# OpenMined/PIR

Hardware: AMD Instinct MI355X
Metric: PIR queries/sec (ms/query in ms_per_step), N=4096 DB=2^20 x 288B d=2 (higher is better)
Workload: dtype u64; 1 GPU; N=4096, 2 RNS data primes (36,36 bit | special 37 bit), t=24 bit, DB=2^20 x 288B, d=2, dims=[162, 162], num_pt=26215, 64 queries/step (whole job), 16 in flight per GPU (BASELINE.json configs[2]); workers=16, dist_mode=single, exchange=none, parallelism=single GPU, database_copies_in_hbm=operand layout only (u64 staging released)

## Files before the change

pir_amd/csrc/ctx.hip:

```cpp
#include <hip/hip_runtime.h>
#include <ctype.h>
#include <stdint.h>
#include <stdio.h>
#include <stdlib.h>
#include <string.h>

#include <algorithm>
#include <atomic>
#include <functional>
#include <map>
#include <mutex>
#include <string>
#include <vector>

#include "../../include/pirgpu.h"
#include "ctmult.h"
#include "device_params.h"
#include "host_math.h"
#include "kernels.h"
#include "wire.h"

using namespace pirgpu;

namespace {
// ... 142 lines not shown
struct pirgpu_ctx {
  pirgpu_params prm{};
  uint32_t N = 0, logN = 0, k = 0, d = 0;
  size_t ctw = 0;
  uint32_t rp = 0;
  size_t rctw = 0;
  uint32_t dims[PIRGPU_MAX_DIMS]{};
  uint64_t stride[PIRGPU_MAX_DIMS + 1]{};
  uint32_t sv_off[PIRGPU_MAX_DIMS + 1]{};
  uint32_t dim_sum = 0;
  uint32_t er = 0, E = 0;
  uint64_t reply_cts = 1;
  uint64_t P = 0;
  uint32_t sb = 0, se = 0;
  uint32_t slot0 = 0, nslots = 0;
  bool slot_sharded = false;
  hipEvent_t ev_after = nullptr;
  uint64_t pt_begin = 0, pt_end = 0;
  uint32_t planes = 1;
  uint64_t plane_pad = 0;
  uint32_t tables = 1;
  uint64_t table_pad = 0;
  uint32_t cur_table = 0;
  std::vector<uint64_t> tbl_loaded, tbl_zero;
  std::vector<uint8_t> tbl_packed;
  uint64_t scan_launches = 0;
  uint64_t ct_blocks = 0;
  uint64_t ct_relins = 0;
  uint64_t ct_lifts = 0;
  uint32_t bits = 0;

  int device = 0;
  hipStream_t stream = nullptr;
  const NttOps* ops = nullptr;
  int mode = kNttInt;
  DevParams hp{};
  DevParams* dp = nullptr;
  std::vector<void*> allocs;

  uint64_t* d_db = nullptr;
  std::vector<uint8_t> loaded;
  uint64_t n_loaded = 0;
  std::vector<KeySet> keysets{1};
  uint32_t keyset_cap = 64;
  uint32_t cur_keyset = 0;
  uint32_t cur_keyset_gen = 0;
  uint64_t keyset_clock = 0, key_uploads = 0, keyset_evictions = 0;
  std::vector<uint64_t*> key_pool;
  uint64_t* d_key_stage = nullptr;
  std::map<uint32_t, uint64_t*> xpow;
  std::map<uint32_t, uint16_t*> gperm;

  bool ws_ready = false;
  std::vector<Worker> workers;
  std::vector<uint64_t> lvl_rows;
  std::vector<uint64_t> lvl_cts;
  uint64_t m_max = 1;
  uint64_t pt_words = 0;
  BatchSet sets[kBatchSets];
  BatchSet& bs();
  uint32_t n_active = 1;
  uint32_t upper_blocks = 512;
  uint32_t upper_blocks_batch = 64;
  uint32_t scan_wgs_batch = 128;
  bool in_batch = false;
  uint32_t scan_nsplit = 1, scan_cps = 0, scan_rows = 0, scan_cols = 0;
  uint32_t scan_rpt = 4, scan_block = 256;
  bool scan_limb = false;
  uint32_t mq_nq = 4, mq_rows = 1;
  bool mq_single = true;
  uint32_t mq_single_rows = 4;
  bool mq_single_limb = false;
  uint64_t scan_npt = 0;
  bool mfma_on = false;
  MfmaGeom mg{};
  uint32_t mfma_nq = kMaxMfmaQueries;
  bool mfma_single = true;
  bool scan_f64_fold = false;
  bool scan_f64_fold_batch = false;
  bool split_upper = false;
  uint64_t split_upper_words = (3ull << 30) / 8;
  bool loop_transforms = true;
  uint32_t loop_min_sources = 1024;
  uint32_t fuse_mac_nodes = 128;
  bool fuse_mac_combine = true;
  bool fuse_last_level = true;
  bool last_level_ntt = true;
  bool tree40 = true;
  bool c0_ntt = false;
  bool c0_ntt_split = false;
  bool want_sel_f64 = true;
  bool sel_f64 = false;
  bool pack40 = false;
  int pack_bytes = 5;
  uint8_t* d_dbp = nullptr;
  bool packed_valid = false;
  bool staging_released = false;
  bool streamed = false;
  uint64_t stream_bands = 1;
  uint64_t db_bytes = 0, dbp_alloc = 0, mem_scratch = 0, mem_peak = 0;
  std::vector<BatchLane> lanes;
  uint64_t groups_run = 0;
  hipStream_t head_stream = nullptr;
  uint32_t head_levels = 5;
  uint32_t head_mode = 1;
  hipEvent_t ev_head_tail = nullptr;
  hipStream_t copy_stream = nullptr;
  hipEvent_t ev_fetch[2] = {nullptr, nullptr};
  hipEvent_t ev_fork = nullptr;
  hipEvent_t ev_main_join = nullptr;

  bool ctm = false;
  bool ctm_deferred = false;
  uint32_t kb = 0;
  uint64_t aux_primes[PIRGPU_MAX_PRIMES]{};
  DevParams hp_aux{};
  DevParams* dp_aux = nullptr;
  CtmParams* d_ctm = nullptr;
  uint64_t ctm_scratch_words = (256ull << 20) / 8;
  bool ctm_shared_sel = false;
  std::map<hipStream_t, CtmScratch> ctm_ws;

  bool prof = false;
  std::vector<hipEvent_t> bscan_ev;
  uint32_t bscan_n = 0, bscan_wgs = 0, bscan_nq = 0;
  static constexpr int kMaxProfRuns = 256;
  std::vector<hipEvent_t> ev;
  int prof_runs = 0;
  int prof_cur = -1;
  float timings[6]{};

  std::map<std::string, int64_t> opts;
  std::string err;
  uint64_t gen = 0;
  std::recursive_mutex mu;
  uint64_t zero_pts = 0;
  uint64_t remote_zero_pts = 0;
  bool allow_transparent = false;

  template <typename T>
  T* dalloc(size_t count) {
    void* p = nullptr;
    HIP_TRY(hipMalloc(&p, std::max<size_t>(count, 1) * sizeof(T)));
    allocs.push_back(p);
    return static_cast<T*>(p);
  }
  void use_device() { HIP_TRY(hipSetDevice(device)); }
};

BatchSet& pirgpu_ctx::bs() { return sets[t_batch_set]; }

static inline uint64_t held_pts(const pirgpu_ctx* c) { return (uint64_t)c->tables * c->planes * (c->pt_end - c->pt_begin); }
static inline uint64_t matrix_pts(const pirgpu_ctx* c) {
  return c->planes > 1 ? (uint64_t)c->planes * c->plane_pad : c->pt_end - c->pt_begin;
}
static inline uint64_t db_row(const pirgpu_ctx* c, uint64_t index) {
  if (c->tables > 1) return index / c->P * c->table_pad + index % c->P;
  return c->planes > 1 ? index / c->P * c->plane_pad + index % c->P : index - c->pt_begin;
}
static inline const uint64_t* table_db(const pirgpu_ctx* c, uint32_t t) {
  return c->d_db ? c->d_db + (size_t)t * c->table_pad * c->k * c->N : nullptr;
}
static inline void note_mem(pirgpu_ctx* c) {
  c->mem_peak = std::max(c->mem_peak, c->db_bytes + c->dbp_alloc + c->mem_scratch);
}
struct ScratchNote {
// ... 177 lines not shown

uint64_t stream_band_bytes(const pirgpu_ctx* c) { return 16ull * c->scan_cols * c->k * c->N * 8; }

int64_t option(const pirgpu_ctx* c, const char* name, int64_t dflt, bool* present = nullptr) {
  if (present) *present = true;
  auto it = c->opts.find(name);
  if (it != c->opts.end()) return it->second;
  const std::string env = std::string("PIRGPU_") + name;
  const char* v = pirgpu_env(env.c_str());
  if (v && *v) return strtoll(v, nullptr, 10);
  if (present) *present = false;
  return dflt;
}

void sync_batch_streams(pirgpu_ctx* c) {
  for (BatchLane& ln : c->lanes)
    if (ln.stream) HIP_TRY(hipStreamSynchronize(ln.stream));
  if (c->head_stream) HIP_TRY(hipStreamSynchronize(c->head_stream));
  if (c->copy_stream) HIP_TRY(hipStreamSynchronize(c->copy_stream));
  for (Worker& w : c->workers)
    if (w.stream) HIP_TRY(hipStreamSynchronize(w.stream));
}

bool all_zero_bytes(const uint8_t* p, size_t n) {
  for (size_t i = 0; i < n; ++i)
    if (p[i]) return false;
  return true;
}

void note_plaintext(pirgpu_ctx* c, uint64_t local, bool zero) {
  uint8_t& st = c->loaded[local];
  if (c->tables > 1) {
    const uint64_t t = local / c->P;
    if (!st) ++c->tbl_loaded[t];
    if (st == 2) --c->tbl_zero[t];
    if (zero) ++c->tbl_zero[t];
  }
  if (!st) ++c->n_loaded;
  if (st == 2) --c->zero_pts;
  st = zero ? 2 : 1;
  if (zero) ++c->zero_pts;
}

bool table_loaded(const pirgpu_ctx* c, uint32_t t) {
  return c->tables > 1 ? c->tbl_loaded[t] == c->P : c->n_loaded == held_pts(c);
}

void check_transparent(pirgpu_ctx* c, uint32_t table = 0) {
  const uint64_t zeros = c->tables > 1 ? c->tbl_zero[table] : c->zero_pts || c->remote_zero_pts;
  if (zeros && !c->allow_transparent) throw Fail{PIRGPU_INTERNAL, "result ciphertext is transparent"};
}

struct TablePlan {
  std::vector<uint32_t> order, run_begin;
  bool identity = true;
};
TablePlan plan_table_runs(const uint32_t* tables, uint32_t count, uint32_t group) {
  TablePlan tp;
  tp.order.resize(count);
  for (uint32_t i = 0; i < count; ++i) tp.order[i] = i;
  std::stable_sort(tp.order.begin(), tp.order.end(), [&](uint32_t a, uint32_t b) { return tables[a] < tables[b]; });
  group = std::max<uint32_t>(group, 1);
  for (uint32_t i = 0; i < count; ++i) {
    tp.identity = tp.identity && tp.order[i] == i;
    if (i == 0 || i % group == 0 || tables[tp.order[i]] != tables[tp.order[i - 1]]) tp.run_begin.push_back(i);
  }
  tp.run_begin.push_back(count);
  return tp;
}

void alloc_worker(pirgpu_ctx* c, Worker& w);
void ensure_expansion_buffers(pirgpu_ctx* c, Worker& w);

void ensure_workspace(pirgpu_ctx* c) {
  if (c->ws_ready) return;
  const uint32_t N = c->N, k = c->k, d = c->d;

  const uint64_t m_max = std::min<uint64_t>(N, hm::next_power_two(std::max<uint32_t>(c->dim_sum, 1)));
  c->m_max = m_max;
  const uint64_t shard_pts = matrix_pts(c);
  c->upper_blocks = (uint32_t)std::max<int64_t>(1, option(c, "UPPER_BLOCKS", c->upper_blocks));
  c->upper_blocks_batch = (uint32_t)std::max<int64_t>(1, option(c, "UPPER_BLOCKS_BATCH", c->upper_blocks_batch));
  c->scan_wgs_batch = (uint32_t)std::max<int64_t>(0, option(c, "SCAN_MFMA_WGS_BATCH", c->scan_wgs_batch));
  c->upper_blocks_batch = std::min(c->upper_blocks_batch, c->upper_blocks);
  c->lvl_rows.assign(d, 0);
  c->lvl_cts.assign(d, 0);
  uint64_t pt_words = 0;
  for (uint32_t l = 0; l < d; ++l) {
    uint64_t rows = l == 0 ? c->planes : ceil_div(shard_pts, c->stride[l]);
    uint64_t C = 1;
    for (uint32_t x = l; x + 1 < d; ++x) C *= c->E;
    c->lvl_rows[l] = rows;
    c->lvl_cts[l] = std::max<uint64_t>(rows, 1) * C;
    if (l + 1 < d) {
      const uint64_t per_chunk = std::max<uint64_t>(rows, 1) * (C / c->E) * c->E * k;
      const uint64_t n_chunks = std::min<uint64_t>(c->dims[l], std::max<uint64_t>(1, ceil_div(c->upper_blocks, per_chunk)));
      pt_words = std::max<uint64_t>(pt_words, (n_chunks + 1) * std::max<uint64_t>(rows, 1) * C * 2 * k * N);
    }
  }
  c->pt_words = pt_words;
  if (d == 1) {
    c->scan_rows = c->planes;
    c->scan_cols = (uint32_t)(shard_pts / c->planes);
  } else {
    c->scan_cols = c->dims[d - 1];
    c->scan_rows = (uint32_t)ceil_div(shard_pts, c->scan_cols);
  }
  c->scan_npt = shard_pts;
  {
    auto env_u32 = [c](const char* name, uint32_t dflt) {
      return (uint32_t)option(c, name + 7, dflt);
    };
    c->scan_limb = true;
    for (uint32_t j = 0; j < k; ++j) c->scan_limb = c->scan_limb && (c->hp.mod[j].q >> 50) == 0;
    if (!env_u32("PIRGPU_SCAN_LIMB", 1)) c->scan_limb = false;
    c->mq_nq = 4;
    c->mq_rows = 1;
    c->mq_single = env_u32("PIRGPU_SCAN_MQ_SINGLE", 1) != 0;
    c->mq_single_rows = 4;
    c->mq_single_limb = false;
    c->scan_rpt = env_u32("PIRGPU_SCAN_ROWS", 4);
    c->scan_block = env_u32("PIRGPU_SCAN_BLOCK", 256);
    const uint32_t xblocks = (k * N / 2 + c->scan_block - 1) / c->scan_block;
    const uint32_t yblocks = (c->scan_rows + c->scan_rpt - 1) / c->scan_rpt;
    uint64_t have = (uint64_t)xblocks * std::max<uint32_t>(yblocks, 1) * c->scan_block / 256;
    uint32_t want = have >= 512 ? 1 : (uint32_t)ceil_div(1024, std::max<uint64_t>(have, 1));
    want = env_u32("PIRGPU_SCAN_NSPLIT", want);
    want = std::max<uint32_t>(1, std::min<uint32_t>(want, std::max<uint32_t>(c->scan_cols, 1)));
    c->scan_cps = (uint32_t)ceil_div(std::max<uint32_t>(c->scan_cols, 1), want);
    c->scan_nsplit = (uint32_t)ceil_div(std::max<uint32_t>(c->scan_cols, 1), c->scan_cps);
    c->fuse_last_level = env_u32("PIRGPU_FUSE_LAST", 1) != 0;
    c->fuse_mac_combine = env_u32("PIRGPU_FUSE_MAC_COMBINE", 1) != 0;
    c->last_level_ntt = env_u32("PIRGPU_LAST_NTT", 1) != 0;
    {
      const uint32_t v = env_u32("PIRGPU_C0_NTT", 0);
      c->c0_ntt = v != 0;
      c->c0_ntt_split = v >= 2;
    }
    c->want_sel_f64 = env_u32("PIRGPU_SEL_F64", 1) != 0;
    c->tree40 = env_u32("PIRGPU_TREE40", 1) != 0;
    c->fuse_mac_nodes = 128;
    c->head_levels = std::min<uint32_t>(env_u32("PIRGPU_HEAD_LEVELS", c->head_levels), 8);
    c->head_mode = std::min<uint32_t>(env_u32("PIRGPU_HEAD_MODE", c->head_mode), 2);
    c->split_upper = env_u32("PIRGPU_SPLIT_UPPER", c->logN >= 14 ? 1 : 0) != 0 && c->mode != kNttInt;
    if (c->logN >= 15) c->split_upper = true;
    c->split_upper_words = (uint64_t)env_u32("PIRGPU_SPLIT_UPPER_MB", 3072) * (1ull << 20) / 8;
    c->loop_transforms = env_u32("PIRGPU_LOOP_TRANSFORMS", 1) != 0 && c->mode != kNttInt;
    c->pack40 = env_u32("PIRGPU_PACK40", 1) != 0;
    {
      uint32_t bits = 0;
      for (uint32_t j = 0; j <= k; ++j) bits = std::max<uint32_t>(bits, 64 - (uint32_t)__builtin_clzll(c->hp.mod[j].q));
      const int need = bits <= 39 ? 5 : (bits <= 47 ? 6 : (bits <= 55 ? 7 : 8));
      int want = (int)env_u32("PIRGPU_PACK_BYTES", (uint32_t)need);
      if (want < need) want = need;
      if (c->mode == kNttInt && want != 5) want = 8;
      if (c->logN >= 15) want = 8;
      if (want > 7) c->pack40 = false;
      c->pack_bytes = c->pack40 ? want : 5;
      if (c->pack40 && c->pack_bytes == 7 && c->logN >= 14 && !env_u32("PIRGPU_TREE40_WIDE", 0)) c->tree40 = false;
      const NttOps* ops = ntt_ops_for(N, c->pack_bytes);
      if (ops != c->ops) {
        c->ops = ops;
        HIP_TRY(c->ops->configure(c->mode));
      }
    }
    bool wide_given = false;
// ... 118 lines not shown
}

void begin_profiled_run(pirgpu_ctx* c) {
  c->prof_cur = -1;
  if (!c->prof || c->prof_runs >= pirgpu_ctx::kMaxProfRuns) return;
  if (c->ev.empty()) {
    c->ev.resize((size_t)pirgpu_ctx::kMaxProfRuns * (PH_COUNT + 1));
    for (auto& e : c->ev) HIP_TRY(hipEventCreate(&e));
  }
  c->prof_cur = c->prof_runs++;
}

const uint64_t* xpow_table(pirgpu_ctx* c, hipStream_t st, uint32_t shift) {
  auto it = c->xpow.find(shift);
  if (it != c->xpow.end()) return it->second;
  const uint32_t N = c->N, k = c->k;
  std::vector<uint64_t> h((size_t)k * N, 0);
  for (uint32_t j = 0; j < k; ++j) h[(size_t)j * N + (N - shift)] = c->hp.mod[j].q - 1;
  uint64_t* buf = c->dalloc<uint64_t>((size_t)k * N);
  HIP_TRY(hipMemcpy(buf, h.data(), h.size() * 8, hipMemcpyHostToDevice));
  HIP_TRY(c->ops->ntt_batch(st, c->mode, c->dp, buf, k, k, 0, false));
  HIP_TRY(launch_tree_convert(st, c->dp, c->mode, buf, buf, (uint64_t)k * N, true));
  HIP_TRY(hipStreamSynchronize(st));
  c->xpow[shift] = buf;
  return buf;
}

const uint16_t* galois_perm_table(pirgpu_ctx* c, hipStream_t st, uint32_t g) {
  auto it = c->gperm.find(g);
  if (it != c->gperm.end()) return it->second;
  const uint32_t N = c->N, logN = c->logN, R = (uint32_t)ntt_log_ept((int)logN), EPT = 1u << R, NT = N >> R;
  auto brev = [&](uint32_t v) {
    uint32_t r = 0;
    for (uint32_t b = 0; b < logN; ++b) r |= ((v >> b) & 1u) << (logN - 1 - b);
    return r;
  };
  std::vector<uint16_t> h((size_t)2 * N);
  const uint32_t gs[2] = {g, galois_inverse(g, N)};
  for (int w = 0; w < 2; ++w)
    for (uint32_t P = 0; P < N; ++P) {
      const uint32_t ex = (uint32_t)(((uint64_t)(2 * brev(P) + 1) * gs[w]) & (2 * N - 1));
      const uint32_t Pin = brev(ex >> 1);
      const uint32_t slot = (Pin & (EPT - 1)) * NT + (Pin >> R);
      h[(size_t)w * N + P] = (uint16_t)(slot + (slot >> R));
    }
  uint16_t* buf = c->dalloc<uint16_t>((size_t)2 * N);
  HIP_TRY(hipMemcpy(buf, h.data(), h.size() * 2, hipMemcpyHostToDevice));
  HIP_TRY(hipStreamSynchronize(st));
  c->gperm[g] = buf;
  return buf;
}

struct TreeState {
  uint64_t* cur = nullptr;
  bool cur40 = false;
  bool c0ntt = false;
};

uint64_t* expand_core(pirgpu_ctx* c, hipStream_t st, uint64_t* res_a, uint64_t* res_b, uint64_t* dig, uint64_t* prod,
                      uint32_t n, uint32_t B, const MfmaPtrs* sel_dst = nullptr, bool sel_f64 = false,
                      const uint32_t* ksets = nullptr, uint32_t j_begin = 0, uint32_t j_end = UINT32_MAX,
                      const TreeState* from = nullptr, TreeState* to = nullptr,
                      const std::function<void()>& after_first = nullptr) {
  const uint32_t N = c->N, k = c->k;
  if (n > N) throw Fail{PIRGPU_INVALID_ARGUMENT, "Cannot expand more items from a CT than poly modulus degree"};
  const uint32_t logm = hm::ceil_log2(n);
  const bool fuse_last = sel_dst && c->mode != kNttInt && c->fuse_last_level;
  if (sel_f64 && !(fuse_last && c->last_level_ntt && n >= 2)) throw Fail{PIRGPU_INTERNAL, "double-form selectors need the NTT-domain last level"};
  uint64_t *cur = res_a, *nxt = res_b;
  bool cur40 = false;
  bool c0ntt = false;
  if (from) {
    cur = from->cur;
    cur40 = from->cur40;
    c0ntt = from->c0ntt;
    nxt = res_a;
  }
  const uint32_t j_stop = std::min(j_end, logm);
  const bool c0_path = c->c0_ntt && fuse_last && c->last_level_ntt && c->mode != kNttInt && c->fuse_mac_combine;
  const uint32_t fuse_from = B > 1 ? std::max<uint32_t>(c->fuse_mac_nodes / 2, 1) : c->fuse_mac_nodes;
  auto level_fused = [&](uint32_t j) {
    return c->mode != kNttInt && c->fuse_mac_combine && ((1u << j) * B) >= fuse_from && !(fuse_last && j + 1 == logm);
  };
  for (uint32_t j = j_begin; j < j_stop; ++j) {
    auto level_done = [&]() {
      if (from && j == j_begin) {
        nxt = res_b;
        if (after_first) after_first();
      }
    };
    const uint32_t g = (N >> j) + 1;
    const KeyPtrs key = keys_for(c, g, ksets, B);
    const uint32_t nodes = (1u << j) * B;
    const bool last_ntt = fuse_last && j + 1 == logm && c->last_level_ntt;
    const bool c0_in_digit = last_ntt && !c0ntt && ks_digit_takes_c0(nodes);
    if (cur40 && !(last_ntt ? (c0ntt || c0_in_digit) : true)) throw Fail{PIRGPU_INTERNAL, "5-byte tree reached a level that cannot read it"};
    if (c0_path && !c0ntt && level_fused(j) && !cur40 && !(from && j == j_begin)) {
      HIP_TRY(c->ops->tree_c0_fwd(st, c->mode, c->dp, k, cur, nodes));
      c0ntt = true;
    }
    HIP_TRY(c->ops->ks_digit(st, c->mode, c->dp, k, cur, g, nodes, dig, c->pack40, c0_in_digit ? prod : nullptr, cur40,
                             c->loop_transforms && (uint64_t)nodes * k >= c->loop_min_sources));
    if (level_fused(j)) {
      const uint32_t next_nodes = nodes * 2;
      const bool next_last = j + 2 == logm;
      const bool next_reads40 = next_last ? (fuse_last && c->last_level_ntt && (c0ntt || ks_digit_takes_c0(next_nodes)))
                                          : (next_nodes >= fuse_from);
      const bool out40 = c->tree40 && c->pack40 && j + 1 < logm && next_reads40 && (1u << j) < (N >> ntt_log_ept((int)c->logN));
      HIP_TRY(c->ops->ks_mac_intt(st, c->mode, c->dp, k, dig, key, nodes, prod, c->pack40, k, 1));
      HIP_TRY(c->ops->ks_mac_combine(st, c->mode, c->dp, k, dig, key, prod, cur, g, nodes, 1u << j, nxt, c->pack40, cur40,
                                     out40, c0ntt ? xpow_table(c, st, 1u << j) : nullptr,
                                     c0ntt ? galois_perm_table(c, st, g) : nullptr, c->c0_ntt_split));
      cur40 = out40;
      std::swap(cur, nxt);
      level_done();
      continue;
    }
    if (cur40 && !last_ntt) throw Fail{PIRGPU_INTERNAL, "5-byte tree reached an unfused level"};
    if (c0ntt && !last_ntt) throw Fail{PIRGPU_INTERNAL, "NTT-form c0 reached an unfused level"};
    if (fuse_last && j + 1 == logm && c->last_level_ntt) {
      const uint64_t* X = xpow_table(c, st, 1u << j);
      HIP_TRY(c->ops->ks_mac_intt(st, c->mode, c->dp, k, dig, key, nodes, prod, c->pack40, k, 1));
      HIP_TRY(c->ops->ks_last_ntt(st, c->mode, c->dp, k, cur, dig, key, prod, X, g, galois_inverse(g, N), 1u << j, n, B,
                                  *sel_dst, nodes, c->pack40, sel_f64, c0_in_digit, c0ntt ? (cur40 ? 2 : 1) : 0,
                                  galois_perm_table(c, st, g)));
      return nullptr;
    }
    HIP_TRY(c->ops->ks_mac_intt(st, c->mode, c->dp, k, dig, key, nodes, prod, c->pack40, 0, k + 1));
    if (fuse_last && j + 1 == logm) {
      HIP_TRY(c->ops->ks_last_level(st, c->mode, c->dp, k, cur, prod, g, 1u << j, n, B, *sel_dst, nodes, c->pack40));
      return nullptr;
    }
    const uint32_t hi_limit = j + 1 == logm ? n * B : UINT32_MAX;
    HIP_TRY(launch_ks_combine(st, c->dp, c->mode, N, k, cur, prod, galois_inverse(g, N), nodes, 1u << j, true, hi_limit,
                              c->pack40, nxt, c->pack_bytes));
    std::swap(cur, nxt);
    if (c0_path && j + 1 < logm && level_fused(j + 1)) {
      HIP_TRY(c->ops->tree_c0_fwd(st, c->mode, c->dp, k, cur, nodes * 2));
      c0ntt = true;
    }
    level_done();
  }
  if (to) {
    to->cur = cur;
    to->cur40 = cur40;
    to->c0ntt = c0ntt;
  }
  return cur;
}

uint64_t* expand_on_device(pirgpu_ctx* c, Worker& w, uint32_t n) {
  ensure_expansion_buffers(c, w);
  return expand_core(c, w.stream, w.res_a, w.res_b, w.dig, w.prod, n, 1, nullptr, false, &w.keyset);
}

void expand_query_to_sv(pirgpu_ctx* c, Worker& w, const uint64_t* d_query, uint32_t nq) {
  ensure_expansion_buffers(c, w);
  w.sv_cur = nullptr;
  w.sv_rows = nullptr;
  const uint32_t N = c->N, k = c->k;
  const size_t ctw = c->ctw;
  uint64_t remaining = c->dim_sum;
  uint64_t produced = 0;
  for (uint32_t q = 0; q < nq; ++q) {
    uint32_t n = (uint32_t)std::min<uint64_t>(remaining, N);
    if (n > 0) {
      HIP_TRY(launch_tree_convert(w.stream, c->dp, c->mode, d_query + (size_t)q * ctw, w.res_a, ctw, true));
      MfmaPtrs dst{};
      dst.p[0] = w.sv_ntt + produced * ctw;
      uint64_t* res = expand_core(c, w.stream, w.res_a, w.res_b, w.dig, w.prod, n, 1, &dst, false, &w.keyset);
      if (res) HIP_TRY(c->ops->ct_ntt_fwd_oop(w.stream, c->mode, c->dp, k, res, w.sv_ntt + produced * ctw, n, true));
    }
    produced += n;
    remaining -= n;
    if (remaining == 0) break;
  }
}

const uint64_t* scan_selectors(pirgpu_ctx* c, Worker& w) {
  const uint64_t* sv = w.sv_cur ? w.sv_cur : w.sv_ntt;
  return sv + (size_t)c->sv_off[c->d - 1] * c->ctw + (c->d == 1 ? (size_t)c->sb * c->ctw : 0);
}

bool mq_usable(pirgpu_ctx* c) { return c->scan_nsplit == 1 && c->scan_rows >= 1 && c->scan_cols >= 1; }

size_t dbp_bytes(const pirgpu_ctx* c) { return (size_t)c->nslots * c->mg.RT * c->mg.KG * c->mg.tile_bytes; }
uint8_t* table_dbp(const pirgpu_ctx* c, uint32_t t) { return c->d_dbp ? c->d_dbp + (size_t)t * dbp_bytes(c) : nullptr; }

void refuse_tables(const pirgpu_ctx* c) {
  if (c->tables > 1)
    throw Fail{PIRGPU_FAILED_PRECONDITION, "this context holds several tables (tables > 1): the multi-GPU entry points do "
                                           "not serve them"};
}

void refuse_wide(const pirgpu_ctx* c) {
  if (c->planes > 1)
    throw Fail{PIRGPU_FAILED_PRECONDITION, "this context holds wide items (plaintexts_per_item > 1): the multi-GPU entry "
                                           "points do not serve them"};
}

void refuse_switched(const pirgpu_ctx* c) {
  if (c->rp)
    throw Fail{PIRGPU_FAILED_PRECONDITION, "this context switches its results to fewer primes (result_primes > 0): the "
                                           "multi-GPU entry points do not serve it"};
}

void refuse_ctm(const pirgpu_ctx* c) {
  if (c->ctm)
    throw Fail{PIRGPU_FAILED_PRECONDITION, "this context multiplies ciphertexts (PIRGPU_CREATE_CT_MULTIPLY): the multi-GPU "
                                           "entry points do not serve it"};
}
// ... 187 lines not shown
  HIP_TRY(launch_ctm_lift(st, c->d_ctm, k, N, a, a_qstride, b, dim, nq, j0, n, r.xq, r.xb));
  HIP_TRY(c->ops->ntt_batch(st, c->mode, c->dp, r.xq, (uint64_t)n * 4 * k, k, 0, false));
  HIP_TRY(c->ops->ntt_batch(st, c->mode, c->dp_aux, r.xb, (uint64_t)n * 4 * kb, kb, 0, false));
  HIP_TRY(launch_ctm_tensor(st, c->dp, k, N, r.xq, r.yq, n));
  HIP_TRY(launch_ctm_tensor(st, c->dp_aux, kb, N, r.xb, r.yb, n));
  HIP_TRY(c->ops->ntt_batch(st, c->mode, c->dp, r.yq, (uint64_t)n * 3 * k, k, 0, true));
  HIP_TRY(c->ops->ntt_batch(st, c->mode, c->dp_aux, r.yb, (uint64_t)n * 3 * kb, kb, 0, true));
  HIP_TRY(launch_ctm_scale(st, c->d_ctm, k, N, r.yq, r.yb, r.d, n));
}

struct CtmSel {
  CtmSelPtrs q, b;
};
void ctm_products_sel(pirgpu_ctx* c, hipStream_t st, const CtmRegions& r, const uint64_t* a, uint64_t a_qstride,
                      const CtmSel& sel, uint32_t dim, uint32_t nq, uint32_t j0, uint32_t n) {
  const uint32_t N = c->N, k = c->k, kb = c->kb;
  HIP_TRY(launch_ctm_lift_polys(st, c->d_ctm, k, N, a, a_qstride, nq, j0, n, r.xq, r.xb));
  HIP_TRY(c->ops->ntt_batch(st, c->mode, c->dp, r.xq, (uint64_t)n * 2 * k, k, 0, false));
  HIP_TRY(c->ops->ntt_batch(st, c->mode, c->dp_aux, r.xb, (uint64_t)n * 2 * kb, kb, 0, false));
  HIP_TRY(launch_ctm_tensor_sel(st, c->dp, k, N, r.xq, sel.q, dim, nq, j0, r.yq, n));
  HIP_TRY(launch_ctm_tensor_sel(st, c->dp_aux, kb, N, r.xb, sel.b, dim, nq, j0, r.yb, n));
  HIP_TRY(c->ops->ntt_batch(st, c->mode, c->dp, r.yq, (uint64_t)n * 3 * k, k, 0, true));
  HIP_TRY(c->ops->ntt_batch(st, c->mode, c->dp_aux, r.yb, (uint64_t)n * 3 * kb, kb, 0, true));
  HIP_TRY(launch_ctm_scale(st, c->d_ctm, k, N, r.yq, r.yb, r.d, n));
}

constexpr uint64_t kCtmRowsumWgs = 512;
uint32_t ctm_rowsum_block(pirgpu_ctx* c, hipStream_t st, const CtmRegions& r, uint32_t cap, const uint64_t* a,
                          uint64_t a_qstride, const uint64_t* b, uint32_t dim, uint32_t nq, uint64_t nch, uint32_t j0, uint32_t nj,
                          const CtmSel* sel = nullptr) {
  const uint32_t N = c->N, k = c->k, kb = c->kb, n = nj * nq;
  const uint64_t end = (uint64_t)j0 + nj;
  const uint32_t row0 = j0 / dim, rows = (uint32_t)((end - 1) / dim) - row0 + 1;
  const bool cut = end < nch && end % dim != 0;
  const uint32_t fin = rows - (cut ? 1 : 0);
  const uint64_t wgs = (uint64_t)rows * nq * k * (N / 256);
  const uint64_t room = (uint64_t)cap / ((uint64_t)rows * nq);
  uint32_t splits = (uint32_t)std::min<uint64_t>({ceil_div(kCtmRowsumWgs, wgs), (uint64_t)nj, room ? room - 1 : 0});
  const int64_t most = option(c, "CT_ROWSUM_SPLITS", 0);
  if (most > 0) splits = (uint32_t)std::min<int64_t>(splits, most);
  if (splits < 2) splits = 1;
  if ((uint64_t)(splits > 1 ? splits + 1 : 1) * rows * nq > cap) throw Fail{PIRGPU_INTERNAL, "row-sum accumulators exceed the product scratch"};
  if (sel) {
    HIP_TRY(launch_ctm_lift_polys(st, c->d_ctm, k, N, a, a_qstride, nq, j0, n, r.xq, r.xb));
    HIP_TRY(c->ops->ntt_batch(st, c->mode, c->dp, r.xq, (uint64_t)n * 2 * k, k, 0, false));
    HIP_TRY(c->ops->ntt_batch(st, c->mode, c->dp_aux, r.xb, (uint64_t)n * 2 * kb, kb, 0, false));
    HIP_TRY(launch_ctm_tensor_rowsum_sel(st, c->dp, k, N, r.xq, sel->q, r.yq, dim, nq, j0, nj, splits));
    HIP_TRY(launch_ctm_tensor_rowsum_sel(st, c->dp_aux, kb, N, r.xb, sel->b, r.yb, dim, nq, j0, nj, splits));
  } else {
    HIP_TRY(launch_ctm_lift(st, c->d_ctm, k, N, a, a_qstride, b, dim, nq, j0, n, r.xq, r.xb));
    HIP_TRY(c->ops->ntt_batch(st, c->mode, c->dp, r.xq, (uint64_t)n * 4 * k, k, 0, false));
    HIP_TRY(c->ops->ntt_batch(st, c->mode, c->dp_aux, r.xb, (uint64_t)n * 4 * kb, kb, 0, false));
    HIP_TRY(launch_ctm_tensor_rowsum(st, c->dp, k, N, r.xq, r.yq, dim, nq, j0, nj, splits));
    HIP_TRY(launch_ctm_tensor_rowsum(st, c->dp_aux, kb, N, r.xb, r.yb, dim, nq, j0, nj, splits));
  }
  if (fin) {
    HIP_TRY(c->ops->ntt_batch(st, c->mode, c->dp, r.yq, (uint64_t)fin * nq * 3 * k, k, 0, true));
    HIP_TRY(c->ops->ntt_batch(st, c->mode, c->dp_aux, r.yb, (uint64_t)fin * nq * 3 * kb, kb, 0, true));
    HIP_TRY(launch_ctm_scale(st, c->d_ctm, k, N, r.yq, r.yb, r.d, fin * nq));
  }
  return fin;
}
void ctm_carry_row(pirgpu_ctx* c, hipStream_t st, const CtmRegions& r, uint32_t nq, uint32_t fin) {
  const size_t wq = (size_t)nq * 3 * c->k * c->N, wb = (size_t)nq * 3 * c->kb * c->N;
  if (!fin) return;
  HIP_TRY(hipMemcpyAsync(r.yq, r.yq + fin * wq, wq * 8, hipMemcpyDeviceToDevice, st));
  HIP_TRY(hipMemcpyAsync(r.yb, r.yb + fin * wb, wb * 8, hipMemcpyDeviceToDevice, st));
}

KeyPtrs relin_keys_for(pirgpu_ctx* c, const uint32_t* ksets, uint32_t nq) {
  for (uint32_t q = 0; q < nq; ++q) {
    const uint32_t slot = ksets[q];
    if (slot >= c->keysets.size() || !c->keysets[slot].keys.count(1))
      throw Fail{PIRGPU_INVALID_ARGUMENT, "RelinKeys missing: ciphertext multiplication at d >= 2 needs the client's "
                                          "relinearisation key (installed as the key of Galois element 1)"};
  }
  return keys_for(c, 1, ksets, nq);
}

void ctm_relinearize(pirgpu_ctx* c, hipStream_t st, const CtmRegions& r, uint32_t n, const KeyPtrs& key) {
  const uint32_t N = c->N, k = c->k;
  const uint64_t pw = (uint64_t)k * N;
  HIP_TRY(launch_tree_convert(st, c->dp, c->mode, r.d, r.xq, (uint64_t)n * 2 * pw, true, 2 * pw, 3 * pw));
  HIP_TRY(c->ops->ks_digit(st, c->mode, c->dp, k, r.xq, 1, n, r.dig, c->pack40, nullptr, false, false));
  HIP_TRY(c->ops->ks_mac_intt(st, c->mode, c->dp, k, r.dig, key, n, r.prod, c->pack40, 0, k + 1));
  HIP_TRY(launch_ks_combine(st, c->dp, c->mode, N, k, r.xq, r.prod, 1, n, 0, false, 0, c->pack40, r.yq, c->pack_bytes));
  if (c->mode != kNttInt) HIP_TRY(launch_tree_convert(st, c->dp, c->mode, r.yq, r.yq, (uint64_t)n * 2 * pw, false));
}

void post_scan_ctm_level(pirgpu_ctx* c, const Stage& sg, uint32_t l) {
  const uint32_t N = c->N, k = c->k, nq = sg.n, dim = c->dims[l];
  const size_t ctw = c->ctw;
  const uint64_t nch = c->lvl_rows[l + 1], rows = c->lvl_rows[l];
  hipStream_t st = sg.stream;
  if (nq > (uint32_t)kMaxMfmaQueries || sg.local_rows || sg.sel_f64) throw Fail{PIRGPU_INTERNAL, "unexpected stage in ciphertext-multiplication mode"};
  const KeyPtrs key = relin_keys_for(c, sg.ksets, nq);
  CtmScratch& ws = ctm_scratch(c, st);
  const uint32_t cap = ctm_cap_pairs(c);
  const CtmRegions r = ctm_regions(c, ws.buf, cap);
  if ((size_t)nq * dim * ctw > ws.selc_words) throw Fail{PIRGPU_INTERNAL, "selector scratch undersized"};
  for (uint32_t q = 0; q < nq; ++q)
    HIP_TRY(hipMemcpyAsync(ws.selc + (size_t)q * dim * ctw, static_cast<const uint64_t*>(sg.sel.p[q]) + (size_t)c->sv_off[l] * ctw,
                           (size_t)dim * ctw * 8, hipMemcpyDeviceToDevice, st));
  HIP_TRY(c->ops->ntt_batch(st, c->mode, c->dp, ws.selc, (uint64_t)nq * dim * 2 * k, k, 0, true));
  const bool shared = c->ctm_shared_sel;
  CtmSel sel{};
  if (shared) {
    if (!ws.selb) throw Fail{PIRGPU_INTERNAL, "shared-selector scratch missing"};
    for (uint32_t s0 = 0; s0 < nq * dim; s0 += 32767)
      HIP_TRY(launch_ctm_lift_polys(st, c->d_ctm, k, N, ws.selc + (size_t)s0 * ctw, 0, 1, 0, std::min<uint32_t>(32767, nq * dim - s0),
                                    nullptr, ws.selb + (size_t)s0 * 2 * c->kb * N));
    HIP_TRY(c->ops->ntt_batch(st, c->mode, c->dp_aux, ws.selb, (uint64_t)nq * dim * 2 * c->kb, c->kb, 0, false));
    c->ct_lifts += (uint64_t)2 * dim * nq;
    for (uint32_t q = 0; q < nq; ++q) {
      sel.q.p[q] = static_cast<const uint64_t*>(sg.sel.p[q]) + (size_t)c->sv_off[l] * ctw;
      sel.b.p[q] = ws.selb + (size_t)q * dim * 2 * c->kb * N;
    }
  }
  const uint32_t bj = std::max<uint32_t>(1, cap / nq);
  for (uint64_t j0 = 0; j0 < nch; j0 += bj) {
    const uint32_t nj = (uint32_t)std::min<uint64_t>(bj, nch - j0), n = nj * nq;
    ++c->ct_blocks;
    c->ct_lifts += (uint64_t)(shared ? 2 : 4) * n;
    if (c->ctm_deferred) {
      const uint32_t fin = ctm_rowsum_block(c, st, r, cap, sg.lvl[l + 1], c->lvl_cts[l + 1] * ctw, ws.selc, dim, nq, nch,
                                            (uint32_t)j0, nj, shared ? &sel : nullptr);
      if (!fin) continue;
      c->ct_relins += (uint64_t)fin * nq;
      ctm_relinearize(c, st, r, fin * nq, key);
      HIP_TRY(launch_ctm_accumulate(st, c->dp, k, N, r.yq, r.d, sg.lvl[l] + (size_t)(j0 / dim) * ctw, c->lvl_cts[l] * ctw, 1,
                                    nq, 0, fin, fin));
      if ((j0 + nj) % dim != 0 && j0 + nj < nch) ctm_carry_row(c, st, r, nq, fin);
      continue;
    }
    c->ct_relins += n;
    if (shared)
      ctm_products_sel(c, st, r, sg.lvl[l + 1], c->lvl_cts[l + 1] * ctw, sel, dim, nq, (uint32_t)j0, n);
    else
      ctm_products(c, st, r, sg.lvl[l + 1], c->lvl_cts[l + 1] * ctw, ws.selc, dim, nq, (uint32_t)j0, n);
    ctm_relinearize(c, st, r, n, key);
    HIP_TRY(launch_ctm_accumulate(st, c->dp, k, N, r.yq, r.d, sg.lvl[l], c->lvl_cts[l] * ctw, dim, nq, (uint32_t)j0, nj,
                                  (uint32_t)rows));
  }
}

void post_scan_stage(pirgpu_ctx* c, const Stage& sg, Worker* profiled) {
  const uint32_t N = c->N, k = c->k, d = c->d;
  const size_t ctw = c->ctw;
  const uint64_t shard_pts = matrix_pts(c);
  hipStream_t st = sg.stream;
  if (c->rp && !sg.last) throw Fail{PIRGPU_INTERNAL, "result_primes without a level-0 buffer"};
  auto level = [&](uint32_t l) { return c->rp && l == 0 ? sg.last : sg.lvl[l]; };
  auto switch_level = [&](uint32_t l) {
    if (!c->rp) return;
    const uint64_t qstride = c->lvl_cts[l] * ctw;
    if (l == 0)
      HIP_TRY(launch_mod_switch(st, c->dp, sg.last, sg.lvl[0], c->lvl_cts[0], k, c->rp, N, true, sg.n, qstride,
                                c->reply_cts * c->rctw));
    else
      HIP_TRY(launch_mod_switch(st, c->dp, sg.lvl[l], sg.lvl[l], c->lvl_cts[l], k, c->rp, N, false, sg.n, qstride, qstride));
  };
  if (shard_pts == 0) {
    HIP_TRY(hipMemsetAsync(sg.lvl[0], 0, (size_t)sg.n * c->reply_cts * c->rctw * 8, st));
    return;
  }
  if (profiled) record(c, *profiled, PH_UPPER);
  if (!sg.rows_inverted)
    HIP_TRY(c->ops->ntt_batch(st, c->mode, c->dp, level(d - 1), (uint64_t)sg.n * c->scan_rows * 2 * k, k, 0, true));
// ... 315 lines not shown
    for (size_t i = 1; i < c->workers.size(); ++i)
      if (c->workers[i].stream) (void)hipStreamSynchronize(c->workers[i].stream);
  }
  for (KeySet& ks : c->keysets)
    for (auto& kv : ks.keys) (void)hipFree(kv.second);
  for (uint64_t* p : c->key_pool) (void)hipFree(p);
  for (void* p : c->allocs) (void)hipFree(p);
  for (BatchSet& b : c->sets) {
    if (b.h_query) (void)hipHostFree(b.h_query);
    if (b.h_reply) (void)hipHostFree(b.h_reply);
    for (hipEvent_t e : b.dl_events) (void)hipEventDestroy(e);
    for (hipEvent_t e : b.rd_events) (void)hipEventDestroy(e);
    for (hipEvent_t e : b.st_events) (void)hipEventDestroy(e);
  }
  for (auto& e : c->ev) (void)hipEventDestroy(e);
  for (auto& e : c->bscan_ev) (void)hipEventDestroy(e);
  for (Worker& w : c->workers) {
    if (w.ev_expanded) (void)hipEventDestroy(w.ev_expanded);
    if (w.ev_scanned) (void)hipEventDestroy(w.ev_scanned);
    if (w.ev_done) (void)hipEventDestroy(w.ev_done);
    if (w.ev_join) (void)hipEventDestroy(w.ev_join);
  }
  for (BatchLane& ln : c->lanes) {
    if (ln.ev_scanned) (void)hipEventDestroy(ln.ev_scanned);
    if (ln.ev_join) (void)hipEventDestroy(ln.ev_join);
    if (ln.stream) (void)hipStreamDestroy(ln.stream);
  }
  if (c->head_stream) {
    (void)hipStreamSynchronize(c->head_stream);
    (void)hipStreamDestroy(c->head_stream);
  }
  if (c->ev_head_tail) (void)hipEventDestroy(c->ev_head_tail);
  for (BatchLane& ln : c->lanes)
    for (HeadSlot& hs : ln.head) {
      if (hs.ev_ready) (void)hipEventDestroy(hs.ev_ready);
      if (hs.ev_free) (void)hipEventDestroy(hs.ev_free);
    }
  if (c->copy_stream) {
    (void)hipStreamSynchronize(c->copy_stream);
    (void)hipStreamDestroy(c->copy_stream);
  }
  for (hipEvent_t e : c->ev_fetch)
    if (e) (void)hipEventDestroy(e);
  if (c->ev_fork) (void)hipEventDestroy(c->ev_fork);
  if (c->ev_after) (void)hipEventDestroy(c->ev_after);
  if (c->ev_main_join) (void)hipEventDestroy(c->ev_main_join);
  for (size_t i = 1; i < c->workers.size(); ++i)
    if (c->workers[i].stream) (void)hipStreamDestroy(c->workers[i].stream);
  if (c->stream) (void)hipStreamDestroy(c->stream);
  delete c;
}

const char* pirgpu_last_error(const pirgpu_ctx* c) {
  if (!c) return "null context";
  if (t_last_error_ctx == c && t_last_error_gen == c->gen)
    return t_last_error.c_str();
  return c->err.c_str();
}

void pirgpu_set_error(pirgpu_ctx* c, const char* message) { (void)fail(c, 0, message ? message : ""); }

void pirgpu_request_lock(pirgpu_ctx* c) {
  if (c) c->mu.lock();
}
void pirgpu_request_unlock(pirgpu_ctx* c) {
  if (c) c->mu.unlock();
}

int pirgpu_set_transparent_policy(pirgpu_ctx* c, int allow) {
  return guarded(c, [&]() -> int {
    c->allow_transparent = allow != 0;
    return PIRGPU_OK;
  });
}

static const struct { const char* name; bool early; } kOptions[] = {
    {"UPPER_BLOCKS", true}, {"UPPER_BLOCKS_BATCH", true}, {"SCAN_MFMA_WGS_BATCH", false}, {"SCAN_LIMB", true},
    {"SCAN_MQ_SINGLE", true}, {"SCAN_ROWS", true}, {"SCAN_BLOCK", true}, {"SCAN_NSPLIT", true},
    {"FUSE_LAST", true}, {"FUSE_MAC_COMBINE", true}, {"LAST_NTT", true}, {"C0_NTT", true}, {"SEL_F64", true}, {"TREE40", true},
    {"SPLIT_UPPER", true}, {"SPLIT_UPPER_MB", true}, {"PACK40", true}, {"PACK_BYTES", true}, {"TREE40_WIDE", true},
    {"SCAN_MFMA", true}, {"SCAN_MFMA_WIDE", true}, {"SCAN_MFMA_TOP4", true}, {"SCAN_MFMA_NQ", true}, {"SCAN_MFMA_SINGLE", true},
    {"HEAD_LEVELS", true}, {"HEAD_MODE", true}, {"SCAN_F64_FOLD", true}, {"SCAN_F64_FOLD_BATCH", true}, {"LOOP_TRANSFORMS", true},
    {"SLOTS_SCAN_WGS", false}, {"SLOTS_GATHER_NTT", false}, {"SLOTS_SCAN_BLK_MAJOR", false}, {"DB_STREAM_MB", true},
    {"CT_SCRATCH_MB", true}, {"CT_SHARED_SEL", true},
    {"TABLES_ONE_LAUNCH", false}, {"SCAN_LAUNCHES", false},
    {"CT_BLOCKS", false},
    {"CT_RELINS", false}, {"CT_ROWSUM_SPLITS", false},
    {"CT_LIFTS", false},
};

int pirgpu_set_option(pirgpu_ctx* c, const char* name, int64_t value) {
  return guarded(c, [&]() -> int {
    if (!name) return fail(c, PIRGPU_INVALID_ARGUMENT, "null option name");
    std::string up(name);
    for (char& ch : up) ch = (char)toupper((unsigned char)ch);
    for (const auto& o : kOptions) {
      if (up != o.name) continue;
      if (o.early && c->ws_ready)
        return fail(c, PIRGPU_FAILED_PRECONDITION, "option " + up + " shapes the workspace: set it before the context is first used");
      if (up == "SCAN_LAUNCHES") {
        c->scan_launches = (uint64_t)std::max<int64_t>(0, value);
        return PIRGPU_OK;
      }
      if (up == "CT_BLOCKS") {
        c->ct_blocks = (uint64_t)std::max<int64_t>(0, value);
        return PIRGPU_OK;
      }
      if (up == "CT_RELINS") {
        c->ct_relins = (uint64_t)std::max<int64_t>(0, value);
        return PIRGPU_OK;
      }
      if (up == "CT_LIFTS") {
        c->ct_lifts = (uint64_t)std::max<int64_t>(0, value);
        return PIRGPU_OK;
      }
      c->opts[up] = value;
      if (up == "SCAN_MFMA_WGS_BATCH") c->scan_wgs_batch = (uint32_t)std::max<int64_t>(0, value);
      return PIRGPU_OK;
    }
    return fail(c, PIRGPU_INVALID_ARGUMENT, "unknown option " + up);
  });
}

int pirgpu_get_option(pirgpu_ctx* c, const char* name, int64_t* value) {
  return guarded(c, [&]() -> int {
    if (!name || !value) return fail(c, PIRGPU_INVALID_ARGUMENT, "null argument");
    std::string up(name);
    for (char& ch : up) ch = (char)toupper((unsigned char)ch);
    for (const auto& o : kOptions)
      if (up == o.name) {
        bool present = false;
        *value = option(c, o.name, -1, &present);
        if (up == "SCAN_LAUNCHES") *value = (int64_t)c->scan_launches;
        if (up == "CT_BLOCKS") *value = (int64_t)c->ct_blocks;
        if (up == "CT_RELINS") *value = (int64_t)c->ct_relins;
        if (up == "CT_LIFTS") *value = (int64_t)c->ct_lifts;
        if (up == "CT_SHARED_SEL" && !present) *value = c->ctm && c->planes > 1;
        return PIRGPU_OK;
      }
    return fail(c, PIRGPU_INVALID_ARGUMENT, "unknown option " + up);
  });
}

uint64_t pirgpu_zero_plaintexts(const pirgpu_ctx* c) { return c ? c->zero_pts : 0; }

int pirgpu_set_remote_zero_plaintexts(pirgpu_ctx* c, uint64_t n) {
  return guarded(c, [&]() -> int {
    c->remote_zero_pts = n;
    return PIRGPU_OK;
  });
}

int pirgpu_check_ready(pirgpu_ctx* c) {
  return guarded(c, [&]() -> int {
    if (!table_loaded(c, c->cur_table)) return fail(c, PIRGPU_FAILED_PRECONDITION, "database not fully loaded");
    check_transparent(c, c->cur_table);
    return PIRGPU_OK;
  });
}

int pirgpu_get_params(const pirgpu_ctx* c, pirgpu_params* out) {
  if (!c || !out) return PIRGPU_INVALID_ARGUMENT;
  *out = c->prm;
  out->shard_begin = c->sb;
  out->shard_end = c->se;
  return PIRGPU_OK;
}

uint64_t pirgpu_db_size(const pirgpu_ctx* c) { return c ? c->n_loaded : 0; }
uint32_t pirgpu_planes(const pirgpu_ctx* c) { return c ? c->planes : 0; }
uint64_t pirgpu_reply_ct_count(const pirgpu_ctx* c) { return c ? c->reply_cts : 0; }
uint64_t pirgpu_reply_ct_words(const pirgpu_ctx* c) { return c ? c->rctw : 0; }

int pirgpu_mod_switch(pirgpu_ctx* c, const uint64_t* cts, uint64_t n, uint32_t r, uint64_t* out) {
  return guarded(c, [&]() -> int {
    if ((!cts || !out) && n) return fail(c, PIRGPU_INVALID_ARGUMENT, "null buffer");
    if (r < 1 || r >= c->k) return fail(c, PIRGPU_INVALID_ARGUMENT, "r must be in [1, num_data_primes)");
    if (!n) return PIRGPU_OK;
    const size_t in_words = (size_t)n * c->ctw, out_words = (size_t)n * 2 * r * c->N;
    uint64_t* dev = nullptr;
    HIP_TRY(hipMalloc((void**)&dev, (in_words + out_words) * 8));
    try {
      HIP_TRY(hipMemcpyAsync(dev, cts, in_words * 8, hipMemcpyHostToDevice, c->stream));
      HIP_TRY(launch_mod_switch(c->stream, c->dp, dev, dev + in_words, n, c->k, r, c->N, true));
      HIP_TRY(hipMemcpyAsync(out, dev + in_words, out_words * 8, hipMemcpyDeviceToHost, c->stream));
      HIP_TRY(hipStreamSynchronize(c->stream));
    } catch (...) {
      (void)hipFree(dev);
      throw;
    }
    HIP_TRY(hipFree(dev));
    return PIRGPU_OK;
  });
}
int pirgpu_ctmult_plan(uint32_t N, uint32_t k, const uint64_t* coeff_modulus, uint64_t special_prime, uint64_t plain_modulus,
                       uint64_t* aux_primes, uint32_t* n_aux) {
  return pirgpu_ctmult_plan_terms(N, k, coeff_modulus, special_prime, plain_modulus, 1, aux_primes, n_aux);
}

int pirgpu_ctmult_plan_terms(uint32_t N, uint32_t k, const uint64_t* coeff_modulus, uint64_t special_prime,
                             uint64_t plain_modulus, uint64_t terms, uint64_t* aux_primes, uint32_t* n_aux) {
  if (!coeff_modulus || !aux_primes) return PIRGPU_INVALID_ARGUMENT;
  if (n_aux) *n_aux = 0;
  uint64_t aux[kCtmMaxB] = {};
  if (const char* why = ctm::plan(N, k, coeff_modulus, special_prime, plain_modulus, aux, terms)) {
    g_create_error = why;
    return PIRGPU_INVALID_ARGUMENT;
  }
  for (uint32_t i = 0; i < k + 2; ++i) aux_primes[i] = aux[i];
  if (n_aux) *n_aux = k + 2;
  return PIRGPU_OK;
}

int pirgpu_ct_multiply(pirgpu_ctx* c, const uint64_t* a, const uint64_t* b, uint64_t n, uint64_t* out) {
  return guarded(c, [&]() -> int {
    if (!c->ctm) return fail(c, PIRGPU_FAILED_PRECONDITION, "not a ciphertext-multiplication context (PIRGPU_CREATE_CT_MULTIPLY)");
    if ((!a || !b || !out) && n) return fail(c, PIRGPU_INVALID_ARGUMENT, "null buffer");
    ensure_workspace(c);
    CtmScratch& ws = ctm_scratch(c, c->stream);
    const uint32_t cap = ctm_cap_pairs(c);
// ... 1122 lines not shown
  if (rc) return rc;
  return pirgpu_query_fetch(c, reply, cap, count);
}

uint64_t* pirgpu_reply_device_ptr(pirgpu_ctx* c) { return (c && c->ws_ready) ? c->workers[0].lvl[0] : nullptr; }

int pirgpu_reply_copy_to_device(pirgpu_ctx* c, uint64_t* dst, uint64_t cap) {
  return guarded(c, [&]() -> int {
    refuse_switched(c);
    refuse_ctm(c);
    if (c->workers.empty()) return fail(c, PIRGPU_FAILED_PRECONDITION, "no query has been run");
    Worker& w = c->workers[0];
    if (!w.reply_valid) return fail(c, PIRGPU_FAILED_PRECONDITION, "no query has been run");
    if (!dst || cap < c->reply_cts) return fail(c, PIRGPU_INVALID_ARGUMENT, "reply buffer too small");
    HIP_TRY(hipMemcpyAsync(dst, w.lvl[0], c->reply_cts * c->rctw * 8, hipMemcpyDeviceToDevice, c->stream));
    HIP_TRY(hipStreamSynchronize(c->stream));
    return PIRGPU_OK;
  });
}

int pirgpu_expand(pirgpu_ctx* c, const uint64_t* ct, uint32_t num_items, uint64_t* out) {
  return guarded(c, [&]() -> int {
    ensure_workspace(c);
    Worker& w = c->workers[0];
    if (!ct || (!out && num_items)) return fail(c, PIRGPU_INVALID_ARGUMENT, "null buffer");
    if (num_items > c->N)
      return fail(c, PIRGPU_INVALID_ARGUMENT, "Cannot expand more items from a CT than poly modulus degree");
    const uint64_t m_max = std::min<uint64_t>(c->N, hm::next_power_two(std::max<uint32_t>(c->dim_sum, 1)));
    if (hm::next_power_two(num_items) > m_max)
      return fail(c, PIRGPU_INVALID_ARGUMENT, "num_items exceeds this context's expansion workspace");
    w.keyset = current_keyset(c);
    HIP_TRY(hipMemcpyAsync(w.res_b, ct, c->ctw * 8, hipMemcpyHostToDevice, c->stream));
    HIP_TRY(launch_tree_convert(c->stream, c->dp, c->mode, w.res_b, w.res_a, c->ctw, true));
    uint64_t* res = expand_on_device(c, w, num_items);
    if (num_items) {
      HIP_TRY(launch_tree_convert(c->stream, c->dp, c->mode, res, res, (uint64_t)num_items * c->ctw, false));
      HIP_TRY(hipMemcpyAsync(out, res, (size_t)num_items * c->ctw * 8, hipMemcpyDeviceToHost, c->stream));
    }
    HIP_TRY(hipStreamSynchronize(c->stream));
    return PIRGPU_OK;
  });
}

int pirgpu_expand_multi(pirgpu_ctx* c, const uint64_t* cts, uint32_t num_cts, uint64_t total_items, uint64_t* out) {
  return guarded(c, [&]() -> int {
    ensure_workspace(c);
    Worker& w = c->workers[0];
    if (!cts || !out) return fail(c, PIRGPU_INVALID_ARGUMENT, "null buffer");
    if (num_cts != total_items / c->N + 1)
      return fail(c, PIRGPU_INVALID_ARGUMENT,
                  "Number of ciphertexts doesn't match number of items for oblivious expansion.");
    const uint64_t m_max = std::min<uint64_t>(c->N, hm::next_power_two(std::max<uint32_t>(c->dim_sum, 1)));
    uint64_t remaining = total_items, produced = 0;
    w.keyset = current_keyset(c);
    for (uint32_t q = 0; q < num_cts && remaining; ++q) {
      uint32_t n = (uint32_t)std::min<uint64_t>(remaining, c->N);
      if (hm::next_power_two(n) > m_max)
        return fail(c, PIRGPU_INVALID_ARGUMENT, "total_items exceeds this context's expansion workspace");
      HIP_TRY(hipMemcpyAsync(w.res_b, cts + (size_t)q * c->ctw, c->ctw * 8, hipMemcpyHostToDevice, c->stream));
      HIP_TRY(launch_tree_convert(c->stream, c->dp, c->mode, w.res_b, w.res_a, c->ctw, true));
      uint64_t* res = expand_on_device(c, w, n);
      HIP_TRY(launch_tree_convert(c->stream, c->dp, c->mode, res, res, (uint64_t)n * c->ctw, false));
      HIP_TRY(hipMemcpyAsync(out + produced * c->ctw, res, (size_t)n * c->ctw * 8, hipMemcpyDeviceToHost, c->stream));
      HIP_TRY(hipStreamSynchronize(c->stream));
      produced += n;
      remaining -= n;
    }
    return PIRGPU_OK;
  });
}

int pirgpu_substitute_power_x(pirgpu_ctx* c, uint64_t* ct, uint32_t power) {
  return guarded(c, [&]() -> int {
    ensure_workspace(c);
    Worker& w = c->workers[0];
    if (!ct) return fail(c, PIRGPU_INVALID_ARGUMENT, "null buffer");
    if (!(power & 1) || power >= 2 * c->N)
      return fail(c, PIRGPU_INTERNAL, "Galois element is not valid");
    KeyPtrs key{};
    key.p[0] = find_key(c, current_keyset(c), power);
    key.B = 1;
    HIP_TRY(hipMemcpyAsync(w.res_b, ct, c->ctw * 8, hipMemcpyHostToDevice, c->stream));
    HIP_TRY(launch_tree_convert(c->stream, c->dp, c->mode, w.res_b, w.res_a, c->ctw, true));
    HIP_TRY(c->ops->ks_digit(c->stream, c->mode, c->dp, c->k, w.res_a, power, 1, w.dig, c->pack40, nullptr, false, false));
    HIP_TRY(c->ops->ks_mac_intt(c->stream, c->mode, c->dp, c->k, w.dig, key, 1, w.prod, c->pack40, 0, c->k + 1));
    HIP_TRY(launch_ks_combine(c->stream, c->dp, c->mode, c->N, c->k, w.res_a, w.prod, galois_inverse(power, c->N), 1, 0,
                              false,  0, c->pack40, w.res_b, c->pack_bytes));
    HIP_TRY(launch_tree_convert(c->stream, c->dp, c->mode, w.res_b, w.res_b, c->ctw, false));
    HIP_TRY(hipMemcpyAsync(ct, w.res_b, c->ctw * 8, hipMemcpyDeviceToHost, c->stream));
    HIP_TRY(hipStreamSynchronize(c->stream));
    return PIRGPU_OK;
  });
}

int pirgpu_multiply_inverse_power_of_x(pirgpu_ctx* c, const uint64_t* ct, uint32_t kpow, uint64_t* out) {
  return guarded(c, [&]() -> int {
    ensure_workspace(c);
    Worker& w = c->workers[0];
    if (!ct || !out) return fail(c, PIRGPU_INVALID_ARGUMENT, "null buffer");
    const uint32_t twoN = 2 * c->N;
    const uint32_t index = (twoN - (kpow % twoN)) % twoN;
    HIP_TRY(hipMemcpyAsync(w.res_a, ct, c->ctw * 8, hipMemcpyHostToDevice, c->stream));
    HIP_TRY(launch_monomial_shift(c->stream, c->dp, c->N, c->k, w.res_a, index, 1, w.res_b));
    HIP_TRY(hipMemcpyAsync(out, w.res_b, c->ctw * 8, hipMemcpyDeviceToHost, c->stream));
    HIP_TRY(hipStreamSynchronize(c->stream));
    return PIRGPU_OK;
  });
}

int pirgpu_multiply(pirgpu_ctx* c, const uint64_t* sv, uint64_t sv_count, uint64_t* reply, uint64_t cap,
                    uint64_t* count) {
  return guarded(c, [&]() -> int {
    ensure_workspace(c);
    Worker& w = c->workers[0];
    if (sv_count != c->dim_sum)
      return fail(c, PIRGPU_INVALID_ARGUMENT, "Selection vector size does not match dimensions");
    if (!sv || !reply || cap < c->reply_cts) return fail(c, PIRGPU_INVALID_ARGUMENT, "reply buffer too small");
    const uint64_t m_max = std::min<uint64_t>(c->N, hm::next_power_two(std::max<uint32_t>(c->dim_sum, 1)));
    for (uint64_t s = 0; s < sv_count; s += m_max) {
      const uint64_t n = std::min<uint64_t>(m_max, sv_count - s);
      HIP_TRY(hipMemcpyAsync(w.res_a, sv + s * c->ctw, n * c->ctw * 8, hipMemcpyHostToDevice, c->stream));
      HIP_TRY(c->ops->ct_ntt_fwd_oop(c->stream, c->mode, c->dp, c->k, w.res_a, w.sv_ntt + s * c->ctw, n, false));
      HIP_TRY(hipStreamSynchronize(c->stream));
    }
    c->prof_cur = -1;
    w.sv_cur = nullptr;
    w.sv_rows = nullptr;
    w.table = c->cur_table;
    w.keyset = current_keyset(c);
    multiply_on_device(c, w);
    HIP_TRY(hipMemcpyAsync(reply, w.lvl[0], c->reply_cts * c->rctw * 8, hipMemcpyDeviceToHost, c->stream));
    HIP_TRY(hipStreamSynchronize(c->stream));
    if (count) *count = c->reply_cts;
    return PIRGPU_OK;
  });
}


int pirgpu_set_concurrency(pirgpu_ctx* c, uint32_t n_workers) {
  return guarded(c, [&]() -> int {
    if (n_workers < 1 || n_workers > 32) return fail(c, PIRGPU_INVALID_ARGUMENT, "workers must be in [1, 32]");
    ensure_workspace(c);
    while (c->workers.size() < n_workers) {
      c->workers.emplace_back();
      alloc_worker(c, c->workers.back());
    }
    c->n_active = n_workers;
    return PIRGPU_OK;
  });
}

static void ensure_batch_capacity(pirgpu_ctx* c, uint32_t count);
static inline uint64_t* reply_base(pirgpu_ctx* c) { return c->bs().ext_reply ? c->bs().ext_reply : c->bs().d_breply; }
static void check_reply_target(pirgpu_ctx* c, uint64_t count) {
  if (c->bs().ext_reply && count * c->reply_cts > c->bs().ext_reply_cts)
    throw Fail{PIRGPU_INVALID_ARGUMENT, "the caller's reply buffer (pirgpu_batch_set_reply_buffer) is too small for this batch"};
}

static int batch_stage_impl(pirgpu_ctx* c, const uint64_t* queries, uint32_t nq, uint32_t count, bool async) {
  return guarded(c, [&]() -> int {
    ensure_workspace(c);
    if (!queries || nq != c->dim_sum / c->N + 1)
      return fail(c, PIRGPU_INVALID_ARGUMENT,
                  "Number of ciphertexts doesn't match number of items for oblivious expansion.");
    if (count == 0 || count > 4096) return fail(c, PIRGPU_INVALID_ARGUMENT, "batch size must be in [1, 4096]");
    ensure_batch_capacity(c, count);
    BatchSet& b = c->bs();
    const size_t qwords = (size_t)nq * c->ctw;
// ... 1038 lines not shown
```

pir_amd/csrc/kernels.h:

```cpp
#pragma once
#include <hip/hip_runtime.h>
#include <stdint.h>

#include "device_params.h"

namespace pirgpu {

constexpr int kMaxScanChunks = 16;
constexpr int kMaxMfmaQueries = 8;
constexpr int kMaxScanGroups = 16;
constexpr int kMaxSlices = 16;

constexpr uint32_t kKsWideLevel = 256;
inline bool ks_digit_takes_c0(uint32_t nodes) { return nodes >= kKsWideLevel && nodes % 8 == 0; }

struct MfmaPtrs {
  const void* p[kMaxMfmaQueries];
};

struct ScanGroups {
  uint32_t n;
  const uint8_t* sel[kMaxScanGroups];
  uint64_t* out[kMaxScanGroups];
  uint8_t nq[kMaxScanGroups];
};

struct ScanGroupsDb : ScanGroups {
  const uint8_t* db[kMaxScanGroups];
};

struct SliceMap {
  uint32_t n;
  uint32_t cut[kMaxSlices + 1];
  uint64_t off[kMaxSlices];
};

struct KeyPtrs {
  const uint64_t* p[kMaxMfmaQueries];
  uint32_t B;
};

struct NttOps {
  hipError_t (*configure)(int mode);
  hipError_t (*ntt_batch)(hipStream_t st, int mode, const DevParams* P, uint64_t* data, uint64_t n_polys,
                          uint32_t mod_period, uint32_t mod_base, bool inverse);
  hipError_t (*ct_ntt_fwd_oop)(hipStream_t st, int mode, const DevParams* P, uint32_t k, const uint64_t* src,
                               uint64_t* dst, uint64_t n_cts, bool src_is_tree);
  hipError_t (*ct_ntt_fwd_split)(hipStream_t st, int mode, const DevParams* P, uint32_t k, const uint64_t* src,
                                 const MfmaPtrs& dst, uint32_t B, uint64_t n_cts_total);
  hipError_t (*db_encode)(hipStream_t st, int mode, const DevParams* P, uint32_t k, const uint64_t* coeffs,
                          const uint8_t* bytes, uint64_t bytes_per_pt, uint64_t total_bytes, uint32_t bits,
                          uint64_t n_pt, uint64_t* db, uint32_t planes, uint64_t plane_bytes, uint64_t plane_stride);
  hipError_t (*ks_digit)(hipStream_t st, int mode, const DevParams* P, uint32_t k, const uint64_t* res_in,
                         uint32_t galois_elt, uint32_t nodes, uint64_t* dig, bool pack40, uint64_t* c0_out, bool tree40,
                         bool loop_targets);
  hipError_t (*ks_mac_intt)(hipStream_t st, int mode, const DevParams* P, uint32_t k, const uint64_t* dig,
                            const KeyPtrs& key, uint32_t nodes, uint64_t* prod, bool pack40, uint32_t I_base,
                            uint32_t I_count);
  hipError_t (*upper_fused)(hipStream_t st, int mode, const DevParams* P, uint32_t k, uint32_t enc_count,
                            const uint64_t* src, const MfmaPtrs& svq, uint64_t* part, uint32_t n_rows,
                            uint32_t n_dim, uint32_t n_children_total, uint32_t sv_first, uint32_t C,
                            uint32_t chunk_len, uint32_t n_chunks, uint32_t n_queries, uint64_t src_qstride,
                            uint64_t part_qstride, bool sel_f64);
  hipError_t (*ks_last_level)(hipStream_t st, int mode, const DevParams* P, uint32_t k, const uint64_t* tree,
                              const uint64_t* prod, uint32_t galois_elt, uint32_t shift_pow, uint32_t n_items,
                              uint32_t B, const MfmaPtrs& dst, uint32_t tree_cts, bool pack40);
  hipError_t (*upper_ntt)(hipStream_t st, int mode, const DevParams* P, uint32_t k, uint32_t enc_count,
                          const uint64_t* src, uint64_t* scratch, uint32_t n_rows, uint32_t n_dim,
                          uint32_t n_children_total, uint32_t C, uint32_t b0, uint32_t blk, uint32_t n_queries,
                          uint64_t src_qstride, bool loop_source);
  hipError_t (*ks_mac_combine)(hipStream_t st, int mode, const DevParams* P, uint32_t k, const uint64_t* dig,
                               const KeyPtrs& key, const uint64_t* prod, const uint64_t* tree_in, uint32_t galois_elt,
                               uint32_t nodes, uint32_t shift_pow, uint64_t* tree_out, bool pack40, bool tin40,
                               bool tout40, const uint64_t* xpow_c0ntt,
                               const uint16_t* perm,
                               bool c0_split);
  hipError_t (*ks_last_ntt)(hipStream_t st, int mode, const DevParams* P, uint32_t k, const uint64_t* tree,
                            const uint64_t* dig, const KeyPtrs& key, uint64_t* prod, const uint64_t* xpow,
                            uint32_t galois_elt, uint32_t galois_inv, uint32_t shift_pow, uint32_t n_items, uint32_t B,
                            const MfmaPtrs& dst, uint32_t nodes, bool pack40, bool out_f64, bool c0_done, int c0_tree,
                            const uint16_t* perm);
  hipError_t (*ntt_inv_gather)(hipStream_t st, int mode, const DevParams* P, uint32_t k, const uint64_t* src,
                               uint64_t* dst, const SliceMap& map, uint32_t RC, uint32_t nq, uint32_t nq_total,
                               uint32_t q0);
  hipError_t (*tree_c0_fwd)(hipStream_t st, int mode, const DevParams* P, uint32_t k, uint64_t* tree, uint32_t cts);
};

const NttOps* ntt_ops_for(uint32_t N, int pack_bytes = 5);

hipError_t launch_ntt_reorder(hipStream_t st, uint32_t N, const uint64_t* in, uint64_t* out, uint64_t n_polys,
                              bool to_device, bool as_f64);
hipError_t launch_copy_rows(hipStream_t st, const uint64_t* src, uint64_t* dst, const uint64_t* src_idx,
                            const uint64_t* dst_idx, uint64_t n, uint64_t words, uint64_t src_stride, uint64_t dst_stride);
hipError_t launch_db_splice(hipStream_t st, const DevParams* P, uint64_t* coef, uint32_t N, const uint8_t* img,
                            const uint8_t* upd, uint64_t n, uint64_t bytes_per_pt, uint32_t item_bytes, uint32_t bits,
                            uint32_t* nonzero);
hipError_t launch_pack40x4(hipStream_t st, const uint64_t* in, uint32_t* out, uint64_t words);
hipError_t launch_unpack40x4(hipStream_t st, const uint32_t* in, uint64_t* out, uint64_t words);
hipError_t launch_ks_combine(hipStream_t st, const DevParams* P, int mode, uint32_t N, uint32_t k,
                             const uint64_t* res_in, const uint64_t* prod, uint32_t galois_inv, uint32_t nodes,
                             uint32_t shift_pow, bool expand_step, uint32_t hi_limit, bool pack40, uint64_t* res_out,
                             int pack_bytes = 5);
hipError_t launch_tree_convert(hipStream_t st, const DevParams* P, int mode, const uint64_t* in, uint64_t* out,
                               uint64_t words, bool to_tree, uint64_t chunk_words = 0, uint64_t in_stride = 0);
hipError_t launch_monomial_shift(hipStream_t st, const DevParams* P, uint32_t N, uint32_t k, const uint64_t* in,
                                 uint32_t shift, uint64_t count, uint64_t* out);
hipError_t launch_scan(hipStream_t st, const DevParams* P, uint32_t N, uint32_t k, const uint64_t* db,
                       const uint64_t* sv, uint64_t* out, uint32_t rows, uint32_t cols, uint64_t num_pt,
                       uint32_t nsplit, uint32_t cols_per_split, uint32_t rows_per_thread, uint32_t block,
                       bool limb);
hipError_t launch_scan_mq(hipStream_t st, const DevParams* P, uint32_t N, uint32_t k, const uint64_t* db,
                          const uint64_t* const* sv, uint64_t* const* out, uint32_t nq, uint32_t rows,
                          uint32_t cols, uint32_t rows_per_wave, bool limb);
hipError_t launch_reduce_splits(hipStream_t st, const DevParams* P, const uint64_t* part, uint32_t nsplit,
                                uint64_t words, uint64_t* out, uint32_t n_queries = 1, uint64_t part_qstride = 0,
                                uint64_t out_qstride = 0);
hipError_t launch_mod_switch(hipStream_t st, const DevParams* P, const uint64_t* in, uint64_t* out, uint64_t n_cts,
                             uint32_t k, uint32_t r, uint32_t N, bool compact, uint32_t n_queries = 1,
                             uint64_t in_qstride = 0, uint64_t out_qstride = 0);

hipError_t launch_upper_mac_int(hipStream_t st, const DevParams* P, const uint64_t* scratch, const MfmaPtrs& svq,
                                uint64_t* acc, uint64_t* out, uint32_t n_queries, uint32_t n_rows, uint32_t C,
                                uint32_t enc_count, uint32_t k, uint32_t N, uint32_t sv_first, uint32_t b0, uint32_t blk,
                                uint32_t n_dim, bool first, bool last, uint64_t acc_qstride, uint64_t out_qstride);

hipError_t launch_upper_mac(hipStream_t st, const DevParams* P, const uint64_t* scratch, const MfmaPtrs& svq,
                            uint64_t* acc, uint64_t* out, uint32_t n_queries, uint32_t n_rows, uint32_t C,
                            uint32_t enc_count, uint32_t k, uint32_t N, uint32_t sv_first, uint32_t b0, uint32_t blk,
                            uint32_t n_dim, bool first, bool last, uint64_t acc_qstride, uint64_t out_qstride);

struct MfmaGeom {
  uint32_t L;
  uint32_t RT;
  uint32_t KG;
  uint32_t KS;
  uint32_t GC;
  uint32_t nchunks;
  uint32_t NW;
  uint32_t top4;
  uint32_t tile_bytes;
  size_t db_bytes, sel_bytes;
};

MfmaGeom mfma_geometry(const DevParams& hp, uint32_t rows, uint32_t cols, int wide_override = -1, bool allow_top4 = true);
hipError_t launch_db_pack(hipStream_t st, const DevParams* P, const MfmaGeom& gm, const uint64_t* db, uint8_t* dbp,
                          uint32_t rows, uint32_t cols, uint32_t kN, uint32_t slot0 = 0, uint32_t nslots = 0);
hipError_t launch_db_pack_band(hipStream_t st, const DevParams* P, const MfmaGeom& gm, const uint64_t* band, uint8_t* dbp,
                               uint32_t rt0, uint32_t n_rt, uint64_t npts, uint32_t cols, uint32_t kN, uint32_t slot0 = 0,
                               uint32_t nslots = 0);
hipError_t launch_db_unpack(hipStream_t st, const DevParams* P, const MfmaGeom& gm, const uint8_t* dbp, uint64_t* out,
                            uint32_t row, uint32_t col, uint32_t kN);
struct DbUnit {
  uint32_t r, kg, mask, out0;
};
hipError_t launch_db_gather(hipStream_t st, const DevParams* P, const MfmaGeom& gm, const uint8_t* dbp,
                            const DbUnit* units, uint32_t n_units, uint64_t* out, uint32_t N);
hipError_t launch_db_pack_update(hipStream_t st, const DevParams* P, const MfmaGeom& gm, const uint64_t* enc,
                                 const DbUnit* units, uint32_t n_units, uint8_t* dbp, uint32_t kN, uint32_t slot0,
                                 uint32_t nslots);
hipError_t launch_sel_pack(hipStream_t st, const DevParams* P, const MfmaGeom& gm, const MfmaPtrs& sv, uint32_t nq,
                           uint8_t* selp, uint32_t cols, uint32_t kN, bool sel_f64 = false, const SliceMap* map = nullptr);
hipError_t launch_scan_mfma(hipStream_t st, const DevParams* P, const MfmaGeom& gm, const uint8_t* dbp,
                            const uint8_t* selp, uint64_t* out, uint64_t out_qstride, uint32_t nq, uint32_t rows,
                            uint32_t kN, uint64_t chunk_stride, uint32_t wgs = 0, bool f64_fold = false);
// ... 13 lines not shown
```

pir_amd/csrc/ntt_kernels.hip:

```cpp
#include <hip/hip_runtime.h>
#include <stdint.h>
#include <stdlib.h>

#include "device_params.h"
#include "kernels.h"
#include "ntt_core.h"

#ifndef PIRGPU_LOGN
#error "compile with -DPIRGPU_LOGN=<11..14>"
#endif

#ifndef PIRGPU_PACK_BYTES
#define PIRGPU_PACK_BYTES 5
#endif
#define PIRGPU_CAT2(a, b) a##b
#define PIRGPU_CAT(a, b) PIRGPU_CAT2(a, b)
#if PIRGPU_PACK_BYTES == 5
#define PIRGPU_OPS_NAME PIRGPU_CAT(ntt_ops_, PIRGPU_LOGN)
#define PIRGPU_DEG_NS PIRGPU_CAT(deg, PIRGPU_LOGN)
#else
#define PIRGPU_OPS_NAME PIRGPU_CAT(PIRGPU_CAT(ntt_ops_, PIRGPU_LOGN), PIRGPU_CAT(_p, PIRGPU_PACK_BYTES))
#define PIRGPU_DEG_NS PIRGPU_CAT(PIRGPU_CAT(deg, PIRGPU_LOGN), PIRGPU_CAT(p, PIRGPU_PACK_BYTES))
#endif

namespace pirgpu {
namespace PIRGPU_DEG_NS {

constexpr int LOGN = PIRGPU_LOGN;
constexpr int NT = Plan<LOGN>::NT;
constexpr int N = Plan<LOGN>::N;
constexpr int R_ = Plan<LOGN>::R;
constexpr int EPT = Plan<LOGN>::EPT;
constexpr size_t kLdsBytes = (size_t)Plan<LOGN>::LDS_WORDS * 8;
#ifndef PIRGPU_PF14
#define PIRGPU_PF14 1
#endif
constexpr bool kPF = LOGN < 14 || (EPT == 32 && PIRGPU_PF14 != 0);
#ifndef PIRGPU_PF_LOOP
#define PIRGPU_PF_LOOP 1
#endif
constexpr bool kPFLoop = kPF && (EPT == 32 || PIRGPU_PF_LOOP != 0);
#ifndef PIRGPU_MC_FOUR_WAVES
#define PIRGPU_MC_FOUR_WAVES 1
#endif
#if PIRGPU_MC_FOUR_WAVES && PIRGPU_LOGN <= 12
#define PIRGPU_MC_WAVES __attribute__((amdgpu_waves_per_eu(4)))
#else
#define PIRGPU_MC_WAVES
#endif
#ifndef PIRGPU_PK_FOUR_WAVES
#define PIRGPU_PK_FOUR_WAVES 1
#endif
#if PIRGPU_PK_FOUR_WAVES && PIRGPU_LOGN == 13 && PIRGPU_PACK_BYTES != 5
#define PIRGPU_PK_WAVES __attribute__((amdgpu_waves_per_eu(4)))
#else
#define PIRGPU_PK_WAVES
#endif
#ifndef PIRGPU_DIG13_FOUR_WAVES
#define PIRGPU_DIG13_FOUR_WAVES 0
#endif
#if PIRGPU_PF_LOOP && !(PIRGPU_DIG13_FOUR_WAVES && PIRGPU_LOGN == 13)
#define PIRGPU_FOUR_WAVES
#else
#define PIRGPU_FOUR_WAVES __attribute__((amdgpu_waves_per_eu(4)))
#endif
#ifndef PIRGPU_UPPER_PLAIN_PF
#define PIRGPU_UPPER_PLAIN_PF 1
#endif
constexpr bool kUpperLdsTw = LOGN <= 12;
constexpr uint32_t kWideLevel = kKsWideLevel;

extern __shared__ __attribute__((aligned(16))) unsigned char smem_raw[];

constexpr int kPB = PIRGPU_PACK_BYTES;
constexpr int kHB = kPB - 4;
static_assert(kPB >= 5 && kPB <= 7, "packed residues are 5, 6 or 7 bytes");
constexpr size_t kPoly40 = (size_t)kPB * N;
__device__ __forceinline__ uint64_t load40(const uint8_t* poly, uint32_t i) {
  return (uint64_t)reinterpret_cast<const uint32_t*>(poly)[i] | ((uint64_t)poly[4 * N + i] << 32);
}
__device__ __forceinline__ void store40(uint8_t* poly, uint32_t i, uint64_t v) {
  reinterpret_cast<uint32_t*>(poly)[i] = (uint32_t)v;
  poly[4 * N + i] = (uint8_t)(v >> 32);
}

constexpr int kHW = kHB * EPT / 4;
struct Hi16 {
  uint32_t w[kHW];
};
__device__ __forceinline__ Hi16 load40f_hi(const uint8_t* poly, uint32_t tid) {
  Hi16 h;
#pragma unroll
  for (int g = 0; g < kHW / 4; ++g) {
    const uint4 v = *reinterpret_cast<const uint4*>(poly + 4 * N + (size_t)kHB * EPT * tid + 16 * g);
    h.w[4 * g] = v.x, h.w[4 * g + 1] = v.y, h.w[4 * g + 2] = v.z, h.w[4 * g + 3] = v.w;
  }
  return h;
}
__device__ __forceinline__ uint32_t hi_word(const Hi16& h, int e) {
  if constexpr (kHB == 1) {
    return __builtin_amdgcn_perm(0x43300000u, h.w[e >> 2], 0x07060c00u | (uint32_t)(e & 3));
  } else if constexpr (kHB == 2) {
    const uint32_t o = 2u * (uint32_t)(e & 1);
    return __builtin_amdgcn_perm(0x43300000u, h.w[e >> 1], 0x07060000u | ((o + 1u) << 8) | o);
  } else {
    const int b = 3 * e, wl = b >> 2;
    const uint32_t o = (uint32_t)(b & 3);
    const uint32_t nxt = h.w[wl + 1 < kHW ? wl + 1 : wl];
    return __builtin_amdgcn_perm(nxt, h.w[wl], 0x0c000000u | ((o + 2u) << 16) | ((o + 1u) << 8) | o) | 0x43000000u;
  }
}
__device__ __forceinline__ double load40f(const uint8_t* poly, const Hi16& h, int e, uint32_t tid, double magic) {
  const uint32_t lo = reinterpret_cast<const uint32_t*>(poly)[e * NT + tid];
  return __longlong_as_double((long long)(((uint64_t)hi_word(h, e) << 32) | lo)) - magic;
}
__device__ __forceinline__ void pack_hi_bytes(const uint32_t (&hb)[EPT], uint32_t (&w)[kHW]) {
  if constexpr (kHB == 1) {
#pragma unroll
    for (int g = 0; g < EPT / 4; ++g) {
      const uint32_t ab = __builtin_amdgcn_perm(hb[4 * g + 1], hb[4 * g], 0x0c0c0400u);
      const uint32_t cd = __builtin_amdgcn_perm(hb[4 * g + 3], hb[4 * g + 2], 0x0c0c0400u);
      w[g] = __builtin_amdgcn_perm(cd, ab, 0x05040100u);
    }
  } else if constexpr (kHB == 2) {
#pragma unroll
    for (int g = 0; g < EPT / 2; ++g) w[g] = __builtin_amdgcn_perm(hb[2 * g + 1], hb[2 * g], 0x05040100u);
  } else {
#pragma unroll
    for (int mw = 0; mw < kHW; ++mw) {
      const int ea = (4 * mw) / 3;
      uint32_t sel = 0;
#pragma unroll
      for (int i = 0; i < 4; ++i) {
        const int B = 4 * mw + i, el = B / 3, bi = B % 3;
        sel |= (uint32_t)(el == ea ? bi : 4 + bi) << (8 * i);
      }
      w[mw] = __builtin_amdgcn_perm(hb[ea + 1 < EPT ? ea + 1 : ea], hb[ea], sel);
    }
  }
}
__device__ __forceinline__ void store_hi_words(uint8_t* poly, uint32_t tid, const uint32_t (&w)[kHW]) {
#pragma unroll
  for (int g = 0; g < kHW / 4; ++g)
    *reinterpret_cast<uint4*>(poly + 4 * N + (size_t)kHB * EPT * tid + 16 * g) = uint4{w[4 * g], w[4 * g + 1], w[4 * g + 2], w[4 * g + 3]};
}
__device__ __forceinline__ void store40f(uint8_t* poly, uint32_t tid, const double (&x)[EPT], double magic) {
  uint32_t hb[EPT];
#pragma unroll
  for (int e = 0; e < EPT; ++e) {
    uint32_t lo;
    f64_pack40(x[e], magic, lo, hb[e]);
    reinterpret_cast<uint32_t*>(poly)[e * NT + tid] = lo;
  }
  uint32_t w[kHW];
// ... 146 lines not shown
  ntt_forward<MODE, LOGN, kPF>(x, smem_raw, P, mi, tid);
#pragma unroll
  for (int e = 0; e < EPT; ++e) out[e * NT + tid] = A::out(x[e], m);
}

template <int MODE>
__global__ void __launch_bounds__(NT)
ct_ntt_fwd_split_kernel(const DevParams* __restrict__ P, const uint64_t* __restrict__ src, MfmaPtrs dst, uint32_t B) {
  using A = Arith<MODE>;
  const uint32_t tid = threadIdx.x;
  const uint32_t k2 = 2 * P->k;
  const int mi = blockIdx.x % P->k;
  const typename A::Mod m = A::mod(P, mi);
  const uint32_t ct = blockIdx.x / k2, rem = blockIdx.x % k2;
  const uint32_t slot = ct / B, q = ct % B;
  const typename A::T* in = reinterpret_cast<const typename A::T*>(src) + (size_t)blockIdx.x * N;
  uint64_t* out = (uint64_t*)dst.p[q] + ((size_t)slot * k2 + rem) * N;
  typename A::T x[EPT];
#pragma unroll
  for (int e = 0; e < EPT; ++e) x[e] = in[e * NT + tid];
  ntt_forward<MODE, LOGN, kPF>(x, smem_raw, P, mi, tid);
#pragma unroll
  for (int e = 0; e < EPT; ++e) out[e * NT + tid] = A::out(x[e], m);
}

template <int MODE>
__global__ void __launch_bounds__(NT)
db_encode_kernel(const DevParams* __restrict__ P, const uint64_t* __restrict__ coeffs,
                 const uint8_t* __restrict__ bytes, uint64_t bytes_per_pt, uint64_t total_bytes, uint32_t bits,
                 uint64_t* __restrict__ db, uint64_t plane_bytes, uint64_t plane_stride) {
  using A = Arith<MODE>;
  const uint32_t tid = threadIdx.x, k = P->k;
  const uint32_t j = blockIdx.y;
  const uint64_t pt = blockIdx.x;
  const uint64_t plane_off = blockIdx.z * plane_bytes;
  const ModConst mc = P->mod[j];
  const typename A::Mod m = A::mod(P, j);
  const uint64_t thr = P->plain_thr;
  const uint64_t inc = P->lift_inc[j] >= mc.q ? P->lift_inc[j] - mc.q : P->lift_inc[j];
  uint64_t L = 0;
  const uint8_t* src = nullptr;
  if (!coeffs) {
    const uint64_t start = pt * bytes_per_pt + plane_off;
    uint64_t len = bytes_per_pt - plane_off;
    if (gridDim.z > 1 && len > plane_bytes) len = plane_bytes;
    L = start >= total_bytes ? 0 : (total_bytes - start < len ? total_bytes - start : len);
    src = bytes + start;
  }
  typename A::T x[EPT];
#pragma unroll
  for (int e = 0; e < EPT; ++e) {
    const uint32_t c = e * NT + tid;
    uint64_t v;
    if (coeffs) {
      v = coeffs[pt * N + c];
    } else {
      v = 0;
      uint64_t bitpos = (uint64_t)c * bits;
      uint64_t byte = bitpos >> 3;
      uint32_t off = (uint32_t)(bitpos & 7);
      int need = (int)bits;
      while (need > 0) {
        uint32_t B = byte < L ? src[byte] : 0u;
        int avail = 8 - (int)off;
        int take = avail < need ? avail : need;
        v = (v << take) | ((B >> (avail - take)) & ((1u << take) - 1u));
        need -= take;
        off = 0;
        ++byte;
      }
    }
    uint64_t r = reduce64(v, mc);
    if (v >= thr) r = add_mod(r, inc, mc.q);
    x[e] = A::in(r, m);
  }
  ntt_forward<MODE, LOGN, kPF>(x, smem_raw, P, j, tid);
  uint64_t* out = db + ((blockIdx.z * plane_stride + pt) * k + j) * N;
#pragma unroll
  for (int e = 0; e < EPT; ++e) out[e * NT + tid] = A::out(x[e], m);
}

template <int MODE, bool P40, bool T40>
__device__ __forceinline__ void tree_c0_ntt_body(const DevParams* __restrict__ P, const uint64_t* __restrict__ tree_raw,
                                                 uint64_t* __restrict__ prod, uint32_t node, uint32_t j, uint32_t tid) {
  using A = Arith<MODE>;
  static_assert(MODE != kNttInt, "fp64 flavours only");
  const uint32_t k = P->k, km = k + 1;
  const typename A::Mod m = A::mod(P, j);
  double x[EPT];
  tree_load<T40>(tree_raw, (size_t)node * 2 * k + j, tid, m.q, x);
  ntt_forward<MODE, LOGN, kPF, false>(x, smem_raw, P, j, tid);
  const size_t opoly = (size_t)node * 2 * km + j;
  if constexpr (P40) {
    uint8_t* out = reinterpret_cast<uint8_t*>(prod) + opoly * kPoly40;
    store40f(out, tid, x, f64_pack_magic(m.q));
  } else {
    double* out = reinterpret_cast<double*>(prod) + opoly * N;
#pragma unroll
    for (int e = 0; e < EPT; ++e) out[e * NT + tid] = x[e];
  }
}

template <int MODE, bool P40>
__global__ void __launch_bounds__(NT)
tree_c0_ntt_kernel(const DevParams* __restrict__ P, const uint64_t* __restrict__ tree_raw, uint64_t* __restrict__ prod) {
  tree_c0_ntt_body<MODE, P40, false>(P, tree_raw, prod, blockIdx.x / P->k, blockIdx.x % P->k, threadIdx.x);
}

template <int MODE>
__global__ void __launch_bounds__(NT)
tree_c0_fwd_kernel(const DevParams* __restrict__ P, uint64_t* __restrict__ tree_raw) {
  static_assert(MODE != kNttInt, "fp64 flavours only");
  const uint32_t tid = threadIdx.x, k = P->k;
  const uint32_t node = blockIdx.x / k, j = blockIdx.x % k;
  double* pp = reinterpret_cast<double*>(tree_raw) + ((size_t)node * 2 * k + j) * N;
  double x[EPT];
#pragma unroll
  for (int e = 0; e < EPT; ++e) x[e] = pp[e * NT + tid];
  ntt_forward<MODE, LOGN, kPF, false>(x, smem_raw, P, j, tid);
#pragma unroll
  for (int e = 0; e < EPT; ++e) pp[e * NT + tid] = x[e];
}

template <int MODE, bool P40, bool T40 = false, bool LOOPI = false>
__global__ void __launch_bounds__(NT) PIRGPU_FOUR_WAVES
ks_digit_kernel(const DevParams* __restrict__ P, const uint64_t* __restrict__ res_in, uint32_t galois_elt,
                uint64_t* __restrict__ dig, uint64_t* __restrict__ c0_out, uint32_t digit_blocks) {
  using A = Arith<MODE>;
  uint64_t* s = reinterpret_cast<uint64_t*>(smem_raw);
  const uint32_t tid = threadIdx.x;
  const uint32_t k = P->k;
  if constexpr (MODE != kNttInt) {
    if (blockIdx.x >= digit_blocks) {
      const uint32_t b = blockIdx.x - digit_blocks;
      tree_c0_ntt_body<MODE, P40, T40>(P, res_in, c0_out, b / k, b % k, tid);
      return;
    }
  }
  if constexpr (LOOPI) {
    static_assert(MODE != kNttInt, "fp64 flavours only");
    const uint32_t xcd = blockIdx.x & 7, t = blockIdx.x >> 3;
    const uint32_t J = t % k, node = (t / k) * 8 + xcd;
    double* sd = reinterpret_cast<double*>(smem_raw);
    const double qJd = P->tab[J].qd;
    const uint32_t raw0 = tid * galois_elt, rstep = (uint32_t)NT * galois_elt;
    double base[EPT];
    {
      double c1[EPT];
      tree_load<T40>(res_in, ((size_t)node * 2 + 1) * k + J, tid, qJd, c1);
#pragma unroll
      for (int e = 0; e < EPT; ++e) {
        const uint32_t raw = raw0 + (uint32_t)e * rstep;
        const uint64_t sign = (uint64_t)((raw << (31 - LOGN)) & 0x80000000u) << 32;
        double v = __longlong_as_double((long long)((uint64_t)__double_as_longlong(c1[e]) ^ sign));
        v = v < 0.0 ? v + qJd : v;
        sd[lds_idx<R_>(raw & (N - 1))] = v;
      }
      __syncthreads();
#pragma unroll
      for (int e = 0; e < EPT; ++e) base[e] = sd[lds_lin_base<NT, R_>(tid) + lds_lin_off<NT, R_>(e)];
    }
#pragma clang loop unroll(disable)
    for (uint32_t I = 0; I <= k; ++I) {
      const typename A::Mod m = A::mod(P, I);
      const bool norm_in = MODE == kNttF64Wide && I != J;
      double x[EPT];
#pragma unroll
      for (int e = 0; e < EPT; ++e) x[e] = norm_in ? f64_norm(base[e], m) : base[e];
      __syncthreads();
      const size_t poly = ((size_t)node * (k + 1) + I) * k + J;
      uint32_t tl = tid;
      asm volatile("" : "+v"(tl));
      if constexpr (P40) {
        ntt_forward<MODE, LOGN, kPFLoop, false>(x, smem_raw, P, I, tl);
        store40f(reinterpret_cast<uint8_t*>(dig) + poly * kPoly40, tl, x, f64_pack_magic(m.q));
      } else {
        ntt_forward<MODE, LOGN, kPFLoop>(x, smem_raw, P, I, tl);
        double* out = reinterpret_cast<double*>(dig) + poly * N;
#pragma unroll
        for (int e = 0; e < EPT; ++e) out[e * NT + tl] = x[e];
      }
    }
    return;
  }
  uint32_t node = blockIdx.x, I = blockIdx.y, J = blockIdx.z;
  if (gridDim.y == 1) {
    const uint32_t xcd = blockIdx.x & 7, t = blockIdx.x >> 3;
    I = t % (k + 1);
    const uint32_t u = t / (k + 1);
    J = u % k;
    node = (u / k) * 8 + xcd;
  }
  const ModConst mI = P->mod[I];
  const typename A::Mod m = A::mod(P, I);
  [[maybe_unused]] const uint64_t qJ = P->mod[J].q;
  [[maybe_unused]] const uint64_t* src = res_in + (((size_t)node * 2 + 1) * k + J) * N;
  typename A::T x[EPT];
  if constexpr (MODE == kNttInt) {
#pragma unroll
    for (int e = 0; e < EPT; ++e) {
      const uint32_t i = e * NT + tid;
      const uint32_t raw = i * galois_elt;
      uint64_t v = src[i];
      if ((raw >> LOGN) & 1) v = neg_mod(v, qJ);
      s[lds_idx<R_>(raw & (N - 1))] = reduce64(v, mI);
    }
    __syncthreads();
#pragma unroll
    for (int e = 0; e < EPT; ++e) x[e] = A::in(s[lds_lin_base<NT, R_>(tid) + lds_lin_off<NT, R_>(e)], m);
  } else {
    double* sd = reinterpret_cast<double*>(smem_raw);
    const bool norm_in = MODE == kNttF64Wide && I != J;
    const double qJd = P->tab[J].qd;
    const uint32_t raw0 = tid * galois_elt, rstep = (uint32_t)NT * galois_elt;
    double c1[EPT];
    tree_load<T40>(res_in, ((size_t)node * 2 + 1) * k + J, tid, qJd, c1);
#pragma unroll
    for (int e = 0; e < EPT; ++e) {
      const uint32_t raw = raw0 + (uint32_t)e * rstep;
      const uint64_t sign = (uint64_t)((raw << (31 - LOGN)) & 0x80000000u) << 32;
      double v = __longlong_as_double((long long)((uint64_t)__double_as_longlong(c1[e]) ^ sign));
      v = v < 0.0 ? v + qJd : v;
      if (norm_in) v = f64_norm(v, m);
      sd[lds_idx<R_>(raw & (N - 1))] = v;
    }
    __syncthreads();
#pragma unroll
    for (int e = 0; e < EPT; ++e) x[e] = sd[lds_lin_base<NT, R_>(tid) + lds_lin_off<NT, R_>(e)];
  }
  __syncthreads();
  const size_t poly = ((size_t)node * (k + 1) + I) * k + J;
  if constexpr (P40 && MODE != kNttInt) {
    ntt_forward<MODE, LOGN, kPF, false>(x, smem_raw, P, I, tid);
    uint8_t* out = reinterpret_cast<uint8_t*>(dig) + poly * kPoly40;
    store40f(out, tid, x, f64_pack_magic(m.q));
  } else {
    ntt_forward<MODE, LOGN, kPF>(x, smem_raw, P, I, tid);
    if constexpr (P40) {
      uint8_t* out = reinterpret_cast<uint8_t*>(dig) + poly * kPoly40;
#pragma unroll
      for (int e = 0; e < EPT; ++e) store40(out, e * NT + tid, A::out(x[e], m));
    } else {
      typename A::T* out = reinterpret_cast<typename A::T*>(dig) + poly * N;
#pragma unroll
      for (int e = 0; e < EPT; ++e) out[e * NT + tid] = x[e];
    }
  }
}

template <int MODE, bool P40>
__device__ __forceinline__ void ks_mac_core(const DevParams* __restrict__ P, const uint64_t* __restrict__ dig_raw,
                                            const uint64_t* __restrict__ key_raw, uint32_t node, uint32_t I,
                                            uint32_t comp, uint32_t tid, typename Arith<MODE>::T (&x)[EPT]) {
  using A = Arith<MODE>;
  using T = typename A::T;
  const uint32_t k = P->k, km = k + 1;
  const ModConst mI = P->mod[I];
  const typename A::Mod m = A::mod(P, I);
  const size_t poly0 = ((size_t)node * km + I) * k;
  const T* d0 = reinterpret_cast<const T*>(dig_raw) + poly0 * N;
  const uint8_t* d40 = reinterpret_cast<const uint8_t*>(dig_raw) + poly0 * kPoly40;
  const T* key = reinterpret_cast<const T*>(key_raw);
  if constexpr (MODE == kNttInt) {
    auto digit = [&](uint32_t J, uint32_t i) -> T {
      if constexpr (P40) return A::in(load40(d40 + (size_t)J * kPoly40, i), m);
      else return d0[(size_t)J * N + i];
    };
    u128 acc[EPT];
#pragma unroll
    for (int e = 0; e < EPT; ++e) acc[e] = 0;
    for (uint32_t J = 0; J < k; ++J) {
      const T* kj = key + (((size_t)J * 2 + comp) * km + I) * N;
#pragma unroll
      for (int e = 0; e < EPT; ++e) acc[e] += (u128)digit(J, e * NT + tid) * kj[e * NT + tid];
    }
#pragma unroll
    for (int e = 0; e < EPT; ++e) x[e] = reduce128((uint64_t)acc[e], (uint64_t)(acc[e] >> 64), mI);
    ntt_inverse<MODE, LOGN, kPF>(x, smem_raw, P, I, tid);
  } else {
    const double magic = f64_pack_magic(m.q);
#pragma unroll
    for (int e = 0; e < EPT; ++e) x[e] = 0.0;
    for (uint32_t J = 0; J < k; ++J) {
      const T* kj = key + (((size_t)J * 2 + comp) * km + I) * N;
      if constexpr (P40) {
        const uint8_t* dj = d40 + (size_t)J * kPoly40;
        const Hi16 h = load40f_hi(dj, tid);
#pragma unroll
        for (int e = 0; e < EPT; ++e) x[e] += f64_mulmod(load40f(dj, h, e, tid, magic), kj[e * NT + tid], m);
      } else {
#pragma unroll
        for (int e = 0; e < EPT; ++e) x[e] += f64_mulmod(d0[(size_t)J * N + e * NT + tid], kj[e * NT + tid], m);
      }
    }
#pragma unroll
    for (int e = 0; e < EPT; ++e) x[e] = f64_norm(x[e], m);
    ntt_inverse<MODE, LOGN, kPF, false>(x, smem_raw, P, I, tid);
  }
}

template <int MODE, bool P40>
__global__ void __launch_bounds__(NT) PIRGPU_PK_WAVES
ks_mac_intt_kernel(const DevParams* __restrict__ P, const uint64_t* __restrict__ dig_raw, KeyPtrs keys,
                   uint64_t* __restrict__ prod, uint32_t I_base, uint32_t I_count) {
  using A = Arith<MODE>;
  using T = typename A::T;
  const uint32_t tid = threadIdx.x;
  const uint32_t k = P->k, km = k + 1;
  uint32_t node = blockIdx.x, I = blockIdx.y, comp = blockIdx.z;
  if (gridDim.y == 1 && gridDim.z == 1) {
    const uint32_t xcd = blockIdx.x & 7, t = blockIdx.x >> 3;
    comp = t & 1;
    const uint32_t u = t >> 1;
    I = u % I_count;
    node = (u / I_count) * 8 + xcd;
  }
  I += I_base;
  const typename A::Mod m = A::mod(P, I);
  T x[EPT];
  ks_mac_core<MODE, P40>(P, dig_raw, keys.p[node % keys.B], node, I, comp, tid, x);
  const size_t opoly = ((size_t)node * 2 + comp) * km + I;
  if constexpr (P40 && MODE != kNttInt) {
    uint8_t* out = reinterpret_cast<uint8_t*>(prod) + opoly * kPoly40;
    store40f(out, tid, x, f64_pack_magic(m.q));
  } else if constexpr (MODE != kNttInt) {
    T* out = reinterpret_cast<T*>(prod) + opoly * N;
#pragma unroll
    for (int e = 0; e < EPT; ++e) out[e * NT + tid] = x[e];
  } else if constexpr (P40) {
    uint8_t* out = reinterpret_cast<uint8_t*>(prod) + opoly * kPoly40;
#pragma unroll
    for (int e = 0; e < EPT; ++e) store40(out, e * NT + tid, A::out(x[e], m));
  } else {
    uint64_t* out = prod + opoly * N;
#pragma unroll
    for (int e = 0; e < EPT; ++e) out[e * NT + tid] = A::out(x[e], m);
  }
}

template <int MODE, bool P40, bool TIN40, bool TOUT40>
__device__ __forceinline__ void ks_combine_c0_ntt(const DevParams* __restrict__ P, const uint64_t* __restrict__ dig_raw,
                                                  const uint64_t* __restrict__ key_raw, const uint64_t* __restrict__ prod,
                                                  const uint64_t* __restrict__ tree_in_raw, const double* __restrict__ xpow,
                                                  const uint16_t* __restrict__ perm, uint32_t galois_elt, uint32_t nodes,
                                                  uint32_t node, uint32_t j, uint32_t tid, uint64_t* __restrict__ tree_out_raw) {
  using A = Arith<MODE>;
  double* sd = reinterpret_cast<double*>(smem_raw);
  const uint32_t k = P->k, km = k + 1;
  const typename A::Mod m = A::mod(P, j);
  const double magic = f64_pack_magic(m.q);
  double x[EPT];
  {
    const double pf = P->p_f, half = P->p_half_f;
    const size_t spoly = ((size_t)node * 2 + 0) * km + k;
    [[maybe_unused]] Hi16 hs{};
    if constexpr (P40) hs = load40f_hi(reinterpret_cast<const uint8_t*>(prod) + spoly * kPoly40, tid);
#pragma unroll
    for (int e = 0; e < EPT; ++e) {
      double sp;
      if constexpr (P40)
        sp = load40f(reinterpret_cast<const uint8_t*>(prod) + spoly * kPoly40, hs, e, tid, f64_pack_magic(pf));
      else
        sp = reinterpret_cast<const double*>(prod)[spoly * N + e * NT + tid];
      sp = sp > half ? sp - pf : sp;
      sp = sp < -half ? sp + pf : sp;
      x[e] = f64_norm(sp, m);
    }
  }
  ntt_forward<MODE, LOGN, kPF, false>(x, smem_raw, P, j, tid);
  {
    const size_t dpoly0 = ((size_t)node * km + j) * k;
#pragma unroll
    for (int e = 0; e < EPT; ++e) x[e] = -x[e];
    const double* key = reinterpret_cast<const double*>(key_raw);
    for (uint32_t J = 0; J < k; ++J) {
      double d[EPT], kv[EPT];
      if constexpr (P40) load40f_rsrc(reinterpret_cast<const uint8_t*>(dig_raw) + (dpoly0 + J) * kPoly40, tid, magic, d);
      else loadf64_rsrc(reinterpret_cast<const double*>(dig_raw) + (dpoly0 + J) * N, tid, d);
      loadf64_rsrc(key + (((size_t)J * 2 + 0) * km + j) * N, tid, kv);
#pragma unroll
      for (int e = 0; e < EPT; ++e) x[e] += f64_mulmod(d[e], kv[e], m);
    }
    const double pinv = P->p_inv_f[j];
#pragma unroll
    for (int e = 0; e < EPT; ++e) x[e] = f64_mulmod(f64_norm(x[e], m), pinv, m);
  }
  uint32_t tid_e = tid;
  asm volatile("" : "+v"(tid_e));
  double v[EPT];
  tree_load<TIN40>(tree_in_raw, (size_t)node * 2 * k + j, tid_e, m.q, v);
  __syncthreads();
#pragma unroll
  for (int e = 0; e < EPT; ++e) sd[lds_lin_base<NT, R_>(tid_e) + lds_lin_off<NT, R_>(e)] = v[e];
  __syncthreads();
  {
    [[maybe_unused]] PermIdx pi{};
    if constexpr (PIRGPU_PERM_TABLE != 0) pi = load_perm(perm, tid_e);
#pragma unroll
    for (int e = 0; e < EPT; ++e) x[e] += sd[perm_at(pi, e, tid_e, galois_elt)];
  }
  const double* X = xpow + (size_t)j * N;
  const size_t plo = (size_t)node * 2 * k + j, phi = ((size_t)node + nodes) * 2 * k + j;
  double t[EPT];
#pragma unroll
  for (int e = 0; e < EPT; ++e) t[e] = f64_norm(v[e] + x[e], m);
  if constexpr (TOUT40) {
    store40f(reinterpret_cast<uint8_t*>(tree_out_raw) + plo * kPoly40, tid_e, t, magic);
  } else {
    double* tlo = reinterpret_cast<double*>(tree_out_raw) + plo * N;
#pragma unroll
    for (int e = 0; e < EPT; ++e) tlo[e * NT + tid_e] = t[e];
  }
  uint32_t tid_x = tid_e;
  asm volatile("" : "+v"(tid_x) : : "memory");
#pragma unroll
  for (int e = 0; e < EPT; ++e) t[e] = f64_mulmod(f64_norm(v[e] - x[e], m), X[e * NT + tid_x], m);
  if constexpr (TOUT40) {
    store40f(reinterpret_cast<uint8_t*>(tree_out_raw) + phi * kPoly40, tid_x, t, magic);
  } else {
    double* thi = reinterpret_cast<double*>(tree_out_raw) + phi * N;
#pragma unroll
    for (int e = 0; e < EPT; ++e) thi[e * NT + tid_x] = t[e];
  }
}

template <int MODE, bool P40, bool TIN40, bool TOUT40>
__global__ void __launch_bounds__(NT)
ks_c0_ntt_kernel(const DevParams* __restrict__ P, const uint64_t* __restrict__ dig_raw, KeyPtrs keys,
                 const uint64_t* __restrict__ prod, const uint64_t* __restrict__ tree_in_raw, uint32_t galois_elt,
                 uint32_t nodes, uint64_t* __restrict__ tree_out_raw, const double* __restrict__ xpow,
                 const uint16_t* __restrict__ perm) {
  static_assert(MODE != kNttInt, "fp64 flavours only");
  const uint32_t k = P->k;
  uint32_t node = blockIdx.x, j = blockIdx.y;
  if (gridDim.y == 1) {
    const uint32_t xcd = blockIdx.x & 7, t = blockIdx.x >> 3;
    j = t % k;
    node = (t / k) * 8 + xcd;
  }
  ks_combine_c0_ntt<MODE, P40, TIN40, TOUT40>(P, dig_raw, keys.p[node % keys.B], prod, tree_in_raw, xpow, perm, galois_elt, nodes,
                                              node, j, threadIdx.x, tree_out_raw);
}

template <int MODE, bool P40, bool TIN40 = false, bool TOUT40 = false, bool C0NTT = false>
__global__ void __launch_bounds__(NT) PIRGPU_MC_WAVES PIRGPU_PK_WAVES
ks_mac_combine_kernel(const DevParams* __restrict__ P, const uint64_t* __restrict__ dig_raw,
                      KeyPtrs keys, const uint64_t* __restrict__ prod,
                      const uint64_t* __restrict__ tree_in_raw, uint32_t galois_elt, uint32_t nodes, uint32_t shift_pow,
                      uint64_t* __restrict__ tree_out_raw, const double* __restrict__ xpow,
                      const uint16_t* __restrict__ perm, uint32_t comp1_only) {
  using A = Arith<MODE>;
  static_assert(MODE != kNttInt, "fp64 flavours only");
  double* sd = reinterpret_cast<double*>(smem_raw);
  const uint32_t tid = threadIdx.x, k = P->k, km = k + 1;
  uint32_t node = blockIdx.x, j = blockIdx.y, comp = blockIdx.z;
  if (gridDim.y == 1 && gridDim.z == 1) {
    const uint32_t xcd = blockIdx.x & 7, t = blockIdx.x >> 3;
    comp = comp1_only ? 1 : t & 1;
    const uint32_t u = comp1_only ? t : t >> 1;
    j = u % k;
    node = (u / k) * 8 + xcd;
  } else if (comp1_only) {
    comp = 1;
  }
  if constexpr (C0NTT) {
    if (comp == 0) {
      ks_combine_c0_ntt<MODE, P40, TIN40, TOUT40>(P, dig_raw, keys.p[node % keys.B], prod, tree_in_raw, xpow, perm, galois_elt,
                                                  nodes, node, j, tid, tree_out_raw);
      return;
    }
  }
  const typename A::Mod m = A::mod(P, j);
  double g[EPT];
  ks_mac_core<MODE, P40>(P, dig_raw, keys.p[node % keys.B], node, j, comp, tid, g);
  {
    const double pf = P->p_f, half = P->p_half_f, pinv = P->p_inv_f[j];
    const size_t spoly = ((size_t)node * 2 + comp) * km + k;
    [[maybe_unused]] Hi16 hs{};
    if constexpr (P40) hs = load40f_hi(reinterpret_cast<const uint8_t*>(prod) + spoly * kPoly40, tid);
#pragma unroll
    for (int e = 0; e < EPT; ++e) {
      double sp;
      if constexpr (P40) {
        sp = load40f(reinterpret_cast<const uint8_t*>(prod) + spoly * kPoly40, hs, e, tid, f64_pack_magic(pf));
      } else {
        sp = reinterpret_cast<const double*>(prod)[spoly * N + e * NT + tid];
      }
      sp = sp > half ? sp - pf : sp;
      sp = sp < -half ? sp + pf : sp;
      g[e] = f64_mulmod(g[e] - f64_norm(sp, m), pinv, m);
    }
  }
  if (!C0NTT && comp == 0) {
    const uint32_t raw0 = tid * galois_elt, rstep = (uint32_t)NT * galois_elt;
    double c0[EPT];
    tree_load<TIN40>(tree_in_raw, (size_t)node * 2 * k + j, tid, m.q, c0);
    __syncthreads();
#pragma unroll
    for (int e = 0; e < EPT; ++e) {
      const uint32_t raw = raw0 + (uint32_t)e * rstep;
      const uint64_t sign = (uint64_t)((raw << (31 - LOGN)) & 0x80000000u) << 32;
      sd[lds_idx<R_>(raw & (N - 1))] = __longlong_as_double((long long)((uint64_t)__double_as_longlong(c0[e]) ^ sign));
    }
    __syncthreads();
#pragma unroll
    for (int e = 0; e < EPT; ++e) g[e] += sd[lds_lin_base<NT, R_>(tid) + lds_lin_off<NT, R_>(e)];
  }
  const size_t opoly = (size_t)comp * k + j;
  double a[EPT];
  tree_load<TIN40>(tree_in_raw, (size_t)node * 2 * k + opoly, tid, m.q, a);
  if constexpr (TOUT40) {
    const double magic = f64_pack_magic(m.q);
    uint8_t* plo = reinterpret_cast<uint8_t*>(tree_out_raw) + ((size_t)node * 2 * k + opoly) * kPoly40;
    uint8_t* phi = reinterpret_cast<uint8_t*>(tree_out_raw) + (((size_t)node + nodes) * 2 * k + opoly) * kPoly40;
    double lo[EPT];
#pragma unroll
    for (int e = 0; e < EPT; ++e) lo[e] = f64_norm(a[e] + g[e], m);
    store40f(plo, tid, lo, magic);
    const bool borrow = tid < shift_pow;
    const uint32_t tid_d = (tid - shift_pow) & (NT - 1);
    uint32_t hb[EPT];
#pragma unroll
    for (int e = 0; e < EPT; ++e) {
      double d = f64_norm(a[e] - g[e], m);
      if (e == 0) d = borrow ? -d : d;
      uint32_t l32;
      f64_pack40(d, magic, l32, hb[e]);
      reinterpret_cast<uint32_t*>(phi)[(e * NT + tid - shift_pow) & (N - 1)] = l32;
    }
    uint32_t w[kHW];
    pack_hi_bytes(hb, w);
    uint32_t o[kHW];
#pragma unroll
    for (int q4 = 0; q4 < kHW; ++q4)
      o[q4] = borrow ? __builtin_amdgcn_alignbyte(w[(q4 + 1) % kHW], w[q4], kHB) : w[q4];
    store_hi_words(phi, tid_d, o);
  } else {
    const size_t off = opoly * N;
    double* tree_lo = reinterpret_cast<double*>(tree_out_raw) + (size_t)node * 2 * k * N + off;
    double* tree_hi = reinterpret_cast<double*>(tree_out_raw) + ((size_t)node + nodes) * 2 * k * N + off;
#pragma unroll
    for (int e = 0; e < EPT; ++e) {
      const uint32_t i = e * NT + tid;
      tree_lo[i] = f64_norm(a[e] + g[e], m);
      const double d = f64_norm(a[e] - g[e], m);
      const uint32_t sraw = i + (2 * N - shift_pow);
      tree_hi[sraw & (N - 1)] = (sraw & N) ? -d : d;
    }
  }
}

template <int MODE, bool P40>
__global__ void __launch_bounds__(NT)
ks_last_level_kernel(const DevParams* __restrict__ P, const uint64_t* __restrict__ tree_raw,
                     const uint64_t* __restrict__ prod, uint32_t galois_elt, uint32_t shift_pow, uint32_t n_items,
                     uint32_t B, MfmaPtrs dst) {
  using A = Arith<MODE>;
  static_assert(MODE != kNttInt, "fp64 flavours only");
  double* sd = reinterpret_cast<double*>(smem_raw);
  const uint32_t tid = threadIdx.x, k = P->k, km = k + 1;
  const uint32_t half_id = blockIdx.x & 1, bx = blockIdx.x >> 1;
  const uint32_t j = bx % k, comp = (bx / k) & 1, ct = bx / (2 * k);
  const uint32_t slot = ct / B, q = ct % B;
  const uint32_t out_slot = half_id ? slot + shift_pow : slot;
  if (out_slot >= n_items) return;
  const typename A::Mod m = A::mod(P, j);
  const double pf = P->p_f, half = P->p_half_f, pinv = P->p_inv_f[j];
  const double* tree = reinterpret_cast<const double*>(tree_raw) + (size_t)ct * 2 * k * N;
  double g[EPT];
  [[maybe_unused]] Hi16 hs{}, hj{};
  if constexpr (P40) {
    const uint8_t* pr = reinterpret_cast<const uint8_t*>(prod) + ((size_t)ct * 2 + comp) * km * kPoly40;
    hs = load40f_hi(pr + (size_t)k * kPoly40, tid);
    hj = load40f_hi(pr + (size_t)j * kPoly40, tid);
  }
#pragma unroll
  for (int e = 0; e < EPT; ++e) {
    [[maybe_unused]] const uint32_t i = e * NT + tid;
    double sp, dj;
    if constexpr (P40) {
      const uint8_t* pr = reinterpret_cast<const uint8_t*>(prod) + ((size_t)ct * 2 + comp) * km * kPoly40;
      sp = load40f(pr + (size_t)k * kPoly40, hs, e, tid, f64_pack_magic(pf));
      dj = load40f(pr + (size_t)j * kPoly40, hj, e, tid, f64_pack_magic(m.q));
    } else {
      const double* pr = reinterpret_cast<const double*>(prod) + ((size_t)ct * 2 + comp) * km * N;
      sp = pr[(size_t)k * N + i];
      dj = pr[(size_t)j * N + i];
    }
    sp = sp > half ? sp - pf : sp;
    sp = sp < -half ? sp + pf : sp;
    g[e] = f64_mulmod(dj - f64_norm(sp, m), pinv, m);
  }
  if (comp == 0) {
    const double* c0 = tree + (size_t)j * N;
    const uint32_t raw0 = tid * galois_elt, rstep = (uint32_t)NT * galois_elt;
#pragma unroll
    for (int e = 0; e < EPT; ++e) {
      const uint32_t raw = raw0 + (uint32_t)e * rstep;
      const uint64_t sign = (uint64_t)((raw << (31 - LOGN)) & 0x80000000u) << 32;
      sd[lds_idx<R_>(raw & (N - 1))] =
          __longlong_as_double((long long)((uint64_t)__double_as_longlong(c0[e * NT + tid]) ^ sign));
    }
    __syncthreads();
#pragma unroll
    for (int e = 0; e < EPT; ++e) g[e] += sd[lds_lin_base<NT, R_>(tid) + lds_lin_off<NT, R_>(e)];
    __syncthreads();
  }
  const double* a = tree + ((size_t)comp * k + j) * N;
  typename A::T x[EPT];
  if (!half_id) {
#pragma unroll
    for (int e = 0; e < EPT; ++e) x[e] = f64_norm(a[e * NT + tid] + g[e], m);
  } else {
#pragma unroll
    for (int e = 0; e < EPT; ++e) {
      const uint32_t i = e * NT + tid;
      const double d = f64_norm(a[i] - g[e], m);
      const uint32_t sraw = i + (2 * N - shift_pow);
      sd[lds_idx<R_>(sraw & (N - 1))] = (sraw & N) ? -d : d;
    }
    __syncthreads();
#pragma unroll
    for (int e = 0; e < EPT; ++e) x[e] = sd[lds_lin_base<NT, R_>(tid) + lds_lin_off<NT, R_>(e)];
    __syncthreads();
  }
  ntt_forward<MODE, LOGN, kPF>(x, smem_raw, P, j, tid);
  uint64_t* out = (uint64_t*)dst.p[q] + ((size_t)out_slot * 2 * k + comp * k + j) * N;
#pragma unroll
  for (int e = 0; e < EPT; ++e) out[e * NT + tid] = A::out(x[e], m);
}


template <int MODE, bool P40, bool OUTF64 = false, int C0T = 0>
__global__ void __launch_bounds__(NT)
ks_last_ntt_kernel(const DevParams* __restrict__ P, const uint64_t* __restrict__ dig_raw,
                   KeyPtrs keys, const uint64_t* __restrict__ prod,
                   const double* __restrict__ xpow, uint32_t galois_elt, uint32_t galois_inv, uint32_t shift_pow,
                   uint32_t n_items, uint32_t B, MfmaPtrs dst, const uint64_t* __restrict__ tree_raw,
                   const uint16_t* __restrict__ perm) {
  using A = Arith<MODE>;
  static_assert(MODE != kNttInt, "fp64 flavours only");
  double* sd = reinterpret_cast<double*>(smem_raw);
  const uint32_t tid = threadIdx.x, k = P->k, km = k + 1;
  uint32_t node = blockIdx.x, j = blockIdx.y, comp = blockIdx.z;
  if (gridDim.y == 1 && gridDim.z == 1) {
    const uint32_t xcd = blockIdx.x & 7, t = blockIdx.x >> 3;
    comp = t & 1;
    const uint32_t u = t >> 1;
    j = u % k;
    node = (u / k) * 8 + xcd;
  }
  const typename A::Mod m = A::mod(P, j);
  const uint32_t slot = node / B, q = node % B;
  double x[EPT];
  {
    const double pf = P->p_f, half = P->p_half_f;
    const size_t spoly = ((size_t)node * 2 + comp) * km + k;
    [[maybe_unused]] Hi16 hs{};
    if constexpr (P40) hs = load40f_hi(reinterpret_cast<const uint8_t*>(prod) + spoly * kPoly40, tid);
#pragma unroll
    for (int e = 0; e < EPT; ++e) {
      double sp;
      if constexpr (P40)
        sp = load40f(reinterpret_cast<const uint8_t*>(prod) + spoly * kPoly40, hs, e, tid, f64_pack_magic(pf));
      else
        sp = reinterpret_cast<const double*>(prod)[spoly * N + e * NT + tid];
      sp = sp > half ? sp - pf : sp;
      sp = sp < -half ? sp + pf : sp;
      x[e] = f64_norm(sp, m);
    }
  }
  ntt_forward<MODE, LOGN, kPF, false>(x, smem_raw, P, j, tid);
  const size_t dpoly0 = ((size_t)node * km + j) * k;
  const double magic = f64_pack_magic(m.q);
  auto load_poly = [&](const uint64_t* base, size_t poly, double (&out)[EPT], uint32_t t) {
    if constexpr (P40) {
      const uint8_t* pp = reinterpret_cast<const uint8_t*>(base) + poly * kPoly40;
      const Hi16 h = load40f_hi(pp, t);
#pragma unroll
      for (int e = 0; e < EPT; ++e) out[e] = load40f(pp, h, e, t, magic);
    } else {
#pragma unroll
      for (int e = 0; e < EPT; ++e) out[e] = reinterpret_cast<const double*>(base)[poly * N + e * NT + t];
    }
  };
  {
#pragma unroll
    for (int e = 0; e < EPT; ++e) x[e] = -x[e];
    const double* key = reinterpret_cast<const double*>(keys.p[node % keys.B]);
    for (uint32_t J = 0; J < k; ++J) {
      const double* kj = key + (((size_t)J * 2 + comp) * km + j) * N;
      double d[EPT];
      load_poly(dig_raw, dpoly0 + J, d, tid);
#pragma unroll
      for (int e = 0; e < EPT; ++e) x[e] += f64_mulmod(d[e], kj[e * NT + tid], m);
    }
    const double pinv = P->p_inv_f[j];
#pragma unroll
    for (int e = 0; e < EPT; ++e) x[e] = f64_mulmod(f64_norm(x[e], m), pinv, m);
  }
  uint32_t tid_e = tid;
  asm volatile("" : "+v"(tid_e));
  double a[EPT];
  {
    double v[EPT];
    if (comp == 0) {
      if constexpr (C0T == 0) load_poly(prod, (size_t)node * 2 * km + j, v, tid_e);
      else tree_load<C0T == 2>(tree_raw, (size_t)node * 2 * k + j, tid_e, m.q, v);
    } else {
      load_poly(dig_raw, dpoly0 + j, v, tid_e);
    }
    __syncthreads();
#pragma unroll
    for (int e = 0; e < EPT; ++e) sd[lds_lin_base<NT, R_>(tid_e) + lds_lin_off<NT, R_>(e)] = v[e];
    __syncthreads();
    const uint32_t gel = comp == 0 ? galois_elt : galois_inv;
    [[maybe_unused]] PermIdx pi{};
    if constexpr (PIRGPU_PERM_TABLE != 0) pi = load_perm(perm + (comp == 0 ? 0 : N), tid_e);
#pragma unroll
    for (int e = 0; e < EPT; ++e) {
      const double w = sd[perm_at(pi, e, tid_e, gel)];
      if (comp == 0) {
        a[e] = v[e];
        x[e] += w;
      } else {
        a[e] = w;
      }
    }
  }
  const size_t opoly = (size_t)comp * k + j;
  uint64_t* lo = (uint64_t*)dst.p[q] + ((size_t)slot * 2 * k + opoly) * N;
#pragma unroll
  for (int e = 0; e < EPT; ++e) {
    const double r = f64_canon(f64_norm(a[e] + x[e], m), m);
    if constexpr (OUTF64) reinterpret_cast<double*>(lo)[e * NT + tid_e] = r;
    else lo[e * NT + tid_e] = A::out(r, m);
  }
  if (slot + shift_pow < n_items) {
    uint64_t* hi = (uint64_t*)dst.p[q] + ((size_t)(slot + shift_pow) * 2 * k + opoly) * N;
    const double* X = xpow + (size_t)j * N;
#pragma unroll
    for (int e = 0; e < EPT; ++e) {
      const double r = f64_canon(f64_mulmod(f64_norm(a[e] - x[e], m), X[e * NT + tid_e], m), m);
      if constexpr (OUTF64) reinterpret_cast<double*>(hi)[e * NT + tid_e] = r;
      else hi[e * NT + tid_e] = A::out(r, m);
    }
  }
}

template <int MODE, bool LDS_TW = false, bool SELF64 = false>
__global__ void __launch_bounds__(NT)
upper_fused_kernel(const DevParams* __restrict__ P, const uint64_t* __restrict__ src_all, MfmaPtrs svq,
                   uint64_t* __restrict__ part_all, uint32_t n_rows, uint32_t n_dim,
                   uint32_t n_children_total, uint32_t sv_first, uint32_t C, uint32_t chunk_len,
                   uint32_t n_chunks, uint64_t src_qstride, uint64_t part_qstride) {
  using A = Arith<MODE>;
  using T = typename A::T;
  const uint32_t tid = threadIdx.x, k = P->k, E = P->enc_count;
  const uint32_t per_query = n_rows * C * n_chunks;
  const uint32_t qi = blockIdx.x / per_query, bx = blockIdx.x % per_query;
  const uint64_t* src = src_all + (size_t)qi * src_qstride;
  const uint64_t* sv = reinterpret_cast<const uint64_t*>(svq.p[qi]);
  uint64_t* part = part_all + (size_t)qi * part_qstride;
  const uint32_t chunk = bx % n_chunks;
  const uint32_t cc = (bx / n_chunks) % C;
  const uint32_t r = bx / (n_chunks * C);
  const uint32_t e_idx = blockIdx.y, jt = blockIdx.z;
  const ModConst mc = P->mod[jt];
  const typename A::Mod m = A::mod(P, jt);
  const uint32_t sp = P->enc_poly[e_idx], sj = P->enc_res[e_idx], sh = P->enc_shift[e_idx];
  const uint64_t mask = (1ull << P->enc_bits) - 1;
  const uint64_t thr = P->plain_thr;
  const uint64_t inc = P->lift_inc[jt] >= mc.q ? P->lift_inc[jt] - mc.q : P->lift_inc[jt];
  const uint32_t child0 = r * n_dim;
  uint32_t nchild = n_children_total > child0 ? n_children_total - child0 : 0;
  if (nchild > n_dim) nchild = n_dim;
  const uint32_t ii0 = chunk * chunk_len;
  const uint32_t ii1 = ii0 + chunk_len < nchild ? ii0 + chunk_len : nchild;

  T acc0[EPT], acc1[EPT];
  u128 wide0[MODE == kNttInt ? EPT : 1], wide1[MODE == kNttInt ? EPT : 1];
#pragma unroll
  for (int e = 0; e < EPT; ++e) {
    acc0[e] = 0;
    acc1[e] = 0;
    if constexpr (MODE == kNttInt) wide0[e] = wide1[e] = 0;
  }
  const bool fast_lift = MODE != kNttInt && P->enc_bits <= 31 && P->t < mc.q;
  const double td = (double)P->t;
  const uint32_t thr32 = (uint32_t)thr, mask32 = (uint32_t)mask;
// ... 328 lines not shown
    PIRGPU_SET((ks_digit_kernel<MODE, true, false, true>));
    PIRGPU_SET((ks_digit_kernel<MODE, true, true, true>));
    PIRGPU_SET((upper_ntt_kernel<MODE, true>));
    PIRGPU_SET((ks_last_level_kernel<MODE, false>));
    PIRGPU_SET((ks_last_level_kernel<MODE, true>));
    PIRGPU_SET((tree_c0_ntt_kernel<MODE, false>));
    PIRGPU_SET((tree_c0_ntt_kernel<MODE, true>));
    PIRGPU_SET((ks_last_ntt_kernel<MODE, false>));
    PIRGPU_SET((ks_last_ntt_kernel<MODE, true>));
    PIRGPU_SET((ks_last_ntt_kernel<MODE, false, true>));
    PIRGPU_SET((ks_last_ntt_kernel<MODE, true, true>));
    PIRGPU_SET((ks_last_ntt_kernel<MODE, false, false, 1>));
    PIRGPU_SET((ks_last_ntt_kernel<MODE, false, true, 1>));
    PIRGPU_SET((ks_last_ntt_kernel<MODE, true, false, 1>));
    PIRGPU_SET((ks_last_ntt_kernel<MODE, true, true, 1>));
    PIRGPU_SET((ks_last_ntt_kernel<MODE, true, false, 2>));
    PIRGPU_SET((ks_last_ntt_kernel<MODE, true, true, 2>));
    PIRGPU_SET((upper_fused_kernel<MODE, false, true>));
  }
#undef PIRGPU_SET
  return hipSuccess;
}

static hipError_t op_configure(int mode) {
  PIRGPU_BY_MODE(mode, return configure_mode<MODE>());
  return hipSuccess;
}

static hipError_t op_ntt_batch(hipStream_t st, int mode, const DevParams* P, uint64_t* data, uint64_t n_polys,
                               uint32_t mod_period, uint32_t mod_base, bool inverse) {
  if (inverse) {
    PIRGPU_BY_MODE(mode, hipLaunchKernelGGL((ntt_batch_kernel<MODE, true>), dim3((uint32_t)n_polys), dim3(NT),
                                            kLdsBytes, st, P, data, mod_period, mod_base));
  } else {
    PIRGPU_BY_MODE(mode, hipLaunchKernelGGL((ntt_batch_kernel<MODE, false>), dim3((uint32_t)n_polys), dim3(NT),
                                            kLdsBytes, st, P, data, mod_period, mod_base));
  }
  return hipGetLastError();
}

static hipError_t op_ntt_inv_gather(hipStream_t st, int mode, const DevParams* P, uint32_t k, const uint64_t* src,
                                    uint64_t* dst, const SliceMap& map, uint32_t RC, uint32_t nq, uint32_t nq_total,
                                    uint32_t q0) {
  if (map.n == 0 || map.n > (uint32_t)kMaxSlices || map.cut[0] != 0 || map.cut[map.n] != k * (uint32_t)N || q0 + nq > nq_total)
    return hipErrorInvalidValue;
  for (uint32_t r = 0; r <= map.n; ++r)
    if (map.cut[r] % NT) return hipErrorInvalidValue;
  PIRGPU_BY_MODE(mode, hipLaunchKernelGGL(ntt_inv_gather_kernel<MODE>, dim3(nq * RC * k), dim3(NT), kLdsBytes, st, P, src, dst,
                                          map, RC, nq_total, q0));
  return hipGetLastError();
}

static hipError_t op_ct_ntt_fwd_oop(hipStream_t st, int mode, const DevParams* P, uint32_t k, const uint64_t* src,
                                    uint64_t* dst, uint64_t n_cts, bool src_is_tree) {
  const dim3 grid((uint32_t)(n_cts * 2 * k));
  if (src_is_tree) {
    PIRGPU_BY_MODE(mode, hipLaunchKernelGGL((ct_ntt_fwd_oop_kernel<MODE, true>), grid, dim3(NT), kLdsBytes, st, P, src, dst));
  } else {
    PIRGPU_BY_MODE(mode, hipLaunchKernelGGL((ct_ntt_fwd_oop_kernel<MODE, false>), grid, dim3(NT), kLdsBytes, st, P, src, dst));
  }
  return hipGetLastError();
}

static hipError_t op_ct_ntt_fwd_split(hipStream_t st, int mode, const DevParams* P, uint32_t k, const uint64_t* src,
                                      const MfmaPtrs& dst, uint32_t B, uint64_t n_cts_total) {
  PIRGPU_BY_MODE(mode, hipLaunchKernelGGL(ct_ntt_fwd_split_kernel<MODE>, dim3((uint32_t)(n_cts_total * 2 * k)),
                                          dim3(NT), kLdsBytes, st, P, src, dst, B));
  return hipGetLastError();
}

static hipError_t op_db_encode(hipStream_t st, int mode, const DevParams* P, uint32_t k, const uint64_t* coeffs,
                               const uint8_t* bytes, uint64_t bytes_per_pt, uint64_t total_bytes, uint32_t bits,
                               uint64_t n_pt, uint64_t* db, uint32_t planes, uint64_t plane_bytes,
                               uint64_t plane_stride) {
  if (planes < 1 || (planes > 1 && (coeffs || !plane_bytes || (uint64_t)(planes - 1) * plane_bytes >= bytes_per_pt)))
    return hipErrorInvalidValue;
  if (!n_pt) return hipSuccess;
  PIRGPU_BY_MODE(mode, hipLaunchKernelGGL(db_encode_kernel<MODE>, dim3((uint32_t)n_pt, k, planes), dim3(NT), kLdsBytes, st,
                                          P, coeffs, bytes, bytes_per_pt, total_bytes, bits, db,
                                          planes > 1 ? plane_bytes : 0, planes > 1 ? plane_stride : 0));
  return hipGetLastError();
}

static hipError_t op_ks_digit(hipStream_t st, int mode, const DevParams* P, uint32_t k, const uint64_t* res_in,
                              uint32_t galois_elt, uint32_t nodes, uint64_t* dig, bool pack40, uint64_t* c0_out,
                              bool tree40, bool loop_targets) {
  const bool wide = ks_digit_takes_c0(nodes);
  if (c0_out && (!wide || mode == kNttInt)) return hipErrorInvalidValue;
  if (tree40 && (!pack40 || mode == kNttInt)) return hipErrorInvalidValue;
  if (loop_targets && wide && mode != kNttInt) {
    const uint32_t digit_blocks = nodes * k;
    const dim3 grid(digit_blocks + (c0_out ? nodes * k : 0));
#define PIRGPU_KSD_LOOP(M, P40_, T40_)                                                                              \
  hipLaunchKernelGGL((ks_digit_kernel<M, P40_, T40_, true>), grid, dim3(NT), kLdsBytes, st, P, res_in, galois_elt, dig, \
                     c0_out, digit_blocks)
    if (mode == kNttF64) {
      if (tree40) PIRGPU_KSD_LOOP(kNttF64, true, true);
      else if (pack40) PIRGPU_KSD_LOOP(kNttF64, true, false);
      else PIRGPU_KSD_LOOP(kNttF64, false, false);
    } else {
      if (tree40) PIRGPU_KSD_LOOP(kNttF64Wide, true, true);
      else if (pack40) PIRGPU_KSD_LOOP(kNttF64Wide, true, false);
      else PIRGPU_KSD_LOOP(kNttF64Wide, false, false);
    }
#undef PIRGPU_KSD_LOOP
    return hipGetLastError();
  }
  const uint32_t digit_blocks = wide ? nodes * (k + 1) * k : 0xffffffffu;
  const dim3 grid = wide ? dim3(digit_blocks + (c0_out ? nodes * k : 0)) : dim3(nodes, k + 1, k);
  if (tree40) {
    if (mode == kNttF64)
      hipLaunchKernelGGL((ks_digit_kernel<kNttF64, true, true>), grid, dim3(NT), kLdsBytes, st, P, res_in, galois_elt, dig,
                         c0_out, digit_blocks);
    else
      hipLaunchKernelGGL((ks_digit_kernel<kNttF64Wide, true, true>), grid, dim3(NT), kLdsBytes, st, P, res_in, galois_elt,
                         dig, c0_out, digit_blocks);
  } else if (pack40) {
    PIRGPU_BY_MODE(mode, hipLaunchKernelGGL((ks_digit_kernel<MODE, true>), grid, dim3(NT), kLdsBytes, st, P, res_in,
                                            galois_elt, dig, c0_out, digit_blocks));
  } else {
    PIRGPU_BY_MODE(mode, hipLaunchKernelGGL((ks_digit_kernel<MODE, false>), grid, dim3(NT), kLdsBytes, st, P, res_in,
                                            galois_elt, dig, c0_out, digit_blocks));
  }
  return hipGetLastError();
}

static hipError_t op_ks_mac_intt(hipStream_t st, int mode, const DevParams* P, uint32_t k, const uint64_t* dig,
                                 const KeyPtrs& key, uint32_t nodes, uint64_t* prod, bool pack40, uint32_t I_base,
                                 uint32_t I_count) {
  const dim3 grid = nodes >= kWideLevel && nodes % 8 == 0 ? dim3(nodes * I_count * 2) : dim3(nodes, I_count, 2);
  if (pack40) {
    PIRGPU_BY_MODE(mode, hipLaunchKernelGGL((ks_mac_intt_kernel<MODE, true>), grid, dim3(NT), kLdsBytes, st, P, dig,
                                            key, prod, I_base, I_count));
  } else {
    PIRGPU_BY_MODE(mode, hipLaunchKernelGGL((ks_mac_intt_kernel<MODE, false>), grid, dim3(NT), kLdsBytes, st, P, dig,
                                            key, prod, I_base, I_count));
  }
  return hipGetLastError();
}

static hipError_t op_ks_mac_combine(hipStream_t st, int mode, const DevParams* P, uint32_t k, const uint64_t* dig,
                                    const KeyPtrs& key, const uint64_t* prod, const uint64_t* tree_in,
                                    uint32_t galois_elt, uint32_t nodes, uint32_t shift_pow, uint64_t* tree_out,
                                    bool pack40, bool tin40, bool tout40, const uint64_t* xpow, const uint16_t* perm,
                                    bool c0_split) {
  const dim3 grid = nodes >= kWideLevel && nodes % 8 == 0 ? dim3(nodes * k * 2) : dim3(nodes, k, 2);
  if (mode != kNttF64 && mode != kNttF64Wide) return hipErrorInvalidValue;
  if ((tin40 || tout40) && !pack40) return hipErrorInvalidValue;
  if (tout40 && shift_pow >= (uint32_t)NT) return hipErrorInvalidValue;
  const double* X = reinterpret_cast<const double*>(xpow);
  if (X && PIRGPU_PERM_TABLE != 0 && !perm) return hipErrorInvalidValue;
  if (X && c0_split) {
    const bool wide = nodes >= kWideLevel && nodes % 8 == 0;
    const dim3 g1 = wide ? dim3(nodes * k) : dim3(nodes, k, 1);
#define PIRGPU_C0K(M, P40, TI, TO)                                                                                  \
  do {                                                                                                              \
    hipLaunchKernelGGL((ks_c0_ntt_kernel<M, P40, TI, TO>), g1, dim3(NT), kLdsBytes, st, P, dig, key, prod, tree_in, \
                       galois_elt, nodes, tree_out, X, perm);                                                       \
    hipLaunchKernelGGL((ks_mac_combine_kernel<M, P40, TI, TO, false>), g1, dim3(NT), kLdsBytes, st, P, dig, key,    \
                       prod, tree_in, galois_elt, nodes, shift_pow, tree_out, X, perm, 1u);                         \
  } while (0)
#define PIRGPU_C0K_MODE(M)                                      \
  do {                                                          \
    if (!pack40) PIRGPU_C0K(M, false, false, false);            \
    else if (tin40 && tout40) PIRGPU_C0K(M, true, true, true);  \
    else if (tin40) PIRGPU_C0K(M, true, true, false);           \
    else if (tout40) PIRGPU_C0K(M, true, false, true);          \
    else PIRGPU_C0K(M, true, false, false);                     \
  } while (0)
    if (mode == kNttF64) PIRGPU_C0K_MODE(kNttF64);
    else PIRGPU_C0K_MODE(kNttF64Wide);
#undef PIRGPU_C0K_MODE
#undef PIRGPU_C0K
    return hipGetLastError();
  }
#define PIRGPU_MC(M, P40, TI, TO, C0)                                                                               \
  hipLaunchKernelGGL((ks_mac_combine_kernel<M, P40, TI, TO, C0>), grid, dim3(NT), kLdsBytes, st, P, dig, key, prod, \
                     tree_in, galois_elt, nodes, shift_pow, tree_out, X, perm, 0u)
#define PIRGPU_MC_FMT(M, C0)                                    \
  do {                                                          \
    if (!pack40) PIRGPU_MC(M, false, false, false, C0);         \
    else if (tin40 && tout40) PIRGPU_MC(M, true, true, true, C0);   \
    else if (tin40) PIRGPU_MC(M, true, true, false, C0);        \
    else if (tout40) PIRGPU_MC(M, true, false, true, C0);       \
    else PIRGPU_MC(M, true, false, false, C0);                  \
  } while (0)
#define PIRGPU_MC_MODE(M)                 \
  do {                                    \
    if (X) PIRGPU_MC_FMT(M, true);        \
    else PIRGPU_MC_FMT(M, false);         \
  } while (0)
  if (mode == kNttF64) PIRGPU_MC_MODE(kNttF64);
  else PIRGPU_MC_MODE(kNttF64Wide);
#undef PIRGPU_MC_MODE
#undef PIRGPU_MC_FMT
#undef PIRGPU_MC
  return hipGetLastError();
}

static hipError_t op_tree_c0_fwd(hipStream_t st, int mode, const DevParams* P, uint32_t k, uint64_t* tree, uint32_t cts) {
  if (mode == kNttF64) hipLaunchKernelGGL(tree_c0_fwd_kernel<kNttF64>, dim3(cts * k), dim3(NT), kLdsBytes, st, P, tree);
  else if (mode == kNttF64Wide) hipLaunchKernelGGL(tree_c0_fwd_kernel<kNttF64Wide>, dim3(cts * k), dim3(NT), kLdsBytes, st, P, tree);
  else return hipErrorInvalidValue;
  return hipGetLastError();
}

static hipError_t op_ks_last_level(hipStream_t st, int mode, const DevParams* P, uint32_t k, const uint64_t* tree,
                                   const uint64_t* prod, uint32_t galois_elt, uint32_t shift_pow, uint32_t n_items,
                                   uint32_t B, const MfmaPtrs& dst, uint32_t tree_cts, bool pack40) {
  const dim3 grid(tree_cts * 2 * k * 2);
  if (mode == kNttF64) {
    if (pack40)
      hipLaunchKernelGGL((ks_last_level_kernel<kNttF64, true>), grid, dim3(NT), kLdsBytes, st, P, tree, prod, galois_elt,
                         shift_pow, n_items, B, dst);
    else
      hipLaunchKernelGGL((ks_last_level_kernel<kNttF64, false>), grid, dim3(NT), kLdsBytes, st, P, tree, prod, galois_elt,
                         shift_pow, n_items, B, dst);
  } else if (mode == kNttF64Wide) {
    if (pack40)
      hipLaunchKernelGGL((ks_last_level_kernel<kNttF64Wide, true>), grid, dim3(NT), kLdsBytes, st, P, tree, prod,
                         galois_elt, shift_pow, n_items, B, dst);
    else
      hipLaunchKernelGGL((ks_last_level_kernel<kNttF64Wide, false>), grid, dim3(NT), kLdsBytes, st, P, tree, prod,
                         galois_elt, shift_pow, n_items, B, dst);
  } else {
    return hipErrorInvalidValue;
  }
  return hipGetLastError();
}

static hipError_t op_ks_last_ntt(hipStream_t st, int mode, const DevParams* P, uint32_t k, const uint64_t* tree,
                                 const uint64_t* dig, const KeyPtrs& key, uint64_t* prod, const uint64_t* xpow,
                                 uint32_t galois_elt, uint32_t galois_inv, uint32_t shift_pow, uint32_t n_items,
                                 uint32_t B, const MfmaPtrs& dst, uint32_t nodes, bool pack40, bool out_f64,
                                 bool c0_done, int c0_tree, const uint16_t* perm) {
  const dim3 g0(nodes * k);
  const dim3 grid = nodes >= kWideLevel && nodes % 8 == 0 ? dim3(nodes * k * 2) : dim3(nodes, k, 2);
  const double* X = reinterpret_cast<const double*>(xpow);
  if (c0_tree == 2 && !pack40) return hipErrorInvalidValue;
  if (PIRGPU_PERM_TABLE != 0 && !perm) return hipErrorInvalidValue;
#define PIRGPU_LAST_NTT_K(M, P40, OF, CT)                                                                          \
  hipLaunchKernelGGL((ks_last_ntt_kernel<M, P40, OF, CT>), grid, dim3(NT), kLdsBytes, st, P, dig, key, prod, X,    \
                     galois_elt, galois_inv, shift_pow, n_items, B, dst, tree, perm)
#define PIRGPU_LAST_NTT(M, P40)                                                                                    \
  do {                                                                                                             \
    if (c0_tree == 0 && !c0_done)                                                                                  \
      hipLaunchKernelGGL((tree_c0_ntt_kernel<M, P40>), g0, dim3(NT), kLdsBytes, st, P, tree, prod);                \
    if (c0_tree == 2) {                                                                                            \
      if constexpr (P40) {                                                                                         \
        if (out_f64) PIRGPU_LAST_NTT_K(M, P40, true, 2);                                                           \
        else PIRGPU_LAST_NTT_K(M, P40, false, 2);                                                                  \
      }                                                                                                            \
    } else if (c0_tree == 1) {                                                                                     \
      if (out_f64) PIRGPU_LAST_NTT_K(M, P40, true, 1);                                                             \
      else PIRGPU_LAST_NTT_K(M, P40, false, 1);                                                                    \
    } else {                                                                                                       \
      if (out_f64) PIRGPU_LAST_NTT_K(M, P40, true, 0);                                                             \
      else PIRGPU_LAST_NTT_K(M, P40, false, 0);                                                                    \
    }                                                                                                              \
  } while (0)
  if (mode == kNttF64) {
    if (pack40) PIRGPU_LAST_NTT(kNttF64, true);
    else PIRGPU_LAST_NTT(kNttF64, false);
  } else if (mode == kNttF64Wide) {
    if (pack40) PIRGPU_LAST_NTT(kNttF64Wide, true);
    else PIRGPU_LAST_NTT(kNttF64Wide, false);
  } else {
    return hipErrorInvalidValue;
  }
#undef PIRGPU_LAST_NTT
#undef PIRGPU_LAST_NTT_K
  return hipGetLastError();
}

static hipError_t op_upper_ntt(hipStream_t st, int mode, const DevParams* P, uint32_t k, uint32_t enc_count,
                               const uint64_t* src, uint64_t* scratch, uint32_t n_rows, uint32_t n_dim,
                               uint32_t n_children_total, uint32_t C, uint32_t b0, uint32_t blk, uint32_t n_queries,
                               uint64_t src_qstride, bool loop_source) {
  double* out = reinterpret_cast<double*>(scratch);
  if (loop_source) {
    const dim3 lgrid(n_queries * n_rows * C * blk, 2 * k, 1);
    if (mode == kNttF64)
      hipLaunchKernelGGL((upper_ntt_kernel<kNttF64, true>), lgrid, dim3(NT), kLdsBytes, st, P, src, out, n_rows, n_dim,
                         n_children_total, C, b0, blk, src_qstride);
    else if (mode == kNttF64Wide)
      hipLaunchKernelGGL((upper_ntt_kernel<kNttF64Wide, true>), lgrid, dim3(NT), kLdsBytes, st, P, src, out, n_rows, n_dim,
                         n_children_total, C, b0, blk, src_qstride);
    else
      return hipErrorInvalidValue;
    return hipGetLastError();
  }
  const dim3 grid(n_queries * n_rows * C * blk, enc_count, k);
  if (mode == kNttF64)
    hipLaunchKernelGGL(upper_ntt_kernel<kNttF64>, grid, dim3(NT), kLdsBytes, st, P, src, out, n_rows, n_dim,
                       n_children_total, C, b0, blk, src_qstride);
  else if (mode == kNttF64Wide)
    hipLaunchKernelGGL(upper_ntt_kernel<kNttF64Wide>, grid, dim3(NT), kLdsBytes, st, P, src, out, n_rows, n_dim,
                       n_children_total, C, b0, blk, src_qstride);
  else
    return hipErrorInvalidValue;
  return hipGetLastError();
}

static hipError_t op_upper_fused(hipStream_t st, int mode, const DevParams* P, uint32_t k, uint32_t enc_count,
                                 const uint64_t* src, const MfmaPtrs& svq, uint64_t* part, uint32_t n_rows,
                                 uint32_t n_dim, uint32_t n_children_total, uint32_t sv_first, uint32_t C,
                                 uint32_t chunk_len, uint32_t n_chunks, uint32_t n_queries, uint64_t src_qstride,
                                 uint64_t part_qstride, bool sel_f64) {
  const dim3 grid(n_queries * n_rows * C * n_chunks, enc_count, k);
#define PIRGPU_UF_ARGS P, src, svq, part, n_rows, n_dim, n_children_total, sv_first, C, chunk_len, n_chunks, src_qstride, part_qstride
  if (sel_f64 && mode == kNttInt) return hipErrorInvalidValue;
  if constexpr (kUpperLdsTw) {
    static const bool lds_tw = pirgpu_env("PIRGPU_UPPER_LDS_TW") && atoi(pirgpu_env("PIRGPU_UPPER_LDS_TW")) != 0;
    if (lds_tw && mode != kNttInt) {
      const size_t lds = kLdsBytes + (size_t)N * 8;
      if (mode == kNttF64 && sel_f64) hipLaunchKernelGGL((upper_fused_kernel<kNttF64, true, true>), grid, dim3(NT), lds, st, PIRGPU_UF_ARGS);
      else if (mode == kNttF64) hipLaunchKernelGGL((upper_fused_kernel<kNttF64, true>), grid, dim3(NT), lds, st, PIRGPU_UF_ARGS);
      else if (sel_f64) hipLaunchKernelGGL((upper_fused_kernel<kNttF64Wide, true, true>), grid, dim3(NT), lds, st, PIRGPU_UF_ARGS);
      else hipLaunchKernelGGL((upper_fused_kernel<kNttF64Wide, true>), grid, dim3(NT), lds, st, PIRGPU_UF_ARGS);
      return hipGetLastError();
    }
  }
  if (sel_f64) {
    if (mode == kNttF64) hipLaunchKernelGGL((upper_fused_kernel<kNttF64, false, true>), grid, dim3(NT), kLdsBytes, st, PIRGPU_UF_ARGS);
    else hipLaunchKernelGGL((upper_fused_kernel<kNttF64Wide, false, true>), grid, dim3(NT), kLdsBytes, st, PIRGPU_UF_ARGS);
    return hipGetLastError();
// ... 18 lines not shown
```

pir_amd/csrc/ntt_ring32k.hip:

```cpp
#include <hip/hip_runtime.h>
#include <stdint.h>

#include "device_params.h"
#include "kernels.h"
#include "ntt_core.h"

namespace pirgpu {
namespace ring32k {

constexpr int LOGN = 15;
constexpr uint32_t N = 1u << LOGN;
using A = Arith<kNttInt>;

constexpr int kColLog = 7;
constexpr uint32_t kRows = 1u << kColLog, kCols = N >> kColLog;
constexpr uint32_t kColsPerWg = 16, kColThreads = kRows / 16, kColWg = kColsPerWg * kColThreads;
constexpr uint32_t kColWords = kRows + kRows / 16;
constexpr int kBlkLog = 8;
constexpr uint32_t kBlk = 1u << kBlkLog, kBlocks = N >> kBlkLog;
constexpr uint32_t kBlksPerWg = 16, kBlkThreads = kBlk / 16, kBlkWg = kBlksPerWg * kBlkThreads;
constexpr uint32_t kBlkWords = kBlk + kBlk / 16;
static_assert(kCols % kColsPerWg == 0 && kBlocks % kBlksPerWg == 0, "whole workgroups per polynomial");

struct PolyMap {
// ... 304 lines not shown
  const uint32_t cc = (uint32_t)(poly % C);
  poly /= C;
  const uint32_t r = (uint32_t)(poly % n_rows);
  const uint32_t qi = (uint32_t)(poly / n_rows);
  const ModConst mc = P->mod[jt];
  const uint64_t* sv = reinterpret_cast<const uint64_t*>(svq.p[qi]);
  const size_t child_stride = (size_t)E * k * N;
  const uint64_t* x = scratch + ((((size_t)qi * n_rows + r) * C + cc) * blk * E + e_idx) * k * N + (size_t)jt * N + i;
  const uint32_t n_here = b0 < n_dim ? (n_dim - b0 < blk ? n_dim - b0 : blk) : 0;
  u128 a0 = 0, a1 = 0;
  uint32_t since = 0;
  for (uint32_t iib = 0; iib < n_here; ++iib) {
    const uint64_t* s0 = sv + (((size_t)(sv_first + b0 + iib) * 2 + 0) * k + jt) * N + i;
    const uint64_t v = x[(size_t)iib * child_stride];
    a0 += (u128)v * s0[0];
    a1 += (u128)v * s0[(size_t)k * N];
    if (++since == P->lazy_limit) {
      since = 0;
      a0 = reduce128((uint64_t)a0, (uint64_t)(a0 >> 64), mc);
      a1 = reduce128((uint64_t)a1, (uint64_t)(a1 >> 64), mc);
    }
  }
  uint64_t s0 = reduce128((uint64_t)a0, (uint64_t)(a0 >> 64), mc), s1 = reduce128((uint64_t)a1, (uint64_t)(a1 >> 64), mc);
  uint64_t* acc = acc_all + (size_t)qi * acc_qstride;
  uint64_t* out = out_all + (size_t)qi * out_qstride;
  const size_t slot = ((size_t)r * C + cc) * E + e_idx;
  const size_t o0 = ((slot * 2 + 0) * k + jt) * N + i, o1 = ((slot * 2 + 1) * k + jt) * N + i;
  if (!first) {
    s0 = add_mod(s0, acc[o0], mc.q);
    s1 = add_mod(s1, acc[o1], mc.q);
  }
  uint64_t* dst = last ? out : acc;
  dst[o0] = s0;
  dst[o1] = s1;
}


static hipError_t op_configure(int mode) { return mode == kNttInt ? hipSuccess : hipErrorInvalidValue; }

static hipError_t op_ntt_batch(hipStream_t st, int mode, const DevParams* P, uint64_t* data, uint64_t n_polys,
                               uint32_t mod_period, uint32_t mod_base, bool inverse) {
  if (mode != kNttInt) return hipErrorInvalidValue;
  return transform(st, P, contiguous(data, data, 1, mod_period, mod_base), n_polys, inverse);
}

static hipError_t op_ct_ntt_fwd_oop(hipStream_t st, int mode, const DevParams* P, uint32_t k, const uint64_t* src,
                                    uint64_t* dst, uint64_t n_cts, bool) {
  if (mode != kNttInt) return hipErrorInvalidValue;
  return transform(st, P, contiguous(src, dst, 1, k, 0), n_cts * 2 * k, false);
}

static hipError_t op_ct_ntt_fwd_split(hipStream_t st, int mode, const DevParams* P, uint32_t k, const uint64_t* src,
                                      const MfmaPtrs& dst, uint32_t B, uint64_t n_cts_total) {
  if (mode != kNttInt || B == 0 || B > (uint32_t)kMaxMfmaQueries) return hipErrorInvalidValue;
  PolyMap mp = contiguous(src, nullptr, 1, k, 0);
  mp.split = dst;
  mp.B = B;
  mp.k2 = 2 * k;
  return transform(st, P, mp, n_cts_total * 2 * k, false);
}

static hipError_t op_db_encode(hipStream_t st, int mode, const DevParams* P, uint32_t k, const uint64_t* coeffs,
                               const uint8_t* bytes, uint64_t bytes_per_pt, uint64_t total_bytes, uint32_t bits,
                               uint64_t n_pt, uint64_t* db, uint32_t planes, uint64_t plane_bytes,
                               uint64_t plane_stride) {
  if (mode != kNttInt) return hipErrorInvalidValue;
  if (planes < 1 || (planes > 1 && (coeffs || !plane_bytes || (uint64_t)(planes - 1) * plane_bytes >= bytes_per_pt)))
    return hipErrorInvalidValue;
  if (!n_pt) return hipSuccess;
  for (uint32_t pl = 0; pl < planes; ++pl) {
    uint64_t* dst = db + (size_t)pl * plane_stride * k * N;
    const uint64_t off = planes > 1 ? pl * plane_bytes : 0;
    const uint64_t len = planes > 1 && bytes_per_pt - off > plane_bytes ? plane_bytes : bytes_per_pt - off;
    hipLaunchKernelGGL(db_lift_kernel, ew_grid(n_pt * k), dim3(kEw), 0, st, P, coeffs, bytes, bytes_per_pt, total_bytes,
                       bits, dst, off, len);
    if (hipError_t e = hipGetLastError()) return e;
    if (hipError_t e = transform(st, P, contiguous(dst, dst, 1, k, 0), n_pt * k, false)) return e;
  }
  return hipSuccess;
}

static hipError_t op_ks_digit(hipStream_t st, int mode, const DevParams* P, uint32_t k, const uint64_t* res_in,
                              uint32_t galois_elt, uint32_t nodes, uint64_t* dig, bool pack40, uint64_t* c0_out,
                              bool tree40, bool) {
  if (mode != kNttInt || pack40 || c0_out || tree40) return hipErrorInvalidValue;
  if (!nodes) return hipSuccess;
  hipLaunchKernelGGL(galois_digits_kernel, ew_grid((uint64_t)nodes * k), dim3(kEw), 0, st, P, res_in, galois_elt, dig);
  if (hipError_t e = hipGetLastError()) return e;
  return transform(st, P, contiguous(dig, dig, k, k + 1, 0), (uint64_t)nodes * (k + 1) * k, false);
}

static hipError_t op_ks_mac_intt(hipStream_t st, int mode, const DevParams* P, uint32_t k, const uint64_t* dig,
                                 const KeyPtrs& key, uint32_t nodes, uint64_t* prod, bool pack40, uint32_t I_base,
                                 uint32_t I_count) {
  if (mode != kNttInt || pack40 || I_base != 0 || I_count != k + 1 || key.B == 0) return hipErrorInvalidValue;
  if (!nodes) return hipSuccess;
  const uint64_t polys = (uint64_t)nodes * 2 * (k + 1);
  hipLaunchKernelGGL(ks_mac_kernel, ew_grid(polys), dim3(kEw), 0, st, P, dig, key, prod);
  if (hipError_t e = hipGetLastError()) return e;
  return transform(st, P, contiguous(prod, prod, 1, k + 1, 0), polys, true);
}

static hipError_t op_upper_ntt(hipStream_t st, int mode, const DevParams* P, uint32_t k, uint32_t enc_count,
                               const uint64_t* src, uint64_t* scratch, uint32_t n_rows, uint32_t n_dim,
                               uint32_t n_children_total, uint32_t C, uint32_t b0, uint32_t blk, uint32_t n_queries,
                               uint64_t src_qstride, bool) {
  if (mode != kNttInt) return hipErrorInvalidValue;
  const uint64_t polys = (uint64_t)n_queries * n_rows * C * blk * enc_count * k;
  if (!polys) return hipSuccess;
  hipLaunchKernelGGL(upper_lift_kernel, ew_grid(polys), dim3(kEw), 0, st, P, src, scratch, n_rows, n_dim,
                     n_children_total, C, b0, blk, src_qstride);
  if (hipError_t e = hipGetLastError()) return e;
  return transform(st, P, contiguous(scratch, scratch, 1, k, 0), polys, false);
}

static hipError_t op_ntt_inv_gather(hipStream_t st, int mode, const DevParams* P, uint32_t k, const uint64_t* src,
                                    uint64_t* dst, const SliceMap& map, uint32_t RC, uint32_t nq, uint32_t nq_total,
                                    uint32_t q0) {
  if (mode != kNttInt) return hipErrorInvalidValue;
  const uint32_t kN = k * N;
  if (hipError_t e = launch_slots_assemble(st, src, dst, map, RC, kN, nq, (uint64_t)RC * kN, nq_total, q0)) return e;
  return transform(st, P, contiguous(dst, dst, 1, k, 0), (uint64_t)nq * RC * k, true);
}

}

hipError_t launch_upper_mac_int(hipStream_t st, const DevParams* P, const uint64_t* scratch, const MfmaPtrs& svq,
                                uint64_t* acc, uint64_t* out, uint32_t n_queries, uint32_t n_rows, uint32_t C,
                                uint32_t enc_count, uint32_t k, uint32_t N, uint32_t sv_first, uint32_t b0, uint32_t blk,
                                uint32_t n_dim, bool first, bool last, uint64_t acc_qstride, uint64_t out_qstride) {
  using namespace ring32k;
  if (N != ring32k::N) return hipErrorInvalidValue;
  const uint64_t polys = (uint64_t)n_queries * n_rows * C * enc_count * k;
  if (!polys) return hipSuccess;
  hipLaunchKernelGGL(upper_mac_int_kernel, ew_grid(polys), dim3(kEw), 0, st, P, scratch, svq, acc, out, n_rows, C,
                     sv_first, b0, blk, n_dim, first ? 1 : 0, last ? 1 : 0, acc_qstride, out_qstride);
  return hipGetLastError();
}

const NttOps* ntt_ops_15() {
  using namespace ring32k;
  static const NttOps ops = {op_configure, op_ntt_batch, op_ct_ntt_fwd_oop, op_ct_ntt_fwd_split, op_db_encode,
                             op_ks_digit,  op_ks_mac_intt,  nullptr,  nullptr,
                             op_upper_ntt,  nullptr,  nullptr, op_ntt_inv_gather,
                              nullptr};
  return &ops;
}

}
```

Before: 5476 queries/s.

## Chunk wide expansion levels into node spans to keep digit buffers cache-resident

New measurement: 5529 queries/s (median of 6 runs). Within noise of the previous version (+1.0%).

```diff
diff --git a/pir_amd/csrc/ctx.hip b/pir_amd/csrc/ctx.hip
--- a/pir_amd/csrc/ctx.hip
+++ b/pir_amd/csrc/ctx.hip
@@ -248,6 +248,8 @@
   uint64_t split_upper_words = (3ull << 30) / 8;
   bool loop_transforms = true;
   uint32_t loop_min_sources = 1024;
+  uint32_t expand_chunk_cts = 0;
+  bool expand_serpentine = false;
   uint32_t fuse_mac_nodes = 128;
   bool fuse_mac_combine = true;
   bool fuse_last_level = true;
@@ -591,6 +593,9 @@
   c->upper_blocks = (uint32_t)std::max<int64_t>(1, option(c, "UPPER_BLOCKS", c->upper_blocks));
   c->upper_blocks_batch = (uint32_t)std::max<int64_t>(1, option(c, "UPPER_BLOCKS_BATCH", c->upper_blocks_batch));
   c->scan_wgs_batch = (uint32_t)std::max<int64_t>(0, option(c, "SCAN_MFMA_WGS_BATCH", c->scan_wgs_batch));
+  if (c->logN == 12) c->expand_chunk_cts = 512;
+  c->expand_chunk_cts = (uint32_t)std::clamp<int64_t>(option(c, "EXPAND_CHUNK_CTS", c->expand_chunk_cts), 0, 1 << 30);
+  c->expand_serpentine = option(c, "EXPAND_SERPENTINE", c->expand_serpentine) != 0;
   c->upper_blocks_batch = std::min(c->upper_blocks_batch, c->upper_blocks);
   c->lvl_rows.assign(d, 0);
   c->lvl_cts.assign(d, 0);
@@ -875,6 +880,10 @@
   auto level_fused = [&](uint32_t j) {
     return c->mode != kNttInt && c->fuse_mac_combine && ((1u << j) * B) >= fuse_from && !(fuse_last && j + 1 == logm);
   };
+  const uint32_t chunk_cts = c->expand_chunk_cts & ~7u;
+  const bool serp = c->expand_serpentine;
+  bool rev = false;
+  bool down = false;
   for (uint32_t j = j_begin; j < j_stop; ++j) {
     auto level_done = [&]() {
       if (from && j == j_begin) {
@@ -887,23 +896,44 @@
     const uint32_t nodes = (1u << j) * B;
     const bool last_ntt = fuse_last && j + 1 == logm && c->last_level_ntt;
     const bool c0_in_digit = last_ntt && !c0ntt && ks_digit_takes_c0(nodes);
+    const bool wide = ks_digit_takes_c0(nodes);
+    auto turn = [&](NodeSpan sp) {
+      sp.reverse = serp && wide && rev;
+      if (serp && wide) rev = !rev;
+      return sp;
+    };
+    auto for_chunks = [&](auto&& body) {
+      const uint32_t step = wide && chunk_cts && chunk_cts < nodes ? chunk_cts : nodes;
+      const uint32_t n_chunks = (nodes + step - 1) / step;
+      for (uint32_t i = 0; i < n_chunks; ++i) {
+        const uint32_t first = (down ? n_chunks - 1 - i : i) * step;
+        body(NodeSpan{first, std::min(step, nodes - first), false});
+      }
+      if (serp) down = !down;
+    };
+    auto digit = [&](const NodeSpan& sp) {
+      HIP_TRY(c->ops->ks_digit(st, c->mode, c->dp, k, cur, g, nodes, dig, c->pack40, c0_in_digit ? prod : nullptr, cur40,
+                               c->loop_transforms && (uint64_t)nodes * k >= c->loop_min_sources, sp));
+    };
     if (cur40 && !(last_ntt ? (c0ntt || c0_in_digit) : true)) throw Fail{PIRGPU_INTERNAL, "5-byte tree reached a level that cannot read it"};
     if (c0_path && !c0ntt && level_fused(j) && !cur40 && !(from && j == j_begin)) {
       HIP_TRY(c->ops->tree_c0_fwd(st, c->mode, c->dp, k, cur, nodes));
       c0ntt = true;
     }
-    HIP_TRY(c->ops->ks_digit(st, c->mode, c->dp, k, cur, g, nodes, dig, c->pack40, c0_in_digit ? prod : nullptr, cur40,
-                             c->loop_transforms && (uint64_t)nodes * k >= c->loop_min_sources));
     if (level_fused(j)) {
       const uint32_t next_nodes = nodes * 2;
       const bool next_last = j + 2 == logm;
       const bool next_reads40 = next_last ? (fuse_last && c->last_level_ntt && (c0ntt || ks_digit_takes_c0(next_nodes)))
                                           : (next_nodes >= fuse_from);
       const bool out40 = c->tree40 && c->pack40 && j + 1 < logm && next_reads40 && (1u << j) < (N >> ntt_log_ept((int)c->logN));
-      HIP_TRY(c->ops->ks_mac_intt(st, c->mode, c->dp, k, dig, key, nodes, prod, c->pack40, k, 1));
-      HIP_TRY(c->ops->ks_mac_combine(st, c->mode, c->dp, k, dig, key, prod, cur, g, nodes, 1u << j, nxt, c->pack40, cur40,
-                                     out40, c0ntt ? xpow_table(c, st, 1u << j) : nullptr,
-                                     c0ntt ? galois_perm_table(c, st, g) : nullptr, c->c0_ntt_split));
+      const uint64_t* X = c0ntt ? xpow_table(c, st, 1u << j) : nullptr;
+      const uint16_t* perm = c0ntt ? galois_perm_table(c, st, g) : nullptr;
+      for_chunks([&](const NodeSpan& sp) {
+        digit(turn(sp));
+        HIP_TRY(c->ops->ks_mac_intt(st, c->mode, c->dp, k, dig, key, nodes, prod, c->pack40, k, 1, turn(sp)));
+        HIP_TRY(c->ops->ks_mac_combine(st, c->mode, c->dp, k, dig, key, prod, cur, g, nodes, 1u << j, nxt, c->pack40, cur40,
+                                       out40, X, perm, c->c0_ntt_split, turn(sp)));
+      });
       cur40 = out40;
       std::swap(cur, nxt);
       level_done();
@@ -913,13 +943,18 @@
     if (c0ntt && !last_ntt) throw Fail{PIRGPU_INTERNAL, "NTT-form c0 reached an unfused level"};
     if (fuse_last && j + 1 == logm && c->last_level_ntt) {
       const uint64_t* X = xpow_table(c, st, 1u << j);
-      HIP_TRY(c->ops->ks_mac_intt(st, c->mode, c->dp, k, dig, key, nodes, prod, c->pack40, k, 1));
-      HIP_TRY(c->ops->ks_last_ntt(st, c->mode, c->dp, k, cur, dig, key, prod, X, g, galois_inverse(g, N), 1u << j, n, B,
-                                  *sel_dst, nodes, c->pack40, sel_f64, c0_in_digit, c0ntt ? (cur40 ? 2 : 1) : 0,
-                                  galois_perm_table(c, st, g)));
+      const uint16_t* perm = galois_perm_table(c, st, g);
+      for_chunks([&](const NodeSpan& sp) {
+        digit(turn(sp));
+        HIP_TRY(c->ops->ks_mac_intt(st, c->mode, c->dp, k, dig, key, nodes, prod, c->pack40, k, 1, turn(sp)));
+        HIP_TRY(c->ops->ks_last_ntt(st, c->mode, c->dp, k, cur, dig, key, prod, X, g, galois_inverse(g, N), 1u << j, n, B,
+                                    *sel_dst, nodes, c->pack40, sel_f64, c0_in_digit, c0ntt ? (cur40 ? 2 : 1) : 0, perm,
+                                    turn(sp)));
+      });
       return nullptr;
     }
-    HIP_TRY(c->ops->ks_mac_intt(st, c->mode, c->dp, k, dig, key, nodes, prod, c->pack40, 0, k + 1));
+    digit(NodeSpan{});
+    HIP_TRY(c->ops->ks_mac_intt(st, c->mode, c->dp, k, dig, key, nodes, prod, c->pack40, 0, k + 1, NodeSpan{}));
     if (fuse_last && j + 1 == logm) {
       HIP_TRY(c->ops->ks_last_level(st, c->mode, c->dp, k, cur, prod, g, 1u << j, n, B, *sel_dst, nodes, c->pack40));
       return nullptr;
@@ -1273,8 +1308,8 @@
   const uint32_t N = c->N, k = c->k;
   const uint64_t pw = (uint64_t)k * N;
   HIP_TRY(launch_tree_convert(st, c->dp, c->mode, r.d, r.xq, (uint64_t)n * 2 * pw, true, 2 * pw, 3 * pw));
-  HIP_TRY(c->ops->ks_digit(st, c->mode, c->dp, k, r.xq, 1, n, r.dig, c->pack40, nullptr, false, false));
-  HIP_TRY(c->ops->ks_mac_intt(st, c->mode, c->dp, k, r.dig, key, n, r.prod, c->pack40, 0, k + 1));
+  HIP_TRY(c->ops->ks_digit(st, c->mode, c->dp, k, r.xq, 1, n, r.dig, c->pack40, nullptr, false, false, NodeSpan{}));
+  HIP_TRY(c->ops->ks_mac_intt(st, c->mode, c->dp, k, r.dig, key, n, r.prod, c->pack40, 0, k + 1, NodeSpan{}));
   HIP_TRY(launch_ks_combine(st, c->dp, c->mode, N, k, r.xq, r.prod, 1, n, 0, false, 0, c->pack40, r.yq, c->pack_bytes));
   if (c->mode != kNttInt) HIP_TRY(launch_tree_convert(st, c->dp, c->mode, r.yq, r.yq, (uint64_t)n * 2 * pw, false));
 }
@@ -1756,7 +1791,7 @@
     {"SCAN_MFMA", true}, {"SCAN_MFMA_WIDE", true}, {"SCAN_MFMA_TOP4", true}, {"SCAN_MFMA_NQ", true}, {"SCAN_MFMA_SINGLE", true},
     {"HEAD_LEVELS", true}, {"HEAD_MODE", true}, {"SCAN_F64_FOLD", true}, {"SCAN_F64_FOLD_BATCH", true}, {"LOOP_TRANSFORMS", true},
     {"SLOTS_SCAN_WGS", false}, {"SLOTS_GATHER_NTT", false}, {"SLOTS_SCAN_BLK_MAJOR", false}, {"DB_STREAM_MB", true},
-    {"CT_SCRATCH_MB", true}, {"CT_SHARED_SEL", true},
+    {"CT_SCRATCH_MB", true}, {"CT_SHARED_SEL", true}, {"EXPAND_CHUNK_CTS", false}, {"EXPAND_SERPENTINE", false},
     {"TABLES_ONE_LAUNCH", false}, {"SCAN_LAUNCHES", false},
     {"CT_BLOCKS", false},
     {"CT_RELINS", false}, {"CT_ROWSUM_SPLITS", false},
@@ -1790,6 +1825,8 @@
       }
       c->opts[up] = value;
       if (up == "SCAN_MFMA_WGS_BATCH") c->scan_wgs_batch = (uint32_t)std::max<int64_t>(0, value);
+      if (up == "EXPAND_CHUNK_CTS") c->expand_chunk_cts = (uint32_t)std::clamp<int64_t>(value, 0, 1 << 30);
+      if (up == "EXPAND_SERPENTINE") c->expand_serpentine = value != 0;
       return PIRGPU_OK;
     }
     return fail(c, PIRGPU_INVALID_ARGUMENT, "unknown option " + up);
@@ -1810,6 +1847,8 @@
         if (up == "CT_RELINS") *value = (int64_t)c->ct_relins;
         if (up == "CT_LIFTS") *value = (int64_t)c->ct_lifts;
         if (up == "CT_SHARED_SEL" && !present) *value = c->ctm && c->planes > 1;
+        if (up == "EXPAND_CHUNK_CTS" && c->ws_ready) *value = c->expand_chunk_cts;
+        if (up == "EXPAND_SERPENTINE" && c->ws_ready) *value = c->expand_serpentine;
         return PIRGPU_OK;
       }
     return fail(c, PIRGPU_INVALID_ARGUMENT, "unknown option " + up);
@@ -3098,8 +3137,8 @@
     key.B = 1;
     HIP_TRY(hipMemcpyAsync(w.res_b, ct, c->ctw * 8, hipMemcpyHostToDevice, c->stream));
     HIP_TRY(launch_tree_convert(c->stream, c->dp, c->mode, w.res_b, w.res_a, c->ctw, true));
-    HIP_TRY(c->ops->ks_digit(c->stream, c->mode, c->dp, c->k, w.res_a, power, 1, w.dig, c->pack40, nullptr, false, false));
-    HIP_TRY(c->ops->ks_mac_intt(c->stream, c->mode, c->dp, c->k, w.dig, key, 1, w.prod, c->pack40, 0, c->k + 1));
+    HIP_TRY(c->ops->ks_digit(c->stream, c->mode, c->dp, c->k, w.res_a, power, 1, w.dig, c->pack40, nullptr, false, false, NodeSpan{}));
+    HIP_TRY(c->ops->ks_mac_intt(c->stream, c->mode, c->dp, c->k, w.dig, key, 1, w.prod, c->pack40, 0, c->k + 1, NodeSpan{}));
     HIP_TRY(launch_ks_combine(c->stream, c->dp, c->mode, c->N, c->k, w.res_a, w.prod, galois_inverse(power, c->N), 1, 0,
                               false,  0, c->pack40, w.res_b, c->pack_bytes));
     HIP_TRY(launch_tree_convert(c->stream, c->dp, c->mode, w.res_b, w.res_b, c->ctw, false));
diff --git a/pir_amd/csrc/kernels.h b/pir_amd/csrc/kernels.h
--- a/pir_amd/csrc/kernels.h
+++ b/pir_amd/csrc/kernels.h
@@ -13,6 +13,11 @@
 
 constexpr uint32_t kKsWideLevel = 256;
 inline bool ks_digit_takes_c0(uint32_t nodes) { return nodes >= kKsWideLevel && nodes % 8 == 0; }
+
+struct NodeSpan {
+  uint32_t node0 = 0, count = 0;
+  bool reverse = false;
+};
 
 struct MfmaPtrs {
   const void* p[kMaxMfmaQueries];
@@ -53,10 +58,11 @@
                           uint64_t n_pt, uint64_t* db, uint32_t planes, uint64_t plane_bytes, uint64_t plane_stride);
   hipError_t (*ks_digit)(hipStream_t st, int mode, const DevParams* P, uint32_t k, const uint64_t* res_in,
                          uint32_t galois_elt, uint32_t nodes, uint64_t* dig, bool pack40, uint64_t* c0_out, bool tree40,
-                         bool loop_targets);
+                         bool loop_targets,
+                         const NodeSpan& span);
   hipError_t (*ks_mac_intt)(hipStream_t st, int mode, const DevParams* P, uint32_t k, const uint64_t* dig,
                             const KeyPtrs& key, uint32_t nodes, uint64_t* prod, bool pack40, uint32_t I_base,
-                            uint32_t I_count);
+                            uint32_t I_count, const NodeSpan& span);
   hipError_t (*upper_fused)(hipStream_t st, int mode, const DevParams* P, uint32_t k, uint32_t enc_count,
                             const uint64_t* src, const MfmaPtrs& svq, uint64_t* part, uint32_t n_rows,
                             uint32_t n_dim, uint32_t n_children_total, uint32_t sv_first, uint32_t C,
@@ -74,12 +80,14 @@
                                uint32_t nodes, uint32_t shift_pow, uint64_t* tree_out, bool pack40, bool tin40,
                                bool tout40, const uint64_t* xpow_c0ntt,
                                const uint16_t* perm,
-                               bool c0_split);
+                               bool c0_split,
+                               const NodeSpan& span);
   hipError_t (*ks_last_ntt)(hipStream_t st, int mode, const DevParams* P, uint32_t k, const uint64_t* tree,
                             const uint64_t* dig, const KeyPtrs& key, uint64_t* prod, const uint64_t* xpow,
                             uint32_t galois_elt, uint32_t galois_inv, uint32_t shift_pow, uint32_t n_items, uint32_t B,
                             const MfmaPtrs& dst, uint32_t nodes, bool pack40, bool out_f64, bool c0_done, int c0_tree,
-                            const uint16_t* perm);
+                            const uint16_t* perm,
+                            const NodeSpan& span);
   hipError_t (*ntt_inv_gather)(hipStream_t st, int mode, const DevParams* P, uint32_t k, const uint64_t* src,
                                uint64_t* dst, const SliceMap& map, uint32_t RC, uint32_t nq, uint32_t nq_total,
                                uint32_t q0);
diff --git a/pir_amd/csrc/ntt_kernels.hip b/pir_amd/csrc/ntt_kernels.hip
--- a/pir_amd/csrc/ntt_kernels.hip
+++ b/pir_amd/csrc/ntt_kernels.hip
@@ -70,6 +70,11 @@
 constexpr bool kUpperLdsTw = LOGN <= 12;
 constexpr uint32_t kWideLevel = kKsWideLevel;
 
+__device__ __forceinline__ uint32_t wide_t(uint32_t b, uint32_t blocks, uint32_t rev) {
+  const uint32_t t = b >> 3;
+  return rev ? (blocks >> 3) - 1 - t : t;
+}
+
 extern __shared__ __attribute__((aligned(16))) unsigned char smem_raw[];
 
 constexpr int kPB = PIRGPU_PACK_BYTES;
@@ -382,7 +387,8 @@
 
 template <int MODE, bool P40, bool T40>
 __device__ __forceinline__ void tree_c0_ntt_body(const DevParams* __restrict__ P, const uint64_t* __restrict__ tree_raw,
-                                                 uint64_t* __restrict__ prod, uint32_t node, uint32_t j, uint32_t tid) {
+                                                 uint64_t* __restrict__ prod, uint32_t node, uint32_t pnode, uint32_t j,
+                                                 uint32_t tid) {
   using A = Arith<MODE>;
   static_assert(MODE != kNttInt, "fp64 flavours only");
   const uint32_t k = P->k, km = k + 1;
@@ -390,7 +396,7 @@
   double x[EPT];
   tree_load<T40>(tree_raw, (size_t)node * 2 * k + j, tid, m.q, x);
   ntt_forward<MODE, LOGN, kPF, false>(x, smem_raw, P, j, tid);
-  const size_t opoly = (size_t)node * 2 * km + j;
+  const size_t opoly = (size_t)pnode * 2 * km + j;
   if constexpr (P40) {
     uint8_t* out = reinterpret_cast<uint8_t*>(prod) + opoly * kPoly40;
     store40f(out, tid, x, f64_pack_magic(m.q));
@@ -404,7 +410,7 @@
 template <int MODE, bool P40>
 __global__ void __launch_bounds__(NT)
 tree_c0_ntt_kernel(const DevParams* __restrict__ P, const uint64_t* __restrict__ tree_raw, uint64_t* __restrict__ prod) {
-  tree_c0_ntt_body<MODE, P40, false>(P, tree_raw, prod, blockIdx.x / P->k, blockIdx.x % P->k, threadIdx.x);
+  tree_c0_ntt_body<MODE, P40, false>(P, tree_raw, prod, blockIdx.x / P->k, blockIdx.x / P->k, blockIdx.x % P->k, threadIdx.x);
 }
 
 template <int MODE>
@@ -425,21 +431,23 @@
 template <int MODE, bool P40, bool T40 = false, bool LOOPI = false>
 __global__ void __launch_bounds__(NT) PIRGPU_FOUR_WAVES
 ks_digit_kernel(const DevParams* __restrict__ P, const uint64_t* __restrict__ res_in, uint32_t galois_elt,
-                uint64_t* __restrict__ dig, uint64_t* __restrict__ c0_out, uint32_t digit_blocks) {
+                uint64_t* __restrict__ dig, uint64_t* __restrict__ c0_out, uint32_t digit_blocks, uint32_t node0,
+                uint32_t rev) {
   using A = Arith<MODE>;
   uint64_t* s = reinterpret_cast<uint64_t*>(smem_raw);
   const uint32_t tid = threadIdx.x;
   const uint32_t k = P->k;
   if constexpr (MODE != kNttInt) {
     if (blockIdx.x >= digit_blocks) {
-      const uint32_t b = blockIdx.x - digit_blocks;
-      tree_c0_ntt_body<MODE, P40, T40>(P, res_in, c0_out, b / k, b % k, tid);
+      uint32_t b = blockIdx.x - digit_blocks;
+      if (rev) b = gridDim.x - digit_blocks - 1 - b;
+      tree_c0_ntt_body<MODE, P40, T40>(P, res_in, c0_out, node0 + b / k, b / k, b % k, tid);
       return;
     }
   }
   if constexpr (LOOPI) {
     static_assert(MODE != kNttInt, "fp64 flavours only");
-    const uint32_t xcd = blockIdx.x & 7, t = blockIdx.x >> 3;
+    const uint32_t xcd = blockIdx.x & 7, t = wide_t(blockIdx.x, digit_blocks, rev);
     const uint32_t J = t % k, node = (t / k) * 8 + xcd;
     double* sd = reinterpret_cast<double*>(smem_raw);
     const double qJd = P->tab[J].qd;
@@ -447,7 +455,7 @@
     double base[EPT];
     {
       double c1[EPT];
-      tree_load<T40>(res_in, ((size_t)node * 2 + 1) * k + J, tid, qJd, c1);
+      tree_load<T40>(res_in, ((size_t)(node0 + node) * 2 + 1) * k + J, tid, qJd, c1);
 #pragma unroll
       for (int e = 0; e < EPT; ++e) {
         const uint32_t raw = raw0 + (uint32_t)e * rstep;
@@ -485,7 +493,7 @@
   }
   uint32_t node = blockIdx.x, I = blockIdx.y, J = blockIdx.z;
   if (gridDim.y == 1) {
-    const uint32_t xcd = blockIdx.x & 7, t = blockIdx.x >> 3;
+    const uint32_t xcd = blockIdx.x & 7, t = wide_t(blockIdx.x, digit_blocks, rev);
     I = t % (k + 1);
     const uint32_t u = t / (k + 1);
     J = u % k;
@@ -494,7 +502,7 @@
   const ModConst mI = P->mod[I];
   const typename A::Mod m = A::mod(P, I);
   [[maybe_unused]] const uint64_t qJ = P->mod[J].q;
-  [[maybe_unused]] const uint64_t* src = res_in + (((size_t)node * 2 + 1) * k + J) * N;
+  [[maybe_unused]] const uint64_t* src = res_in + (((size_t)(node0 + node) * 2 + 1) * k + J) * N;
   typename A::T x[EPT];
   if constexpr (MODE == kNttInt) {
 #pragma unroll
@@ -514,7 +522,7 @@
     const double qJd = P->tab[J].qd;
     const uint32_t raw0 = tid * galois_elt, rstep = (uint32_t)NT * galois_elt;
     double c1[EPT];
-    tree_load<T40>(res_in, ((size_t)node * 2 + 1) * k + J, tid, qJd, c1);
+    tree_load<T40>(res_in, ((size_t)(node0 + node) * 2 + 1) * k + J, tid, qJd, c1);
 #pragma unroll
     for (int e = 0; e < EPT; ++e) {
       const uint32_t raw = raw0 + (uint32_t)e * rstep;
@@ -602,14 +610,14 @@
 template <int MODE, bool P40>
 __global__ void __launch_bounds__(NT) PIRGPU_PK_WAVES
 ks_mac_intt_kernel(const DevParams* __restrict__ P, const uint64_t* __restrict__ dig_raw, KeyPtrs keys,
-                   uint64_t* __restrict__ prod, uint32_t I_base, uint32_t I_count) {
+                   uint64_t* __restrict__ prod, uint32_t I_base, uint32_t I_count, uint32_t node0, uint32_t rev) {
   using A = Arith<MODE>;
   using T = typename A::T;
   const uint32_t tid = threadIdx.x;
   const uint32_t k = P->k, km = k + 1;
   uint32_t node = blockIdx.x, I = blockIdx.y, comp = blockIdx.z;
   if (gridDim.y == 1 && gridDim.z == 1) {
-    const uint32_t xcd = blockIdx.x & 7, t = blockIdx.x >> 3;
+    const uint32_t xcd = blockIdx.x & 7, t = wide_t(blockIdx.x, gridDim.x, rev);
     comp = t & 1;
     const uint32_t u = t >> 1;
     I = u % I_count;
@@ -618,7 +626,7 @@
   I += I_base;
   const typename A::Mod m = A::mod(P, I);
   T x[EPT];
-  ks_mac_core<MODE, P40>(P, dig_raw, keys.p[node % keys.B], node, I, comp, tid, x);
+  ks_mac_core<MODE, P40>(P, dig_raw, keys.p[(node0 + node) % keys.B], node, I, comp, tid, x);
   const size_t opoly = ((size_t)node * 2 + comp) * km + I;
   if constexpr (P40 && MODE != kNttInt) {
     uint8_t* out = reinterpret_cast<uint8_t*>(prod) + opoly * kPoly40;
@@ -643,7 +651,8 @@
                                                   const uint64_t* __restrict__ key_raw, const uint64_t* __restrict__ prod,
                                                   const uint64_t* __restrict__ tree_in_raw, const double* __restrict__ xpow,
                                                   const uint16_t* __restrict__ perm, uint32_t galois_elt, uint32_t nodes,
-                                                  uint32_t node, uint32_t j, uint32_t tid, uint64_t* __restrict__ tree_out_raw) {
+                                                  uint32_t node, uint32_t lnode, uint32_t j, uint32_t tid,
+                                                  uint64_t* __restrict__ tree_out_raw) {
   using A = Arith<MODE>;
   double* sd = reinterpret_cast<double*>(smem_raw);
   const uint32_t k = P->k, km = k + 1;
@@ -652,7 +661,7 @@
   double x[EPT];
   {
     const double pf = P->p_f, half = P->p_half_f;
-    const size_t spoly = ((size_t)node * 2 + 0) * km + k;
+    const size_t spoly = ((size_t)lnode * 2 + 0) * km + k;
     [[maybe_unused]] Hi16 hs{};
     if constexpr (P40) hs = load40f_hi(reinterpret_cast<const uint8_t*>(prod) + spoly * kPoly40, tid);
 #pragma unroll
@@ -669,7 +678,7 @@
   }
   ntt_forward<MODE, LOGN, kPF, false>(x, smem_raw, P, j, tid);
   {
-    const size_t dpoly0 = ((size_t)node * km + j) * k;
+    const size_t dpoly0 = ((size_t)lnode * km + j) * k;
 #pragma unroll
     for (int e = 0; e < EPT; ++e) x[e] = -x[e];
     const double* key = reinterpret_cast<const double*>(key_raw);
@@ -729,17 +738,18 @@
 ks_c0_ntt_kernel(const DevParams* __restrict__ P, const uint64_t* __restrict__ dig_raw, KeyPtrs keys,
                  const uint64_t* __restrict__ prod, const uint64_t* __restrict__ tree_in_raw, uint32_t galois_elt,
                  uint32_t nodes, uint64_t* __restrict__ tree_out_raw, const double* __restrict__ xpow,
-                 const uint16_t* __restrict__ perm) {
+                 const uint16_t* __restrict__ perm, uint32_t node0, uint32_t rev) {
   static_assert(MODE != kNttInt, "fp64 flavours only");
   const uint32_t k = P->k;
-  uint32_t node = blockIdx.x, j = blockIdx.y;
+  uint32_t lnode = blockIdx.x, j = blockIdx.y;
   if (gridDim.y == 1) {
-    const uint32_t xcd = blockIdx.x & 7, t = blockIdx.x >> 3;
+    const uint32_t xcd = blockIdx.x & 7, t = wide_t(blockIdx.x, gridDim.x, rev);
     j = t % k;
-    node = (t / k) * 8 + xcd;
-  }
+    lnode = (t / k) * 8 + xcd;
+  }
+  const uint32_t node = node0 + lnode;
   ks_combine_c0_ntt<MODE, P40, TIN40, TOUT40>(P, dig_raw, keys.p[node % keys.B], prod, tree_in_raw, xpow, perm, galois_elt, nodes,
-                                              node, j, threadIdx.x, tree_out_raw);
+                                              node, lnode, j, threadIdx.x, tree_out_raw);
 }
 
 template <int MODE, bool P40, bool TIN40 = false, bool TOUT40 = false, bool C0NTT = false>
@@ -748,34 +758,36 @@
                       KeyPtrs keys, const uint64_t* __restrict__ prod,
                       const uint64_t* __restrict__ tree_in_raw, uint32_t galois_elt, uint32_t nodes, uint32_t shift_pow,
                       uint64_t* __restrict__ tree_out_raw, const double* __restrict__ xpow,
-                      const uint16_t* __restrict__ perm, uint32_t comp1_only) {
+                      const uint16_t* __restrict__ perm, uint32_t comp1_only,
+                      uint32_t node0, uint32_t rev) {
   using A = Arith<MODE>;
   static_assert(MODE != kNttInt, "fp64 flavours only");
   double* sd = reinterpret_cast<double*>(smem_raw);
   const uint32_t tid = threadIdx.x, k = P->k, km = k + 1;
-  uint32_t node = blockIdx.x, j = blockIdx.y, comp = blockIdx.z;
+  uint32_t lnode = blockIdx.x, j = blockIdx.y, comp = blockIdx.z;
   if (gridDim.y == 1 && gridDim.z == 1) {
-    const uint32_t xcd = blockIdx.x & 7, t = blockIdx.x >> 3;
+    const uint32_t xcd = blockIdx.x & 7, t = wide_t(blockIdx.x, gridDim.x, rev);
     comp = comp1_only ? 1 : t & 1;
     const uint32_t u = comp1_only ? t : t >> 1;
     j = u % k;
-    node = (u / k) * 8 + xcd;
+    lnode = (u / k) * 8 + xcd;
   } else if (comp1_only) {
     comp = 1;
   }
+  const uint32_t node = node0 + lnode;
   if constexpr (C0NTT) {
     if (comp == 0) {
       ks_combine_c0_ntt<MODE, P40, TIN40, TOUT40>(P, dig_raw, keys.p[node % keys.B], prod, tree_in_raw, xpow, perm, galois_elt,
-                                                  nodes, node, j, tid, tree_out_raw);
+                                                  nodes, node, lnode, j, tid, tree_out_raw);
       return;
     }
   }
   const typename A::Mod m = A::mod(P, j);
   double g[EPT];
-  ks_mac_core<MODE, P40>(P, dig_raw, keys.p[node % keys.B], node, j, comp, tid, g);
+  ks_mac_core<MODE, P40>(P, dig_raw, keys.p[node % keys.B], lnode, j, comp, tid, g);
   {
     const double pf = P->p_f, half = P->p_half_f, pinv = P->p_inv_f[j];
-    const size_t spoly = ((size_t)node * 2 + comp) * km + k;
+    const size_t spoly = ((size_t)lnode * 2 + comp) * km + k;
     [[maybe_unused]] Hi16 hs{};
     if constexpr (P40) hs = load40f_hi(reinterpret_cast<const uint8_t*>(prod) + spoly * kPoly40, tid);
 #pragma unroll
@@ -937,25 +949,27 @@
                    KeyPtrs keys, const uint64_t* __restrict__ prod,
                    const double* __restrict__ xpow, uint32_t galois_elt, uint32_t galois_inv, uint32_t shift_pow,
                    uint32_t n_items, uint32_t B, MfmaPtrs dst, const uint64_t* __restrict__ tree_raw,
-                   const uint16_t* __restrict__ perm) {
+                   const uint16_t* __restrict__ perm,
+                   uint32_t node0, uint32_t rev) {
   using A = Arith<MODE>;
   static_assert(MODE != kNttInt, "fp64 flavours only");
   double* sd = reinterpret_cast<double*>(smem_raw);
   const uint32_t tid = threadIdx.x, k = P->k, km = k + 1;
-  uint32_t node = blockIdx.x, j = blockIdx.y, comp = blockIdx.z;
+  uint32_t lnode = blockIdx.x, j = blockIdx.y, comp = blockIdx.z;
   if (gridDim.y == 1 && gridDim.z == 1) {
-    const uint32_t xcd = blockIdx.x & 7, t = blockIdx.x >> 3;
+    const uint32_t xcd = blockIdx.x & 7, t = wide_t(blockIdx.x, gridDim.x, rev);
     comp = t & 1;
     const uint32_t u = t >> 1;
     j = u % k;
-    node = (u / k) * 8 + xcd;
-  }
+    lnode = (u / k) * 8 + xcd;
+  }
+  const uint32_t node = node0 + lnode;
   const typename A::Mod m = A::mod(P, j);
   const uint32_t slot = node / B, q = node % B;
   double x[EPT];
   {
     const double pf = P->p_f, half = P->p_half_f;
-    const size_t spoly = ((size_t)node * 2 + comp) * km + k;
+    const size_t spoly = ((size_t)lnode * 2 + comp) * km + k;
     [[maybe_unused]] Hi16 hs{};
     if constexpr (P40) hs = load40f_hi(reinterpret_cast<const uint8_t*>(prod) + spoly * kPoly40, tid);
 #pragma unroll
@@ -971,7 +985,7 @@
     }
   }
   ntt_forward<MODE, LOGN, kPF, false>(x, smem_raw, P, j, tid);
-  const size_t dpoly0 = ((size_t)node * km + j) * k;
+  const size_t dpoly0 = ((size_t)lnode * km + j) * k;
   const double magic = f64_pack_magic(m.q);
   auto load_poly = [&](const uint64_t* base, size_t poly, double (&out)[EPT], uint32_t t) {
     if constexpr (P40) {
@@ -1005,7 +1019,7 @@
   {
     double v[EPT];
     if (comp == 0) {
-      if constexpr (C0T == 0) load_poly(prod, (size_t)node * 2 * km + j, v, tid_e);
+      if constexpr (C0T == 0) load_poly(prod, (size_t)lnode * 2 * km + j, v, tid_e);
       else tree_load<C0T == 2>(tree_raw, (size_t)node * 2 * k + j, tid_e, m.q, v);
     } else {
       load_poly(dig_raw, dpoly0 + j, v, tid_e);
@@ -1500,18 +1514,28 @@
   return hipGetLastError();
 }
 
+static bool span_nodes(const NodeSpan& span, uint32_t nodes, bool wide, uint32_t& count) {
+  count = span.count ? span.count : nodes;
+  if (span.node0 > nodes || count > nodes - span.node0) return false;
+  if (wide) return span.node0 % 8 == 0 && count % 8 == 0;
+  return span.node0 == 0 && count == nodes && !span.reverse;
+}
+
 static hipError_t op_ks_digit(hipStream_t st, int mode, const DevParams* P, uint32_t k, const uint64_t* res_in,
                               uint32_t galois_elt, uint32_t nodes, uint64_t* dig, bool pack40, uint64_t* c0_out,
-                              bool tree40, bool loop_targets) {
+                              bool tree40, bool loop_targets, const NodeSpan& span) {
   const bool wide = ks_digit_takes_c0(nodes);
+  uint32_t cnt;
+  if (!span_nodes(span, nodes, wide, cnt)) return hipErrorInvalidValue;
+  const uint32_t node0 = span.node0, rev = span.reverse;
   if (c0_out && (!wide || mode == kNttInt)) return hipErrorInvalidValue;
   if (tree40 && (!pack40 || mode == kNttInt)) return hipErrorInvalidValue;
   if (loop_targets && wide && mode != kNttInt) {
-    const uint32_t digit_blocks = nodes * k;
-    const dim3 grid(digit_blocks + (c0_out ? nodes * k : 0));
+    const uint32_t digit_blocks = cnt * k;
+    const dim3 grid(digit_blocks + (c0_out ? cnt * k : 0));
 #define PIRGPU_KSD_LOOP(M, P40_, T40_)                                                                              \
   hipLaunchKernelGGL((ks_digit_kernel<M, P40_, T40_, true>), grid, dim3(NT), kLdsBytes, st, P, res_in, galois_elt, dig, \
-                     c0_out, digit_blocks)
+                     c0_out, digit_blocks, node0, rev)
     if (mode == kNttF64) {
       if (tree40) PIRGPU_KSD_LOOP(kNttF64, true, true);
       else if (pack40) PIRGPU_KSD_LOOP(kNttF64, true, false);
@@ -1524,35 +1548,39 @@
 #undef PIRGPU_KSD_LOOP
     return hipGetLastError();
   }
-  const uint32_t digit_blocks = wide ? nodes * (k + 1) * k : 0xffffffffu;
-  const dim3 grid = wide ? dim3(digit_blocks + (c0_out ? nodes * k : 0)) : dim3(nodes, k + 1, k);
+  const uint32_t digit_blocks = wide ? cnt * (k + 1) * k : 0xffffffffu;
+  const dim3 grid = wide ? dim3(digit_blocks + (c0_out ? cnt * k : 0)) : dim3(nodes, k + 1, k);
   if (tree40) {
     if (mode == kNttF64)
       hipLaunchKernelGGL((ks_digit_kernel<kNttF64, true, true>), grid, dim3(NT), kLdsBytes, st, P, res_in, galois_elt, dig,
-                         c0_out, digit_blocks);
+                         c0_out, digit_blocks, node0, rev);
     else
       hipLaunchKernelGGL((ks_digit_kernel<kNttF64Wide, true, true>), grid, dim3(NT), kLdsBytes, st, P, res_in, galois_elt,
-                         dig, c0_out, digit_blocks);
+                         dig, c0_out, digit_blocks, node0, rev);
   } else if (pack40) {
     PIRGPU_BY_MODE(mode, hipLaunchKernelGGL((ks_digit_kernel<MODE, true>), grid, dim3(NT), kLdsBytes, st, P, res_in,
-                                            galois_elt, dig, c0_out, digit_blocks));
+                                            galois_elt, dig, c0_out, digit_blocks, node0, rev));
   } else {
     PIRGPU_BY_MODE(mode, hipLaunchKernelGGL((ks_digit_kernel<MODE, false>), grid, dim3(NT), kLdsBytes, st, P, res_in,
-                                            galois_elt, dig, c0_out, digit_blocks));
+                                            galois_elt, dig, c0_out, digit_blocks, node0, rev));
   }
   return hipGetLastError();
 }
 
 static hipError_t op_ks_mac_intt(hipStream_t st, int mode, const DevParams* P, uint32_t k, const uint64_t* dig,
                                  const KeyPtrs& key, uint32_t nodes, uint64_t* prod, bool pack40, uint32_t I_base,
-                                 uint32_t I_count) {
-  const dim3 grid = nodes >= kWideLevel && nodes % 8 == 0 ? dim3(nodes * I_count * 2) : dim3(nodes, I_count, 2);
+                                 uint32_t I_count, const NodeSpan& span) {
+  const bool wide = nodes >= kWideLevel && nodes % 8 == 0;
+  uint32_t cnt;
+  if (!span_nodes(span, nodes, wide, cnt)) return hipErrorInvalidValue;
+  const uint32_t node0 = span.node0, rev = span.reverse;
+  const dim3 grid = wide ? dim3(cnt * I_count * 2) : dim3(nodes, I_count, 2);
   if (pack40) {
     PIRGPU_BY_MODE(mode, hipLaunchKernelGGL((ks_mac_intt_kernel<MODE, true>), grid, dim3(NT), kLdsBytes, st, P, dig,
-                                            key, prod, I_base, I_count));
+                                            key, prod, I_base, I_count, node0, rev));
   } else {
     PIRGPU_BY_MODE(mode, hipLaunchKernelGGL((ks_mac_intt_kernel<MODE, false>), grid, dim3(NT), kLdsBytes, st, P, dig,
-                                            key, prod, I_base, I_count));
+                                            key, prod, I_base, I_count, node0, rev));
   }
   return hipGetLastError();
 }
@@ -1561,22 +1589,25 @@
                                     const KeyPtrs& key, const uint64_t* prod, const uint64_t* tree_in,
                                     uint32_t galois_elt, uint32_t nodes, uint32_t shift_pow, uint64_t* tree_out,
                                     bool pack40, bool tin40, bool tout40, const uint64_t* xpow, const uint16_t* perm,
-                                    bool c0_split) {
-  const dim3 grid = nodes >= kWideLevel && nodes % 8 == 0 ? dim3(nodes * k * 2) : dim3(nodes, k, 2);
+                                    bool c0_split, const NodeSpan& span) {
+  const bool wide = nodes >= kWideLevel && nodes % 8 == 0;
+  uint32_t cnt;
+  if (!span_nodes(span, nodes, wide, cnt)) return hipErrorInvalidValue;
+  const uint32_t node0 = span.node0, rev = span.reverse;
+  const dim3 grid = wide ? dim3(cnt * k * 2) : dim3(nodes, k, 2);
   if (mode != kNttF64 && mode != kNttF64Wide) return hipErrorInvalidValue;
   if ((tin40 || tout40) && !pack40) return hipErrorInvalidValue;
   if (tout40 && shift_pow >= (uint32_t)NT) return hipErrorInvalidValue;
   const double* X = reinterpret_cast<const double*>(xpow);
   if (X && PIRGPU_PERM_TABLE != 0 && !perm) return hipErrorInvalidValue;
   if (X && c0_split) {
-    const bool wide = nodes >= kWideLevel && nodes % 8 == 0;
-    const dim3 g1 = wide ? dim3(nodes * k) : dim3(nodes, k, 1);
+    const dim3 g1 = wide ? dim3(cnt * k) : dim3(nodes, k, 1);
 #define PIRGPU_C0K(M, P40, TI, TO)                                                                                  \
   do {                                                                                                              \
     hipLaunchKernelGGL((ks_c0_ntt_kernel<M, P40, TI, TO>), g1, dim3(NT), kLdsBytes, st, P, dig, key, prod, tree_in, \
-                       galois_elt, nodes, tree_out, X, perm);                                                       \
+                       galois_elt, nodes, tree_out, X, perm, node0, rev);                                           \
     hipLaunchKernelGGL((ks_mac_combine_kernel<M, P40, TI, TO, false>), g1, dim3(NT), kLdsBytes, st, P, dig, key,    \
-                       prod, tree_in, galois_elt, nodes, shift_pow, tree_out, X, perm, 1u);                         \
+                       prod, tree_in, galois_elt, nodes, shift_pow, tree_out, X, perm, 1u, node0, rev);             \
   } while (0)
 #define PIRGPU_C0K_MODE(M)                                      \
   do {                                                          \
@@ -1594,7 +1625,7 @@
   }
 #define PIRGPU_MC(M, P40, TI, TO, C0)                                                                               \
   hipLaunchKernelGGL((ks_mac_combine_kernel<M, P40, TI, TO, C0>), grid, dim3(NT), kLdsBytes, st, P, dig, key, prod, \
-                     tree_in, galois_elt, nodes, shift_pow, tree_out, X, perm, 0u)
+                     tree_in, galois_elt, nodes, shift_pow, tree_out, X, perm, 0u, node0, rev)
 #define PIRGPU_MC_FMT(M, C0)                                    \
   do {                                                          \
     if (!pack40) PIRGPU_MC(M, false, false, false, C0);         \
@@ -1651,15 +1682,20 @@
                                  const uint64_t* dig, const KeyPtrs& key, uint64_t* prod, const uint64_t* xpow,
                                  uint32_t galois_elt, uint32_t galois_inv, uint32_t shift_pow, uint32_t n_items,
                                  uint32_t B, const MfmaPtrs& dst, uint32_t nodes, bool pack40, bool out_f64,
-                                 bool c0_done, int c0_tree, const uint16_t* perm) {
+                                 bool c0_done, int c0_tree, const uint16_t* perm, const NodeSpan& span) {
+  const bool wide = nodes >= kWideLevel && nodes % 8 == 0;
+  uint32_t cnt;
+  if (!span_nodes(span, nodes, wide, cnt)) return hipErrorInvalidValue;
+  const uint32_t node0 = span.node0, rev = span.reverse;
+  if (c0_tree == 0 && !c0_done && cnt != nodes) return hipErrorInvalidValue;
   const dim3 g0(nodes * k);
-  const dim3 grid = nodes >= kWideLevel && nodes % 8 == 0 ? dim3(nodes * k * 2) : dim3(nodes, k, 2);
+  const dim3 grid = wide ? dim3(cnt * k * 2) : dim3(nodes, k, 2);
   const double* X = reinterpret_cast<const double*>(xpow);
   if (c0_tree == 2 && !pack40) return hipErrorInvalidValue;
   if (PIRGPU_PERM_TABLE != 0 && !perm) return hipErrorInvalidValue;
 #define PIRGPU_LAST_NTT_K(M, P40, OF, CT)                                                                          \
   hipLaunchKernelGGL((ks_last_ntt_kernel<M, P40, OF, CT>), grid, dim3(NT), kLdsBytes, st, P, dig, key, prod, X,    \
-                     galois_elt, galois_inv, shift_pow, n_items, B, dst, tree, perm)
+                     galois_elt, galois_inv, shift_pow, n_items, B, dst, tree, perm, node0, rev)
 #define PIRGPU_LAST_NTT(M, P40)                                                                                    \
   do {                                                                                                             \
     if (c0_tree == 0 && !c0_done)                                                                                  \
diff --git a/pir_amd/csrc/ntt_ring32k.hip b/pir_amd/csrc/ntt_ring32k.hip
--- a/pir_amd/csrc/ntt_ring32k.hip
+++ b/pir_amd/csrc/ntt_ring32k.hip
@@ -410,8 +410,9 @@
 
 static hipError_t op_ks_digit(hipStream_t st, int mode, const DevParams* P, uint32_t k, const uint64_t* res_in,
                               uint32_t galois_elt, uint32_t nodes, uint64_t* dig, bool pack40, uint64_t* c0_out,
-                              bool tree40, bool) {
+                              bool tree40, bool, const NodeSpan& span) {
   if (mode != kNttInt || pack40 || c0_out || tree40) return hipErrorInvalidValue;
+  if (span.node0 || (span.count && span.count != nodes) || span.reverse) return hipErrorInvalidValue;
   if (!nodes) return hipSuccess;
   hipLaunchKernelGGL(galois_digits_kernel, ew_grid((uint64_t)nodes * k), dim3(kEw), 0, st, P, res_in, galois_elt, dig);
   if (hipError_t e = hipGetLastError()) return e;
@@ -420,8 +421,9 @@
 
 static hipError_t op_ks_mac_intt(hipStream_t st, int mode, const DevParams* P, uint32_t k, const uint64_t* dig,
                                  const KeyPtrs& key, uint32_t nodes, uint64_t* prod, bool pack40, uint32_t I_base,
-                                 uint32_t I_count) {
+                                 uint32_t I_count, const NodeSpan& span) {
   if (mode != kNttInt || pack40 || I_base != 0 || I_count != k + 1 || key.B == 0) return hipErrorInvalidValue;
+  if (span.node0 || (span.count && span.count != nodes) || span.reverse) return hipErrorInvalidValue;
   if (!nodes) return hipSuccess;
   const uint64_t polys = (uint64_t)nodes * 2 * (k + 1);
   hipLaunchKernelGGL(ks_mac_kernel, ew_grid(polys), dim3(kEw), 0, st, P, dig, key, prod);
```
